# hszhao/semseg

Hardware: NVIDIA B200
Metric: PSPNet50 473x473 training images/sec (higher is better)
Workload: dtype bf16

## Files before the change

include/semseg_b200.h:

```cpp
#ifndef SEMSEG_B200_H
#define SEMSEG_B200_H

#include <stdint.h>

#ifdef __cplusplus
extern "C" {
#endif

#define SEMSEG_OK 0
#define SEMSEG_E_INVALID (-1)
#define SEMSEG_E_CUDA (-2)
#define SEMSEG_E_UNSUPPORTED (-3)

#define SEMSEG_MAX_TAPS 9

const char* semseg_last_error(void);
int semseg_abi_version(void);
long long semseg_launch_count(void);

int semseg_psamask_fwd(int psa_type, const float* in, float* out, int N, int H, int W, int mH, int mW,
                       void* stream);
int semseg_psamask_bwd(int psa_type, const float* dout, float* din, int N, int H, int W, int mH, int mW,
                       void* stream);

int semseg_psa_attend(int mode, int psa_type, const float* attn, int a_pitch, const void* feat, const void* feat_lo,
                      int feat_pitch, float* stats, void* out, void* out_lo, int out_pitch, int N, int H, int W, int mH,
                      int mW, int C, float scale, void* stream);
int semseg_psa_attend_bwd_attn(int psa_type, const float* attn, int a_pitch, const float* stats, const void* feat,
                               const void* feat_lo, int feat_pitch, const void* out, const void* out_lo, int out_pitch,
                               const void* dout, const void* dout_lo, int dout_pitch, float* dattn, int N, int H, int W,
                               int mH, int mW, int C, float scale, void* stream);

enum {
  SEMSEG_EPI_RAW = 0,
  SEMSEG_EPI_AFFINE = 1,
  SEMSEG_EPI_F32 = 2
};

typedef struct semseg_conv_desc {
  int32_t N, H, W;
  int32_t Cin, Cout;
  const void* x;
  int32_t Nin, Hin, Win, x_pitch;
  const void* w;
  int32_t n_wtaps, w_rows, w_cols;
  int32_t taps;
  int32_t dh[SEMSEG_MAX_TAPS], dw[SEMSEG_MAX_TAPS], wtap[SEMSEG_MAX_TAPS];
  int32_t img_mul, img_add[SEMSEG_MAX_TAPS];
  int32_t epi_mode;
  int32_t relu;
  void* y;
  int32_t y_pitch;
  const float* scale;
  const float* shift;
  const void* residual;
  int32_t res_pitch;
  float* out_f32;
  int32_t out_pitch;
  float* stats_partial;
  const void* x_lo;
  void* y_lo;
  const void* residual_lo;
  int32_t w_split;
  int32_t k_slices;
  int64_t slice_stride;
} semseg_conv_desc;

int semseg_conv_k_slices(int Cin, int taps, int max_kblocks);
int semseg_conv_splitk_rows(int M);
int semseg_conv_splitk_finish(const float* partial, int k_slices, long long slice_stride, int part_pitch, int M, int C,
                              int epi_mode, int relu, const float* scale, const float* shift, const void* residual,
                              const void* residual_lo, int res_pitch, void* y, void* y_lo, int y_pitch,
                              float* stats_partial, void* stream);
int semseg_conv_stats_rows(int N, int H, int W, int Cout);
int semseg_conv_fprop(const semseg_conv_desc* d, void* stream);

typedef struct semseg_wgrad_desc {
  int32_t N, H, W;
  int32_t Cin, Cout;
  const void* x;
  int32_t Nin, Hin, Win, x_pitch;
  const void* dy;
  int32_t dy_pitch;
  int32_t taps;
  int32_t dh[SEMSEG_MAX_TAPS], dw[SEMSEG_MAX_TAPS];
  int32_t img_mul, img_add[SEMSEG_MAX_TAPS];
  float* dw_partial;
  int32_t n_splits;
  const void* x_lo;
  const void* dy_lo;
} semseg_wgrad_desc;

int semseg_conv_wgrad_splits(const semseg_wgrad_desc* d);
int semseg_conv_wgrad(const semseg_wgrad_desc* d, void* stream);
int semseg_wgrad_reduce(const float* dw_partial, int n_splits, int taps, int Cout, int Cin, float* dw_oihw,
                        int accumulate, void* stream);

int semseg_pack_weights(const float* w_oihw, int Cout, int Cin, int taps, void* wf, int rows_f, int cols_f,
                        void* wd, int rows_d, int cols_d, int split, void* stream);

typedef struct semseg_pack_item {
  const float* w;
  void* wf;
  void* wd;
  int Cout, Cin, taps;
  int cols_f, cols_d;
  int tile0, tiles_ci;
  int split;
} semseg_pack_item;
int semseg_pack_weights_multi(const semseg_pack_item* items_dev, int n_items, int n_tiles, int max_taps, void* stream);

int semseg_nchw_f32_to_nhwc_bf16(const float* in, void* out, void* out_lo, int N, int C, int H, int W, int out_pitch,
                                 void* stream);
int semseg_nhwc_bf16_to_nchw_f32(const void* in, const void* in_lo, float* out, int N, int C, int H, int W,
                                 int in_pitch, void* stream);
int semseg_nhwc_f32_to_nchw_f32(const float* in, float* out, int N, int C, int H, int W, int in_pitch,
                                void* stream);

int semseg_im2col3x3s2(const void* x, int x_pitch, int N, int H, int W, int Cin, void* out, void* stream);

int semseg_space_to_phases(const void* x, int x_pitch, int N, int H, int W, int C, void* xp, void* stream);
int semseg_phases_to_space(const void* xp, int N, int H, int W, int C, void* x, void* stream);

int semseg_bn_merge_partials(const float* stats_partial, int rows, int C, float* out_stats, void* stream);
int semseg_bn_stats(const void* x, int M, int C, int pitch, float* workspace, long long workspace_floats,
                    float* out_stats, void* stream);
long long semseg_bn_workspace_floats(int M, int C);
int semseg_bn_finalize(const float* rank_stats, int R, int C, const float* gamma, const float* beta, float eps,
                       float momentum, float* running_mean, float* running_var, float* mean_invstd,
                       float* scale_shift, void* stream);
int semseg_bn_finalize_partials(const float* stats_partial, int rows, int C, const float* gamma, const float* beta, float eps, float momentum,
                                float* running_mean, float* running_var, float* mean_invstd, float* scale_shift,
                                void* stream);
int semseg_bn_finalize_p2p(const float* stats_partial, int rows, int C, const float* gamma, const float* beta,
                           float eps, float momentum, float* running_mean, float* running_var, float* mean_invstd,
                           float* scale_shift, void* const* peer_bufs, void* const* peer_flags, void* counter,
                           int world, int rank, int slot, int slot_floats, unsigned seq, const void* seq_ptr,
                           void* stream);
int semseg_bn_bwd_reduce_p2p(const void* dy, const void* dy_lo, int dy_pitch, const void* y, const void* y_lo,
                             int y_pitch, const void* x, const void* x_lo, int x_pitch, const float* mean_invstd,
                             const float* scale_shift, int M, int C, int relu, float* workspace,
                             long long workspace_floats, float* sums_local, float* sums_total,
                             void* const* peer_bufs, void* const* peer_flags, void* counter, int world, int rank,
                             int slot, int slot_floats, unsigned seq, const void* seq_ptr, void* stream);
int semseg_bn_fold_eval(const float* gamma, const float* beta, const float* running_mean,
                        const float* running_var, float eps, int C, float* scale_shift, void* stream);
int semseg_bn_apply(const void* x, const void* x_lo, int x_pitch, const float* scale_shift, const void* residual,
                    const void* residual_lo, int res_pitch, void* y, void* y_lo, int y_pitch, int M, int C, int relu,
                    void* stream);
int semseg_bn_bwd_reduce(const void* dy, const void* dy_lo, int dy_pitch, const void* y, const void* y_lo, int y_pitch,
                         const void* x, const void* x_lo, int x_pitch, const float* mean_invstd,
                         const float* scale_shift, int M, int C, int relu, float* workspace,
                         long long workspace_floats, float* sums, void* stream);
int semseg_bn_bwd_apply(const void* dy, const void* dy_lo, int dy_pitch, const void* y, const void* y_lo, int y_pitch,
                        const void* x, const void* x_lo, int x_pitch, const float* mean_invstd, const float* gamma,
                        const float* scale_shift, const float* sums, float count, int M, int C, int relu, void* dx,
                        void* dx_lo, int dx_pitch, void* dres, void* dres_lo, int dres_pitch, float* dgamma_dbeta,
                        void* stream);
int semseg_add_act(const void* a, const void* a_lo, int a_pitch, const void* b, const void* b_lo, int b_pitch,
                   void* out, void* out_lo, int out_pitch, int M, int C, void* stream);
int semseg_scale_nc(const void* x, const void* x_lo, int x_pitch, const float* scale, void* out, void* out_lo,
                    int out_pitch, int N, int HW, int C, void* stream);
int semseg_f32_to_act(const float* in, int in_pitch, void* out, void* out_lo, int out_pitch, long long M, int C,
                      int Cp, void* stream);
int semseg_act_to_f32(const void* in, const void* in_lo, int in_pitch, float* out, int out_pitch, long long M, int C,
                      void* stream);

int semseg_maxpool3x3s2_fwd(const void* x, const void* x_lo, void* y, void* y_lo, void* argcode, int N, int H, int W,
                            int C, void* stream);
int semseg_maxpool3x3s2_bwd(const void* argcode, const void* dy, const void* dy_lo, void* dx, void* dx_lo, int N,
                            int H, int W, int C, void* stream);

int semseg_ppm_pool(const void* x, const void* x_lo, int x_pitch, int N, int H, int W, int C, const int* bins,
                    void* const* pooled, void* const* pooled_lo, int nb, void* stream);
int semseg_ppm_pool_bwd(void* const* dpooled, void* const* dpooled_lo, const int* bins, int nb, int N, int H, int W,
                        int C, void* dx, void* dx_lo, int dx_pitch, const void* add, const void* add_lo, int add_pitch,
                        void* stream);
int semseg_ppm_upsample_concat(const void* x, const void* x_lo, int x_pitch, void* const* feats, void* const* feats_lo,
                               const int* bins, int nb, int N, int H, int W, int C, int Cr, void* out, void* out_lo,
                               int out_pitch, void* stream);
int semseg_ppm_upsample_bwd(const void* dout, const void* dout_lo, int dout_pitch, int c_off, void* const* dfeats,
                            void* const* dfeats_lo, const int* bins, int nb, int N, int H, int W, int Cr, void* stream);

int semseg_resize_bilinear_fwd(const void* x, const void* x_lo, int x_pitch, int N, int Hi, int Wi, int C, int Ho,
                               int Wo, void* y, void* y_lo, int y_pitch, void* stream);
int semseg_resize_bilinear_bwd(const void* dy, const void* dy_lo, int dy_pitch, int N, int Hi, int Wi, int C, int Ho,
                               int Wo, void* dx, void* dx_lo, int dx_pitch, void* stream);

long long semseg_upsample_ce_workspace_floats(int N, int Ho, int Wo);
int semseg_upsample_ce_fwd(const float* logits, int pitch, int N, int h, int w, int C, const int64_t* target,
                           int Ho, int Wo, int ignore_index, float* workspace, float* loss_out, int64_t* argmax,
                           float* lse, void* stream);
long long semseg_upsample_ce_bwd_workspace_floats(int N, int Ho, int w, int C);
int semseg_upsample_ce_bwd(const float* logits, int pitch, int N, int h, int w, int C, const int64_t* target,
                           int Ho, int Wo, int ignore_index, const float* lse, const float* loss_info,
                           const float* grad_out, float* workspace, float* dlogits, void* stream);

int semseg_iou_hist(void* pred_i64, const void* target_i64, long long n, int K, long long ignore_index, int write_back,
                    int* counts, void* stream);

#define SEMSEG_SGD_MAX_GROUPS 16
typedef struct semseg_sgd_item {
  float* w;
  float* buf;
  long long n;
  int group;
  int chunk0;
  int first;
  int reserved;
} semseg_sgd_item;
typedef struct semseg_sgd_hyper {
  float lr[SEMSEG_SGD_MAX_GROUPS];
  float momentum[SEMSEG_SGD_MAX_GROUPS];
  float weight_decay[SEMSEG_SGD_MAX_GROUPS];
  float dampening[SEMSEG_SGD_MAX_GROUPS];
  int nesterov;
} semseg_sgd_hyper;
int semseg_sgd_chunk_elems(void);
int semseg_sgd_multi(const semseg_sgd_item* items_dev, const void* grad_ptrs_dev, int n_items, int n_chunks,
                     const semseg_sgd_hyper* hyper, void* stream);

#ifdef __cplusplus
}
#endif
#endif
```

semseg_b200/_lib.py:

```python
import ctypes
import os

_HERE = os.path.dirname(os.path.abspath(__file__))
LIB_PATH = os.path.join(_HERE, "lib", "libsemseg_b200.so")

MAX_TAPS = 9
EPI_RAW, EPI_AFFINE, EPI_F32 = 0, 1, 2

c_int = ctypes.c_int
c_i32 = ctypes.c_int32
c_vp = ctypes.c_void_p
c_f = ctypes.c_float
c_ll = ctypes.c_longlong
I9 = c_i32 * MAX_TAPS


class PackItem(ctypes.Structure):
    _fields_ = [
        ("w", c_vp), ("wf", c_vp), ("wd", c_vp),
        ("Cout", c_i32), ("Cin", c_i32), ("taps", c_i32),
        ("cols_f", c_i32), ("cols_d", c_i32),
        ("tile0", c_i32), ("tiles_ci", c_i32),
        ("split", c_i32),
    ]


class SgdItem(ctypes.Structure):
    _fields_ = [("w", c_vp), ("buf", c_vp), ("n", c_ll), ("group", c_i32), ("chunk0", c_i32), ("first", c_i32),
                ("reserved", c_i32)]


class SgdHyper(ctypes.Structure):
    _fields_ = [("lr", c_f * 16), ("momentum", c_f * 16), ("weight_decay", c_f * 16), ("dampening", c_f * 16),
                ("nesterov", c_i32)]


class ConvDesc(ctypes.Structure):
    _fields_ = [
        ("N", c_i32), ("H", c_i32), ("W", c_i32),
        ("Cin", c_i32), ("Cout", c_i32),
        ("x", c_vp),
        ("Nin", c_i32), ("Hin", c_i32), ("Win", c_i32), ("x_pitch", c_i32),
        ("w", c_vp),
        ("n_wtaps", c_i32), ("w_rows", c_i32), ("w_cols", c_i32),
        ("taps", c_i32),
        ("dh", I9), ("dw", I9), ("wtap", I9),
        ("img_mul", c_i32), ("img_add", I9),
        ("epi_mode", c_i32), ("relu", c_i32),
        ("y", c_vp), ("y_pitch", c_i32),
        ("scale", c_vp), ("shift", c_vp),
        ("residual", c_vp), ("res_pitch", c_i32),
        ("out_f32", c_vp), ("out_pitch", c_i32),
        ("stats_partial", c_vp),
        ("x_lo", c_vp), ("y_lo", c_vp), ("residual_lo", c_vp),
        ("w_split", c_i32),
        ("k_slices", c_i32), ("slice_stride", ctypes.c_int64),
    ]


class WgradDesc(ctypes.Structure):
    _fields_ = [
        ("N", c_i32), ("H", c_i32), ("W", c_i32),
        ("Cin", c_i32), ("Cout", c_i32),
        ("x", c_vp),
        ("Nin", c_i32), ("Hin", c_i32), ("Win", c_i32), ("x_pitch", c_i32),
        ("dy", c_vp), ("dy_pitch", c_i32),
        ("taps", c_i32),
        ("dh", I9), ("dw", I9),
        ("img_mul", c_i32), ("img_add", I9),
        ("dw_partial", c_vp),
        ("n_splits", c_i32),
        ("x_lo", c_vp), ("dy_lo", c_vp),
    ]


SIGNATURES = {
    "semseg_last_error": (ctypes.c_char_p, []),
    "semseg_abi_version": (c_int, []),
    "semseg_launch_count": (c_ll, []),
    "semseg_psamask_fwd": (c_int, [c_int, c_vp, c_vp, c_int, c_int, c_int, c_int, c_int, c_vp]),
    "semseg_psamask_bwd": (c_int, [c_int, c_vp, c_vp, c_int, c_int, c_int, c_int, c_int, c_vp]),
    "semseg_psa_attend": (c_int, [c_int, c_int, c_vp, c_int, c_vp, c_vp, c_int, c_vp, c_vp, c_vp, c_int, c_int, c_int,
                                  c_int, c_int, c_int, c_int, c_f, c_vp]),
    "semseg_psa_attend_bwd_attn": (c_int, [c_int, c_vp, c_int, c_vp, c_vp, c_vp, c_int, c_vp, c_vp, c_int, c_vp, c_vp,
                                           c_int, c_vp, c_int, c_int, c_int, c_int, c_int, c_int, c_f, c_vp]),
    "semseg_conv_stats_rows": (c_int, [c_int, c_int, c_int, c_int]),
    "semseg_conv_k_slices": (c_int, [c_int, c_int, c_int]),
    "semseg_conv_splitk_rows": (c_int, [c_int]),
    "semseg_conv_splitk_finish": (c_int, [c_vp, c_int, c_ll, c_int, c_int, c_int, c_int, c_int, c_vp, c_vp, c_vp, c_vp,
                                          c_int, c_vp, c_vp, c_int, c_vp, c_vp]),
    "semseg_conv_fprop": (c_int, [ctypes.POINTER(ConvDesc), c_vp]),
    "semseg_conv_wgrad_splits": (c_int, [ctypes.POINTER(WgradDesc)]),
    "semseg_conv_wgrad": (c_int, [ctypes.POINTER(WgradDesc), c_vp]),
    "semseg_wgrad_reduce": (c_int, [c_vp, c_int, c_int, c_int, c_int, c_vp, c_int, c_vp]),
    "semseg_pack_weights": (c_int, [c_vp, c_int, c_int, c_int, c_vp, c_int, c_int, c_vp, c_int, c_int, c_int, c_vp]),
    "semseg_pack_weights_multi": (c_int, [c_vp, c_int, c_int, c_int, c_vp]),
    "semseg_sgd_chunk_elems": (c_int, []),
    "semseg_sgd_multi": (c_int, [c_vp, c_vp, c_int, c_int, ctypes.POINTER(SgdHyper), c_vp]),
    "semseg_iou_hist": (c_int, [c_vp, c_vp, ctypes.c_longlong, c_int, ctypes.c_longlong, c_int, c_vp, c_vp]),
    "semseg_im2col3x3s2": (c_int, [c_vp, c_int, c_int, c_int, c_int, c_int, c_vp, c_vp]),
    "semseg_nchw_f32_to_nhwc_bf16": (c_int, [c_vp, c_vp, c_vp, c_int, c_int, c_int, c_int, c_int, c_vp]),
    "semseg_nhwc_bf16_to_nchw_f32": (c_int, [c_vp, c_vp, c_vp, c_int, c_int, c_int, c_int, c_int, c_vp]),
    "semseg_nhwc_f32_to_nchw_f32": (c_int, [c_vp, c_vp, c_int, c_int, c_int, c_int, c_int, c_vp]),
    "semseg_space_to_phases": (c_int, [c_vp, c_int, c_int, c_int, c_int, c_int, c_vp, c_vp]),
    "semseg_phases_to_space": (c_int, [c_vp, c_int, c_int, c_int, c_int, c_vp, c_vp]),
    "semseg_bn_merge_partials": (c_int, [c_vp, c_int, c_int, c_vp, c_vp]),
    "semseg_bn_stats": (c_int, [c_vp, c_int, c_int, c_int, c_vp, c_ll, c_vp, c_vp]),
    "semseg_bn_workspace_floats": (c_ll, [c_int, c_int]),
    "semseg_bn_finalize": (c_int, [c_vp, c_int, c_int, c_vp, c_vp, c_f, c_f, c_vp, c_vp, c_vp, c_vp, c_vp]),
    "semseg_bn_finalize_partials": (c_int, [c_vp, c_int, c_int, c_vp, c_vp, c_f, c_f, c_vp, c_vp, c_vp, c_vp, c_vp]),
    "semseg_bn_finalize_p2p": (c_int, [c_vp, c_int, c_int, c_vp, c_vp, c_f, c_f, c_vp, c_vp, c_vp, c_vp, c_vp, c_vp,
                                       c_vp, c_int, c_int, c_int, c_int, ctypes.c_uint, c_vp, c_vp]),
    "semseg_bn_bwd_reduce_p2p": (c_int, [c_vp, c_vp, c_int, c_vp, c_vp, c_int, c_vp, c_vp, c_int, c_vp, c_vp, c_int,
                                         c_int, c_int, c_vp, c_ll, c_vp, c_vp, c_vp, c_vp, c_vp, c_int, c_int, c_int,
                                         c_int, ctypes.c_uint, c_vp, c_vp]),
    "semseg_bn_fold_eval": (c_int, [c_vp, c_vp, c_vp, c_vp, c_f, c_int, c_vp, c_vp]),
    "semseg_bn_apply": (c_int, [c_vp, c_vp, c_int, c_vp, c_vp, c_vp, c_int, c_vp, c_vp, c_int, c_int, c_int, c_int,
                                c_vp]),
    "semseg_bn_bwd_reduce": (c_int, [c_vp, c_vp, c_int, c_vp, c_vp, c_int, c_vp, c_vp, c_int, c_vp, c_vp, c_int, c_int,
                                     c_int, c_vp, c_ll, c_vp, c_vp]),
    "semseg_bn_bwd_apply": (c_int, [c_vp, c_vp, c_int, c_vp, c_vp, c_int, c_vp, c_vp, c_int, c_vp, c_vp, c_vp, c_vp,
                                    c_f, c_int, c_int, c_int, c_vp, c_vp, c_int, c_vp, c_vp, c_int, c_vp, c_vp]),
    "semseg_add_act": (c_int, [c_vp, c_vp, c_int, c_vp, c_vp, c_int, c_vp, c_vp, c_int, c_int, c_int, c_vp]),
    "semseg_scale_nc": (c_int, [c_vp, c_vp, c_int, c_vp, c_vp, c_vp, c_int, c_int, c_int, c_int, c_vp]),
    "semseg_f32_to_act": (c_int, [c_vp, c_int, c_vp, c_vp, c_int, c_ll, c_int, c_int, c_vp]),
    "semseg_act_to_f32": (c_int, [c_vp, c_vp, c_int, c_vp, c_int, c_ll, c_int, c_vp]),
    "semseg_maxpool3x3s2_fwd": (c_int, [c_vp, c_vp, c_vp, c_vp, c_vp, c_int, c_int, c_int, c_int, c_vp]),
    "semseg_maxpool3x3s2_bwd": (c_int, [c_vp, c_vp, c_vp, c_vp, c_vp, c_int, c_int, c_int, c_int, c_vp]),
    "semseg_ppm_pool": (c_int, [c_vp, c_vp, c_int, c_int, c_int, c_int, c_int, c_vp, c_vp, c_vp, c_int, c_vp]),
    "semseg_ppm_pool_bwd": (c_int, [c_vp, c_vp, c_vp, c_int, c_int, c_int, c_int, c_int, c_vp, c_vp, c_int, c_vp, c_vp,
                                    c_int, c_vp]),
    "semseg_ppm_upsample_concat": (c_int, [c_vp, c_vp, c_int, c_vp, c_vp, c_vp, c_int, c_int, c_int, c_int, c_int,
                                           c_int, c_vp, c_vp, c_int, c_vp]),
    "semseg_ppm_upsample_bwd": (c_int, [c_vp, c_vp, c_int, c_int, c_vp, c_vp, c_vp, c_int, c_int, c_int, c_int, c_int,
                                        c_vp]),
    "semseg_resize_bilinear_fwd": (c_int, [c_vp, c_vp, c_int, c_int, c_int, c_int, c_int, c_int, c_int, c_vp, c_vp, c_int,
                                           c_vp]),
    "semseg_resize_bilinear_bwd": (c_int, [c_vp, c_vp, c_int, c_int, c_int, c_int, c_int, c_int, c_int, c_vp, c_vp, c_int,
                                           c_vp]),
    "semseg_upsample_ce_workspace_floats": (c_ll, [c_int, c_int, c_int]),
    "semseg_upsample_ce_fwd": (c_int, [c_vp, c_int, c_int, c_int, c_int, c_int, c_vp, c_int, c_int, c_int, c_vp,
                                       c_vp, c_vp, c_vp, c_vp]),
    "semseg_upsample_ce_bwd_workspace_floats": (c_ll, [c_int, c_int, c_int, c_int]),
    "semseg_upsample_ce_bwd": (c_int, [c_vp, c_int, c_int, c_int, c_int, c_int, c_vp, c_int, c_int, c_int, c_vp,
                                       c_vp, c_vp, c_vp, c_vp, c_vp]),
}

_lib = None


class SemsegError(RuntimeError):
    pass


def load():
    global _lib
    if _lib is not None:
        return _lib
    if not os.path.exists(LIB_PATH):
        raise SemsegError(
            "libsemseg_b200.so is not built (%s). Run `python -m semseg_b200.build` "
            "(or __graft_entry__.build()); there is no CPU/PyTorch fallback for this path." % LIB_PATH)
    lib = ctypes.CDLL(LIB_PATH)
    for name, (res, args) in SIGNATURES.items():
        fn = getattr(lib, name)
        fn.restype = res
        fn.argtypes = args
    _lib = lib
    return lib


def check(status, what):
    if status != 0:
        msg = load().semseg_last_error()
        raise SemsegError("%s failed (%d): %s" % (what, status, msg.decode() if msg else "?"))


def launch_count():
    return int(load().semseg_launch_count())
```

semseg_b200/csrc/act.cuh:

```cuda
#pragma once
#include <cuda_bf16.h>
#include <stdint.h>

#include "ptx.cuh"

namespace sb {

typedef __nv_bfloat16 bf16_t;

__device__ __forceinline__ void act_unpack8(const uint4& v, float (&f)[8]) {
  const __nv_bfloat162* h = reinterpret_cast<const __nv_bfloat162*>(&v);
#pragma unroll
  for (int q = 0; q < 4; ++q) {
    const float2 t = __bfloat1622float2(h[q]);
    f[2 * q] = t.x;
    f[2 * q + 1] = t.y;
  }
}
__device__ __forceinline__ uint4 act_pack8(const float (&f)[8]) {
  uint4 o;
  o.x = pack_bf16x2(f[0], f[1]);
  o.y = pack_bf16x2(f[2], f[3]);
  o.z = pack_bf16x2(f[4], f[5]);
  o.w = pack_bf16x2(f[6], f[7]);
  return o;
}

template <bool S>
struct Raw8 {
  uint4 h;
  uint4 l;
};
template <bool S>
__device__ __forceinline__ Raw8<S> act_ldraw(const bf16_t* hi, const bf16_t* lo, long long off) {
  Raw8<S> r;
  r.h = *reinterpret_cast<const uint4*>(hi + off);
  if constexpr (S) r.l = *reinterpret_cast<const uint4*>(lo + off);
  return r;
}
template <bool S>
__device__ __forceinline__ void act_unpack(const Raw8<S>& r, float (&f)[8]) {
  act_unpack8(r.h, f);
  if constexpr (S) {
    float g[8];
    act_unpack8(r.l, g);
#pragma unroll
    for (int q = 0; q < 8; ++q) f[q] += g[q];
  }
}
template <bool S>
__device__ __forceinline__ void act_ld8(const bf16_t* hi, const bf16_t* lo, long long off, float (&f)[8]) {
  act_unpack<S>(act_ldraw<S>(hi, lo, off), f);
}
template <bool S>
__device__ __forceinline__ void act_st8(bf16_t* hi, bf16_t* lo, long long off, const float (&f)[8]) {
  const uint4 h = act_pack8(f);
  *reinterpret_cast<uint4*>(hi + off) = h;
  if constexpr (S) {
    float hf[8], r[8];
    act_unpack8(h, hf);
#pragma unroll
    for (int q = 0; q < 8; ++q) r[q] = f[q] - hf[q];
    *reinterpret_cast<uint4*>(lo + off) = act_pack8(r);
  }
}
__device__ __forceinline__ void act_split1(float v, bf16_t& hi, bf16_t& lo) {
  hi = __float2bfloat16_rn(v);
  lo = __float2bfloat16_rn(v - __bfloat162float(hi));
}

#define SB_ACT_DISPATCH(split, ...)            \
  do {                                         \
    if (split) {                               \
      constexpr bool kS = true;                \
      __VA_ARGS__;                             \
    } else {                                   \
      constexpr bool kS = false;               \
      __VA_ARGS__;                             \
    }                                          \
  } while (0)

}
```

semseg_b200/csrc/bn.cu:

```cuda
#include "host_common.h"
#include "ptx.cuh"
#include "act.cuh"

namespace sb {

struct Moments {
  float n, mean, m2;
};
__device__ __forceinline__ Moments merge(const Moments& a, const Moments& b) {
  if (b.n == 0.f) return a;
  if (a.n == 0.f) return b;
  Moments r;
  r.n = a.n + b.n;
  const float d = b.mean - a.mean;
  r.mean = a.mean + d * (b.n / r.n);
  r.m2 = a.m2 + b.m2 + d * d * (a.n * b.n / r.n);
  return r;
}

__global__ void __launch_bounds__(1024) bn_merge_partials_kernel(const float* __restrict__ part, const float* __restrict__ cnt, int T, int C,
                                         float* __restrict__ out) {
  __shared__ Moments sm[32][33];
  const int cl = threadIdx.x & 31;
  const int tl = threadIdx.x >> 5;
  const int c = blockIdx.x * 32 + cl;
  Moments acc = {0.f, 0.f, 0.f};
  if (c < C) {
    for (int t = tl; t < T; t += 32) {
      const float n = cnt[t];
      if (n > 0.f) {
        Moments m;
        m.n = n;
        m.mean = part[(static_cast<size_t>(t) * 2) * C + c] / n;
        m.m2 = part[(static_cast<size_t>(t) * 2 + 1) * C + c];
        acc = merge(acc, m);
      }
    }
  }
  sm[tl][cl] = acc;
  __syncthreads();
  if (tl == 0 && c < C) {
    Moments r = sm[0][cl];
    for (int i = 1; i < 32; ++i) r = merge(r, sm[i][cl]);
    out[c] = r.mean;
    out[C + c] = r.m2;
    out[2 * C + c] = r.n;
  }
}


template <int CH>
__device__ __forceinline__ Moments block_conv_moments(const float* __restrict__ part, int T, int C, int c0,
                                                      Moments (*sm)[CH + 1]) {
  constexpr int RL = 1024 / CH;
  constexpr int U = 8;
  const int cl = threadIdx.x % CH;
  const int rl = threadIdx.x / CH;
  const int c = c0 + cl;
  float S = 0.f, Q = 0.f, n = 0.f;
  if (c < C) {
    for (int t0 = rl; t0 < T; t0 += RL * U) {
      float s[U], q[U], m[U];
#pragma unroll
      for (int u = 0; u < U; ++u) {
        const int t = t0 + RL * u;
        const bool ok = t < T;
        const float* row = part + static_cast<size_t>(ok ? t : 0) * 3 * C;
        s[u] = ok ? row[c] : 0.f;
        q[u] = ok ? row[C + c] : 0.f;
        m[u] = ok ? row[2 * C + c] : 0.f;
      }
#pragma unroll
      for (int u = 0; u < U; ++u) {
        S += s[u];
        Q += q[u];
        n += m[u];
      }
    }
  }
#pragma unroll
  for (int o = CH; o < 32; o <<= 1) {
    S += __shfl_xor_sync(0xffffffffu, S, o);
    Q += __shfl_xor_sync(0xffffffffu, Q, o);
    n += __shfl_xor_sync(0xffffffffu, n, o);
  }
  Moments acc = {0.f, 0.f, 0.f};
  if (n > 0.f) {
    acc.n = n;
    acc.mean = S / n;
    acc.m2 = fmaxf(Q - S * acc.mean, 0.f);
  }
  if ((threadIdx.x & 31) < CH) sm[threadIdx.x >> 5][cl] = acc;
  __syncthreads();
  Moments r = {0.f, 0.f, 0.f};
  const int w = threadIdx.x >> 5, lane = threadIdx.x & 31;
  if (w < CH) {
    r = sm[lane][w];
#pragma unroll
    for (int o = 16; o > 0; o >>= 1) {
      Moments other;
      other.mean = __shfl_down_sync(0xffffffffu, r.mean, o);
      other.m2 = __shfl_down_sync(0xffffffffu, r.m2, o);
      other.n = __shfl_down_sync(0xffffffffu, r.n, o);
      r = merge(r, other);
    }
  }
  return r;
}

static int stats_group_channels(int C) { return C <= 1024 ? 8 : (C <= 2048 ? 16 : 32); }

template <int CH>
__global__ void __launch_bounds__(1024) bn_merge_conv_partials_kernel(const float* __restrict__ part, int T, int C,
                                                                      float* __restrict__ out) {
  __shared__ Moments sm[32][CH + 1];
  const Moments r = block_conv_moments<CH>(part, T, C, blockIdx.x * CH, sm);
  const int c = blockIdx.x * CH + (threadIdx.x >> 5);
  if ((threadIdx.x & 31) == 0 && (threadIdx.x >> 5) < CH && c < C) {
    out[c] = r.mean;
    out[C + c] = r.m2;
    out[2 * C + c] = r.n;
  }
}

template <int CH>
__global__ void __launch_bounds__(1024) bn_finalize_partials_kernel(const float* __restrict__ part, int T, int C,
                                            const float* __restrict__ gamma, const float* __restrict__ beta,
                                            float eps, float momentum, float* __restrict__ running_mean,
                                            float* __restrict__ running_var, float* __restrict__ mean_invstd,
                                            float* __restrict__ scale_shift) {
  __shared__ Moments sm[32][CH + 1];
  const Moments r = block_conv_moments<CH>(part, T, C, blockIdx.x * CH, sm);
  const int c = blockIdx.x * CH + (threadIdx.x >> 5);
  if ((threadIdx.x & 31) == 0 && (threadIdx.x >> 5) < CH && c < C) {
    const float var = r.n > 0.f ? r.m2 / r.n : 0.f;
    const float invstd = rsqrtf(var + eps);
    mean_invstd[c] = r.mean;
    mean_invstd[C + c] = invstd;
    mean_invstd[2 * C + c] = r.n;
    const float sc = (gamma ? gamma[c] : 1.f) * invstd;
    scale_shift[c] = sc;
    scale_shift[C + c] = (beta ? beta[c] : 0.f) - r.mean * sc;
    if (running_mean) running_mean[c] = (1.f - momentum) * running_mean[c] + momentum * r.mean;
    if (running_var) {
      const float unb = r.n > 1.f ? r.m2 / (r.n - 1.f) : var;
      running_var[c] = (1.f - momentum) * running_var[c] + momentum * unb;
    }
  }
}

__global__ void bn_chunk_stats_kernel(const __nv_bfloat16* __restrict__ x, int M, int C, int pitch,
                                      int rows_per_chunk, float* __restrict__ part, float* __restrict__ cnt) {
  __shared__ float s_sum[32][65];
  const int gl = threadIdx.x & 7;
  const int pl = threadIdx.x >> 3;
  const int c0 = blockIdx.x * 64 + gl * 8;
  const int chunk = blockIdx.y;
  const int r0 = chunk * rows_per_chunk;
  const int r1 = min(M, r0 + rows_per_chunk);
  const bool active = c0 < C;
  float s[8] = {0, 0, 0, 0, 0, 0, 0, 0};
  if (active) {
    for (int r = r0 + pl; r < r1; r += 32) {
      const uint4 v = *reinterpret_cast<const uint4*>(x + static_cast<size_t>(r) * pitch + c0);
      const __nv_bfloat162* h = reinterpret_cast<const __nv_bfloat162*>(&v);
#pragma unroll
      for (int q = 0; q < 4; ++q) {
        const float2 f = __bfloat1622float2(h[q]);
        s[2 * q] += f.x;
        s[2 * q + 1] += f.y;
      }
    }
  }
#pragma unroll
  for (int q = 0; q < 8; ++q) s_sum[pl][gl * 8 + q] = s[q];
  __syncthreads();
  const float n = static_cast<float>(r1 - r0);
  float mean[8];
#pragma unroll
  for (int q = 0; q < 8; ++q) {
    float t = 0.f;
    for (int i = 0; i < 32; ++i) t += s_sum[i][gl * 8 + q];
    mean[q] = t / n;
    s[q] = t;
  }
  __syncthreads();
  float m2[8] = {0, 0, 0, 0, 0, 0, 0, 0};
  if (active) {
    for (int r = r0 + pl; r < r1; r += 32) {
      const uint4 v = *reinterpret_cast<const uint4*>(x + static_cast<size_t>(r) * pitch + c0);
      const __nv_bfloat162* h = reinterpret_cast<const __nv_bfloat162*>(&v);
#pragma unroll
      for (int q = 0; q < 4; ++q) {
        const float2 f = __bfloat1622float2(h[q]);
        const float d0 = f.x - mean[2 * q], d1 = f.y - mean[2 * q + 1];
        m2[2 * q] = fmaf(d0, d0, m2[2 * q]);
        m2[2 * q + 1] = fmaf(d1, d1, m2[2 * q + 1]);
      }
    }
  }
#pragma unroll
  for (int q = 0; q < 8; ++q) s_sum[pl][gl * 8 + q] = m2[q];
  __syncthreads();
  if (pl == 0 && active) {
#pragma unroll
    for (int q = 0; q < 8; ++q) {
      float t = 0.f;
      for (int i = 0; i < 32; ++i) t += s_sum[i][gl * 8 + q];
      if (c0 + q < C) {
        part[(static_cast<size_t>(chunk) * 2) * C + c0 + q] = s[q];
        part[(static_cast<size_t>(chunk) * 2 + 1) * C + c0 + q] = t;
      }
    }
  }
  if (blockIdx.x == 0 && threadIdx.x == 0) cnt[chunk] = n;
}

__global__ void bn_finalize_kernel(const float* __restrict__ rs, int R, int C, const float* __restrict__ gamma,
                                   const float* __restrict__ beta, float eps, float momentum,
                                   float* __restrict__ running_mean, float* __restrict__ running_var,
                                   float* __restrict__ mean_invstd, float* __restrict__ scale_shift) {
  const int c = blockIdx.x * blockDim.x + threadIdx.x;
  if (c >= C) return;
  Moments acc = {0.f, 0.f, 0.f};
  for (int r = 0; r < R; ++r) {
    const float* b = rs + static_cast<size_t>(r) * 3 * C;
    Moments m;
    m.mean = b[c];
    m.m2 = b[C + c];
    m.n = b[2 * C + c];
    acc = merge(acc, m);
  }
  const float var = acc.n > 0.f ? acc.m2 / acc.n : 0.f;
  const float invstd = rsqrtf(var + eps);
  mean_invstd[c] = acc.mean;
  mean_invstd[C + c] = invstd;
  mean_invstd[2 * C + c] = acc.n;
  const float g = gamma ? gamma[c] : 1.f;
  const float bt = beta ? beta[c] : 0.f;
  const float sc = g * invstd;
  scale_shift[c] = sc;
  scale_shift[C + c] = bt - acc.mean * sc;
  if (running_mean) running_mean[c] = (1.f - momentum) * running_mean[c] + momentum * acc.mean;
  if (running_var) {
    const float unb = acc.n > 1.f ? acc.m2 / (acc.n - 1.f) : var;
    running_var[c] = (1.f - momentum) * running_var[c] + momentum * unb;
  }
}

__global__ void bn_fold_eval_kernel(const float* __restrict__ gamma, const float* __restrict__ beta,
                                    const float* __restrict__ rm, const float* __restrict__ rv, float eps, int C,
                                    float* __restrict__ scale_shift) {
  const int c = blockIdx.x * blockDim.x + threadIdx.x;
  if (c >= C) return;
  const float invstd = rsqrtf(rv[c] + eps);
  const float sc = (gamma ? gamma[c] : 1.f) * invstd;
  scale_shift[c] = sc;
  scale_shift[C + c] = (beta ? beta[c] : 0.f) - rm[c] * sc;
}

__device__ __forceinline__ void unpack8(const uint4& v, float (&f)[8]) {
  const __nv_bfloat162* h = reinterpret_cast<const __nv_bfloat162*>(&v);
#pragma unroll
  for (int q = 0; q < 4; ++q) {
    const float2 t = __bfloat1622float2(h[q]);
    f[2 * q] = t.x;
    f[2 * q + 1] = t.y;
  }
}
__device__ __forceinline__ uint4 pack8(const float (&f)[8]) {
  uint4 o;
  o.x = pack_bf16x2(f[0], f[1]);
  o.y = pack_bf16x2(f[2], f[3]);
  o.z = pack_bf16x2(f[4], f[5]);
  o.w = pack_bf16x2(f[6], f[7]);
  return o;
}

template <bool S>
__global__ void bn_apply_kernel(const __nv_bfloat16* __restrict__ x, const __nv_bfloat16* __restrict__ x_lo, int x_pitch,
                                const float* __restrict__ ss, const __nv_bfloat16* __restrict__ res,
                                const __nv_bfloat16* __restrict__ res_lo, int res_pitch, __nv_bfloat16* __restrict__ y,
                                __nv_bfloat16* __restrict__ y_lo, int y_pitch, long long M, int C, int relu) {
  const int groups = C >> 3;
  long long idx = static_cast<long long>(blockIdx.x) * blockDim.x + threadIdx.x;
  const long long stride = static_cast<long long>(gridDim.x) * blockDim.x;
  const int c0 = static_cast<int>(idx % groups) << 3;
  float sc[8], sh[8];
#pragma unroll
  for (int q = 0; q < 8; ++q) {
    sc[q] = ss[c0 + q];
    sh[q] = ss[C + c0 + q];
  }
  const long long pstride = stride / groups;
  long long p = idx / groups;
  constexpr int U = 4;
  for (; p + (U - 1) * pstride < M; p += U * pstride) {
    Raw8<S> xv[U], rv[U];
#pragma unroll
    for (int u = 0; u < U; ++u) xv[u] = act_ldraw<S>(x, x_lo, (p + u * pstride) * x_pitch + c0);
    if (res) {
#pragma unroll
      for (int u = 0; u < U; ++u) rv[u] = act_ldraw<S>(res, res_lo, (p + u * pstride) * res_pitch + c0);
    }
#pragma unroll
    for (int u = 0; u < U; ++u) {
      float f[8], r[8] = {0, 0, 0, 0, 0, 0, 0, 0};
      act_unpack<S>(xv[u], f);
      if (res) act_unpack<S>(rv[u], r);
#pragma unroll
      for (int q = 0; q < 8; ++q) {
        float v = fmaf(f[q], sc[q], sh[q]) + r[q];
        if (relu) v = fmaxf(v, 0.f);
        f[q] = v;
      }
      act_st8<S>(y, y_lo, (p + u * pstride) * y_pitch + c0, f);
    }
  }
  for (; p < M; p += pstride) {
    float f[8], r[8] = {0, 0, 0, 0, 0, 0, 0, 0};
    act_ld8<S>(x, x_lo, p * x_pitch + c0, f);
    if (res) act_ld8<S>(res, res_lo, p * res_pitch + c0, r);
#pragma unroll
    for (int q = 0; q < 8; ++q) {
      float v = fmaf(f[q], sc[q], sh[q]) + r[q];
      if (relu) v = fmaxf(v, 0.f);
      f[q] = v;
    }
    act_st8<S>(y, y_lo, p * y_pitch + c0, f);
  }
}

template <bool S>
__global__ void bn_bwd_reduce_kernel(const __nv_bfloat16* __restrict__ dy, const __nv_bfloat16* __restrict__ dy_lo,
                                     int dy_pitch, const __nv_bfloat16* __restrict__ y,
                                     const __nv_bfloat16* __restrict__ y_lo, int y_pitch,
                                     const __nv_bfloat16* __restrict__ x, const __nv_bfloat16* __restrict__ x_lo,
                                     int x_pitch, const float* __restrict__ mean_invstd, const float* __restrict__ ss,
                                     int M, int C, int relu, int rows_per_chunk, float* __restrict__ part) {
  __shared__ float s_a[32][65];
  __shared__ float s_b[32][65];
  const int gl = threadIdx.x & 7;
  const int pl = threadIdx.x >> 3;
  const int c0 = blockIdx.x * 64 + gl * 8;
  const int chunk = blockIdx.y;
  const int r0 = chunk * rows_per_chunk;
  const int r1 = min(M, r0 + rows_per_chunk);
  const bool active = c0 < C;
  float a[8] = {0, 0, 0, 0, 0, 0, 0, 0}, b[8] = {0, 0, 0, 0, 0, 0, 0, 0};
  if (active) {
    float mean[8], invstd[8], msc[8], msh[8];
#pragma unroll
    for (int q = 0; q < 8; ++q) {
      mean[q] = mean_invstd[c0 + q];
      invstd[q] = mean_invstd[C + c0 + q];
      msc[q] = ss ? ss[c0 + q] : 0.f;
      msh[q] = ss ? ss[C + c0 + q] : 0.f;
    }
    const bool mask_from_y = relu && y != nullptr;
    const bool mask_from_x = relu && y == nullptr;
    constexpr int U = S ? 2 : 4;
    auto accumulate = [&](float (&d)[8], const float (&xv)[8], const float (&yv)[8]) {
      if (mask_from_y) {
#pragma unroll
        for (int q = 0; q < 8; ++q)
          if (!(yv[q] > 0.f)) d[q] = 0.f;
      } else if (mask_from_x) {
#pragma unroll
        for (int q = 0; q < 8; ++q)
          if (!(fmaf(xv[q], msc[q], msh[q]) > 0.f)) d[q] = 0.f;
      }
#pragma unroll
      for (int q = 0; q < 8; ++q) {
        a[q] += d[q];
        b[q] = fmaf(d[q], (xv[q] - mean[q]) * invstd[q], b[q]);
      }
    };
    int r = r0 + pl;
    for (; r + (U - 1) * 32 < r1; r += U * 32) {
      Raw8<S> dv[U], xr[U], yr[U];
#pragma unroll
      for (int u = 0; u < U; ++u) {
        dv[u] = act_ldraw<S>(dy, dy_lo, static_cast<long long>(r + u * 32) * dy_pitch + c0);
        xr[u] = act_ldraw<S>(x, x_lo, static_cast<long long>(r + u * 32) * x_pitch + c0);
      }
      if (mask_from_y) {
#pragma unroll
        for (int u = 0; u < U; ++u) yr[u] = act_ldraw<S>(y, y_lo, static_cast<long long>(r + u * 32) * y_pitch + c0);
      }
#pragma unroll
      for (int u = 0; u < U; ++u) {
        float d[8], xv[8], yv[8] = {0, 0, 0, 0, 0, 0, 0, 0};
        act_unpack<S>(dv[u], d);
        act_unpack<S>(xr[u], xv);
        if (mask_from_y) act_unpack<S>(yr[u], yv);
        accumulate(d, xv, yv);
      }
    }
    for (; r < r1; r += 32) {
      float d[8], xv[8], yv[8] = {0, 0, 0, 0, 0, 0, 0, 0};
      act_ld8<S>(dy, dy_lo, static_cast<long long>(r) * dy_pitch + c0, d);
      act_ld8<S>(x, x_lo, static_cast<long long>(r) * x_pitch + c0, xv);
      if (mask_from_y) act_ld8<S>(y, y_lo, static_cast<long long>(r) * y_pitch + c0, yv);
      accumulate(d, xv, yv);
    }
  }
#pragma unroll
  for (int q = 0; q < 8; ++q) {
    s_a[pl][gl * 8 + q] = a[q];
    s_b[pl][gl * 8 + q] = b[q];
  }
  __syncthreads();
  if (pl < 2 && active) {
    float(*src)[65] = pl == 0 ? s_a : s_b;
#pragma unroll
    for (int q = 0; q < 8; ++q) {
      float t = 0.f;
      for (int i = 0; i < 32; ++i) t += src[i][gl * 8 + q];
      if (c0 + q < C) part[(static_cast<size_t>(chunk) * 2 + pl) * C + c0 + q] = t;
    }
  }
}

__global__ void __launch_bounds__(1024) bn_bwd_reduce_final_kernel(const float* __restrict__ part, int chunks, int C,
                                           float* __restrict__ sums) {
  __shared__ float sm[32][33];
  const int cl = threadIdx.x & 31;
  const int tl = threadIdx.x >> 5;
  const int idx = blockIdx.x * 32 + cl;
  float acc = 0.f;
  if (idx < 2 * C) {
    const int which = idx / C, c = idx - which * C;
    constexpr int U = 8;
    for (int t0 = tl; t0 < chunks; t0 += 32 * U) {
      float v[U];
#pragma unroll
      for (int u = 0; u < U; ++u) {
        const int t = t0 + 32 * u;
        v[u] = t < chunks ? part[(static_cast<size_t>(t) * 2 + which) * C + c] : 0.f;
      }
#pragma unroll
      for (int u = 0; u < U; ++u) acc += v[u];
    }
  }
  sm[tl][cl] = acc;
  __syncthreads();
  if (tl == 0 && idx < 2 * C) {
    float r = 0.f;
    for (int i = 0; i < 32; ++i) r += sm[i][cl];
    sums[idx] = r;
  }
}

template <bool S>
__global__ void bn_bwd_apply_kernel(const __nv_bfloat16* __restrict__ dy, const __nv_bfloat16* __restrict__ dy_lo,
                                    int dy_pitch, const __nv_bfloat16* __restrict__ y,
                                    const __nv_bfloat16* __restrict__ y_lo, int y_pitch,
                                    const __nv_bfloat16* __restrict__ x, const __nv_bfloat16* __restrict__ x_lo,
                                    int x_pitch, const float* __restrict__ mean_invstd, const float* __restrict__ gamma,
                                    const float* __restrict__ ss, const float* __restrict__ sums, float inv_count,
                                    long long M, int C, int relu, __nv_bfloat16* __restrict__ dx,
                                    __nv_bfloat16* __restrict__ dx_lo, int dx_pitch, __nv_bfloat16* __restrict__ dres,
                                    __nv_bfloat16* __restrict__ dres_lo, int dres_pitch,
                                    float* __restrict__ dgamma_dbeta) {
  const int groups = C >> 3;
  if (dgamma_dbeta && blockIdx.x == 0) {
    for (int c = threadIdx.x; c < C; c += blockDim.x) {
      dgamma_dbeta[c] = sums[C + c];
      dgamma_dbeta[C + c] = sums[c];
    }
  }
  long long idx = static_cast<long long>(blockIdx.x) * blockDim.x + threadIdx.x;
  const long long stride = static_cast<long long>(gridDim.x) * blockDim.x;
  const int c0 = static_cast<int>(idx % groups) << 3;
  float ka[8], kx[8], kb[8], msc[8], msh[8];
  const bool mask_from_y = relu && y != nullptr;
  const bool mask_from_x = relu && y == nullptr;
#pragma unroll
  for (int q = 0; q < 8; ++q) {
    const int c = c0 + q;
    msc[q] = ss ? ss[c] : 0.f;
    msh[q] = ss ? ss[C + c] : 0.f;
    const float mean = mean_invstd[c], invstd = mean_invstd[C + c];
    const float g = gamma ? gamma[c] : 1.f;
    ka[q] = g * invstd;
    const float ic = inv_count > 0.f ? inv_count : 1.f / mean_invstd[2 * C + c];
    kx[q] = -ka[q] * invstd * sums[C + c] * ic;
    kb[q] = -ka[q] * sums[c] * ic - kx[q] * mean;
  }
  auto finish = [&](float (&d)[8], const float (&xv)[8], const float (&yv)[8], long long pp) {
    if (mask_from_y) {
#pragma unroll
      for (int q = 0; q < 8; ++q)
        if (!(yv[q] > 0.f)) d[q] = 0.f;
    } else if (mask_from_x) {
#pragma unroll
      for (int q = 0; q < 8; ++q)
        if (!(fmaf(xv[q], msc[q], msh[q]) > 0.f)) d[q] = 0.f;
    }
    if (dres) act_st8<S>(dres, dres_lo, pp * dres_pitch + c0, d);
    float o[8];
#pragma unroll
    for (int q = 0; q < 8; ++q) o[q] = fmaf(ka[q], d[q], fmaf(kx[q], xv[q], kb[q]));
    act_st8<S>(dx, dx_lo, pp * dx_pitch + c0, o);
  };
  const long long pstride = stride / groups;
  long long p = idx / groups;
  constexpr int U = 2;
  for (; p + (U - 1) * pstride < M; p += U * pstride) {
    Raw8<S> dv[U], xr[U], yr[U];
#pragma unroll
    for (int u = 0; u < U; ++u) {
      dv[u] = act_ldraw<S>(dy, dy_lo, (p + u * pstride) * dy_pitch + c0);
      xr[u] = act_ldraw<S>(x, x_lo, (p + u * pstride) * x_pitch + c0);
    }
    if (mask_from_y) {
#pragma unroll
      for (int u = 0; u < U; ++u) yr[u] = act_ldraw<S>(y, y_lo, (p + u * pstride) * y_pitch + c0);
    }
#pragma unroll
    for (int u = 0; u < U; ++u) {
      float d[8], xv[8], yv[8] = {0, 0, 0, 0, 0, 0, 0, 0};
      act_unpack<S>(dv[u], d);
      act_unpack<S>(xr[u], xv);
      if (mask_from_y) act_unpack<S>(yr[u], yv);
      finish(d, xv, yv, p + u * pstride);
    }
  }
  for (; p < M; p += pstride) {
    float d[8], xv[8], yv[8] = {0, 0, 0, 0, 0, 0, 0, 0};
    act_ld8<S>(dy, dy_lo, p * dy_pitch + c0, d);
    act_ld8<S>(x, x_lo, p * x_pitch + c0, xv);
    if (mask_from_y) act_ld8<S>(y, y_lo, p * y_pitch + c0, yv);
    finish(d, xv, yv, p);
  }
}

template <bool S>
__global__ void add_act_kernel(const __nv_bfloat16* __restrict__ a, const __nv_bfloat16* __restrict__ a_lo, int a_pitch,
                               const __nv_bfloat16* __restrict__ b, const __nv_bfloat16* __restrict__ b_lo, int b_pitch,
                               __nv_bfloat16* __restrict__ out, __nv_bfloat16* __restrict__ out_lo, int out_pitch,
                               long long M, int C) {
  const int groups = C >> 3;
  const long long total = M * groups;
  for (long long idx = static_cast<long long>(blockIdx.x) * blockDim.x + threadIdx.x; idx < total;
       idx += static_cast<long long>(gridDim.x) * blockDim.x) {
    const long long p = idx / groups;
    const int c0 = static_cast<int>(idx - p * groups) << 3;
    float x[8], z[8];
    act_ld8<S>(a, a_lo, p * a_pitch + c0, x);
    act_ld8<S>(b, b_lo, p * b_pitch + c0, z);
#pragma unroll
    for (int q = 0; q < 8; ++q) x[q] += z[q];
    act_st8<S>(out, out_lo, p * out_pitch + c0, x);
  }
}

template <bool S>
__global__ void scale_nc_kernel(const __nv_bfloat16* __restrict__ x, const __nv_bfloat16* __restrict__ x_lo, int x_pitch,
                                const float* __restrict__ s, __nv_bfloat16* __restrict__ out,
                                __nv_bfloat16* __restrict__ out_lo, int out_pitch, int N, long long HW, int C) {
  const int groups = C >> 3;
  const long long total = static_cast<long long>(N) * HW * groups;
  for (long long idx = static_cast<long long>(blockIdx.x) * blockDim.x + threadIdx.x; idx < total;
       idx += static_cast<long long>(gridDim.x) * blockDim.x) {
    const long long p = idx / groups;
    const int c0 = static_cast<int>(idx - p * groups) << 3;
    const int n = static_cast<int>(p / HW);
    float f[8];
    act_ld8<S>(x, x_lo, p * x_pitch + c0, f);
    const float4 s0 = *reinterpret_cast<const float4*>(s + static_cast<size_t>(n) * C + c0);
    const float4 s1 = *reinterpret_cast<const float4*>(s + static_cast<size_t>(n) * C + c0 + 4);
    f[0] *= s0.x; f[1] *= s0.y; f[2] *= s0.z; f[3] *= s0.w;
    f[4] *= s1.x; f[5] *= s1.y; f[6] *= s1.z; f[7] *= s1.w;
    act_st8<S>(out, out_lo, p * out_pitch + c0, f);
  }
}

template <bool S>
__global__ void __launch_bounds__(256)
conv_splitk_finish_kernel(const float* __restrict__ part, int k_slices, long long slice_stride, int part_pitch, int M, int C,
                          int affine, int relu, const float* __restrict__ scale, const float* __restrict__ shift,
                          const __nv_bfloat16* __restrict__ res, const __nv_bfloat16* __restrict__ res_lo, int res_pitch,
                          __nv_bfloat16* __restrict__ y, __nv_bfloat16* __restrict__ y_lo, int y_pitch,
                          int rows_per_chunk, float* __restrict__ stats) {
  __shared__ float s_a[32][65];
  __shared__ float s_b[32][65];
  const int gl = threadIdx.x & 7;
  const int pl = threadIdx.x >> 3;
  const int c0 = blockIdx.x * 64 + gl * 8;
  const int chunk = blockIdx.y;
  const int r0 = chunk * rows_per_chunk;
  const int r1 = min(M, r0 + rows_per_chunk);
  float a[8] = {0, 0, 0, 0, 0, 0, 0, 0}, b[8] = {0, 0, 0, 0, 0, 0, 0, 0};
  float sc[8], sh[8];
#pragma unroll
  for (int q = 0; q < 8; ++q) {
    sc[q] = (affine && scale) ? scale[c0 + q] : 1.f;
    sh[q] = (affine && shift) ? shift[c0 + q] : 0.f;
  }
  for (int r = r0 + pl; r < r1; r += 32) {
    float v[8] = {0, 0, 0, 0, 0, 0, 0, 0};
    const float* src = part + static_cast<long long>(r) * part_pitch + c0;
    for (int s = 0; s < k_slices; ++s) {
      const float4 p0 = *reinterpret_cast<const float4*>(src + s * slice_stride);
      const float4 p1 = *reinterpret_cast<const float4*>(src + s * slice_stride + 4);
      v[0] += p0.x; v[1] += p0.y; v[2] += p0.z; v[3] += p0.w;
      v[4] += p1.x; v[5] += p1.y; v[6] += p1.z; v[7] += p1.w;
    }
    if (affine) {
      float rr[8] = {0, 0, 0, 0, 0, 0, 0, 0};
      if (res) act_ld8<S>(res, res_lo, static_cast<long long>(r) * res_pitch + c0, rr);
#pragma unroll
      for (int q = 0; q < 8; ++q) {
        float t = fmaf(v[q], sc[q], sh[q]) + rr[q];
        v[q] = relu ? fmaxf(t, 0.f) : t;
      }
    }
    act_st8<S>(y, y_lo, static_cast<long long>(r) * y_pitch + c0, v);
    if (stats) {
      float w[8];
      act_ld8<S>(y, y_lo, static_cast<long long>(r) * y_pitch + c0, w);
#pragma unroll
      for (int q = 0; q < 8; ++q) {
        a[q] += w[q];
        b[q] = fmaf(w[q], w[q], b[q]);
      }
    }
  }
  if (!stats) return;
#pragma unroll
  for (int q = 0; q < 8; ++q) {
    s_a[pl][gl * 8 + q] = a[q];
    s_b[pl][gl * 8 + q] = b[q];
  }
  __syncthreads();
  if (pl < 3) {
    float* row = stats + static_cast<size_t>(chunk) * 3 * C;
#pragma unroll
    for (int q = 0; q < 8; ++q) {
      float t = 0.f;
      if (pl < 2) {
        float(*src)[65] = pl == 0 ? s_a : s_b;
        for (int i = 0; i < 32; ++i) t += src[i][gl * 8 + q];
      } else {
        t = static_cast<float>(r1 - r0);
      }
      row[pl * C + c0 + q] = t;
    }
  }
}

template <bool S>
__global__ void f32_to_act_kernel(const float* __restrict__ in, int in_pitch, __nv_bfloat16* __restrict__ out,
                                  __nv_bfloat16* __restrict__ out_lo, int out_pitch, long long M, int C, int Cp) {
  const int groups = Cp >> 3;
  const long long total = M * groups;
  for (long long idx = static_cast<long long>(blockIdx.x) * blockDim.x + threadIdx.x; idx < total;
       idx += static_cast<long long>(gridDim.x) * blockDim.x) {
    const long long p = idx / groups;
    const int c0 = static_cast<int>(idx - p * groups) << 3;
    float f[8];
#pragma unroll
    for (int q = 0; q < 8; ++q) f[q] = (c0 + q < C) ? in[p * in_pitch + c0 + q] : 0.f;
    act_st8<S>(out, out_lo, p * out_pitch + c0, f);
  }
}

template <bool S>
__global__ void act_to_f32_kernel(const __nv_bfloat16* __restrict__ in, const __nv_bfloat16* __restrict__ in_lo,
                                  int in_pitch, float* __restrict__ out, int out_pitch, long long M, int C) {
  const int groups = C >> 3;
  const long long total = M * groups;
  for (long long idx = static_cast<long long>(blockIdx.x) * blockDim.x + threadIdx.x; idx < total;
       idx += static_cast<long long>(gridDim.x) * blockDim.x) {
    const long long p = idx / groups;
    const int c0 = static_cast<int>(idx - p * groups) << 3;
    float f[8];
    act_ld8<S>(in, in_lo, p * in_pitch + c0, f);
#pragma unroll
    for (int q = 0; q < 8; ++q) out[p * out_pitch + c0 + q] = f[q];
  }
}

struct PeerArgs {
  float* buf[8];
  unsigned* flags[8];
  unsigned* counter;
  int world, rank, slot, slot_floats;
  unsigned seq;
  const unsigned* seq_ptr;
  long long timeout_ticks;
};

__device__ __forceinline__ void st_ll(unsigned long long* p, float v, unsigned seq) {
  const unsigned long long w = (static_cast<unsigned long long>(seq) << 32) | __float_as_uint(v);
  asm volatile("st.relaxed.sys.global.u64 [%0], %1;" ::"l"(p), "l"(w) : "memory");
}
__device__ __forceinline__ float ld_ll(const unsigned long long* p, unsigned seq, const PeerArgs& pa, int peer) {
  unsigned long long w;
  const long long t0 = clock64();
  for (;;) {
    asm volatile("ld.relaxed.sys.global.u64 %0, [%1];" : "=l"(w) : "l"(p) : "memory");
    if (static_cast<unsigned>(w >> 32) == seq) break;
    if (clock64() - t0 > pa.timeout_ticks) {
      printf("semseg_b200: SyncBN peer exchange timed out (rank %d waiting for rank %d, slot %d, seq %u)\n", pa.rank, peer,
             pa.slot, seq);
      __trap();
    }
  }
  return __uint_as_float(static_cast<unsigned>(w & 0xffffffffu));
}

template <int CH>
__global__ void __launch_bounds__(1024) bn_finalize_p2p_kernel(const float* __restrict__ part, int T, int C, const float* __restrict__ gamma,
                                       const float* __restrict__ beta, float eps, float momentum,
                                       float* __restrict__ running_mean, float* __restrict__ running_var,
                                       float* __restrict__ mean_invstd, float* __restrict__ scale_shift, PeerArgs pa) {
  __shared__ Moments sm[32][CH + 1];
  const Moments own_m = block_conv_moments<CH>(part, T, C, blockIdx.x * CH, sm);
  const int c = blockIdx.x * CH + (threadIdx.x >> 5);
  if (!((threadIdx.x & 31) == 0 && (threadIdx.x >> 5) < CH && c < C)) return;
  const unsigned seq = pa.seq_ptr ? *pa.seq_ptr : pa.seq;
  const size_t slot0 = static_cast<size_t>(pa.slot) * pa.world * pa.slot_floats;
  {
    const size_t off = slot0 + static_cast<size_t>(pa.rank) * pa.slot_floats;
    for (int p = 0; p < pa.world; ++p) {
      unsigned long long* dst = reinterpret_cast<unsigned long long*>(pa.buf[p]) + off;
      st_ll(dst + c, own_m.mean, seq);
      st_ll(dst + C + c, own_m.m2, seq);
      st_ll(dst + 2 * C + c, own_m.n, seq);
    }
  }
  Moments r = {0.f, 0.f, 0.f};
  for (int p = 0; p < pa.world; ++p) {
    const unsigned long long* b = reinterpret_cast<const unsigned long long*>(pa.buf[pa.rank]) + slot0 +
                                  static_cast<size_t>(p) * pa.slot_floats;
    Moments m;
    m.mean = ld_ll(b + c, seq, pa, p);
    m.m2 = ld_ll(b + C + c, seq, pa, p);
    m.n = ld_ll(b + 2 * C + c, seq, pa, p);
    r = merge(r, m);
  }
  const float var = r.n > 0.f ? r.m2 / r.n : 0.f;
  const float invstd = rsqrtf(var + eps);
  mean_invstd[c] = r.mean;
  mean_invstd[C + c] = invstd;
  mean_invstd[2 * C + c] = r.n;
  const float sc = (gamma ? gamma[c] : 1.f) * invstd;
  scale_shift[c] = sc;
  scale_shift[C + c] = (beta ? beta[c] : 0.f) - r.mean * sc;
  if (running_mean) running_mean[c] = (1.f - momentum) * running_mean[c] + momentum * r.mean;
  if (running_var) {
    const float unb = r.n > 1.f ? r.m2 / (r.n - 1.f) : var;
    running_var[c] = (1.f - momentum) * running_var[c] + momentum * unb;
  }
}

__global__ void __launch_bounds__(1024) bn_bwd_reduce_final_p2p_kernel(const float* __restrict__ part, int chunks, int C,
                                               float* __restrict__ sums_local, float* __restrict__ sums_total,
                                               PeerArgs pa) {
  __shared__ float sm[32][33];
  const int cl = threadIdx.x & 31;
  const int tl = threadIdx.x >> 5;
  const int idx = blockIdx.x * 32 + cl;
  float acc = 0.f;
  if (idx < 2 * C) {
    const int which = idx / C, c = idx - which * C;
    constexpr int U = 8;
    for (int t0 = tl; t0 < chunks; t0 += 32 * U) {
      float v[U];
#pragma unroll
      for (int u = 0; u < U; ++u) {
        const int t = t0 + 32 * u;
        v[u] = t < chunks ? part[(static_cast<size_t>(t) * 2 + which) * C + c] : 0.f;
      }
#pragma unroll
      for (int u = 0; u < U; ++u) acc += v[u];
    }
  }
  sm[tl][cl] = acc;
  __syncthreads();
  if (!(tl == 0 && idx < 2 * C)) return;
  float own = 0.f;
  for (int i = 0; i < 32; ++i) own += sm[i][cl];
  sums_local[idx] = own;
  const unsigned seq = pa.seq_ptr ? *pa.seq_ptr : pa.seq;
  const size_t slot0 = static_cast<size_t>(pa.slot) * pa.world * pa.slot_floats;
  const size_t off = slot0 + static_cast<size_t>(pa.rank) * pa.slot_floats + idx;
  for (int p = 0; p < pa.world; ++p) st_ll(reinterpret_cast<unsigned long long*>(pa.buf[p]) + off, own, seq);
  float r = 0.f;
  for (int p = 0; p < pa.world; ++p)
    r += ld_ll(reinterpret_cast<const unsigned long long*>(pa.buf[pa.rank]) + slot0 + static_cast<size_t>(p) * pa.slot_floats + idx,
               seq, pa, p);
  sums_total[idx] = r;
}

static int ew_grid(long long total, int threads) {
  long long b = (total + threads - 1) / threads;
  const long long cap = static_cast<long long>(num_sms()) * 16;
  if (b > cap) b = cap;
  if (b < 1) b = 1;
  return static_cast<int>(b);
}

static int ew_grid_fixed_channels(long long total, int threads, int groups) {
  long long b = ew_grid(total, threads);
  long long m = 1;
  while ((m * threads) % groups != 0) ++m;
  b = (b + m - 1) / m * m;
  return static_cast<int>(b);
}

static int chunk_rows(int M) {
  int rows = cdiv(M, 1024);
  if (rows < 256) rows = 256;
  return (rows + 31) & ~31;
}

}

using namespace sb;
typedef __nv_bfloat16 bf16;

extern "C" long long semseg_bn_workspace_floats(int M, int C) {
  if (M <= 0 || C <= 0) return 0;
  const int rows = chunk_rows(M);
  const long long chunks = cdiv(M, rows);
  return chunks * 2 * C + chunks + 3LL * C;
}

extern "C" int semseg_bn_merge_partials(const float* stats_partial, int rows, int C, float* out_stats, void* stream_) {
  cudaStream_t stream = static_cast<cudaStream_t>(stream_);
  SB_CHECK_ARG(stats_partial && out_stats && rows > 0 && C > 0, "bn_merge_partials: bad args");
  switch (stats_group_channels(C)) {
    case 8: bn_merge_conv_partials_kernel<8><<<cdiv(C, 8), 1024, 0, stream>>>(stats_partial, rows, C, out_stats); break;
    case 16: bn_merge_conv_partials_kernel<16><<<cdiv(C, 16), 1024, 0, stream>>>(stats_partial, rows, C, out_stats); break;
    default: bn_merge_conv_partials_kernel<32><<<cdiv(C, 32), 1024, 0, stream>>>(stats_partial, rows, C, out_stats); break;
  }
  SB_LAUNCHED();
  return SEMSEG_OK;
}

extern "C" int semseg_bn_finalize_partials(const float* stats_partial, int num_tiles, int C,
                                           const float* gamma, const float* beta, float eps, float momentum,
                                           float* running_mean, float* running_var, float* mean_invstd,
                                           float* scale_shift, void* stream_) {
  cudaStream_t stream = static_cast<cudaStream_t>(stream_);
  SB_CHECK_ARG(stats_partial && mean_invstd && scale_shift && num_tiles > 0 && C > 0,
               "bn_finalize_partials: bad args");
  switch (stats_group_channels(C)) {
    case 8: bn_finalize_partials_kernel<8><<<cdiv(C, 8), 1024, 0, stream>>>(stats_partial, num_tiles, C, gamma, beta, eps, momentum, running_mean, running_var, mean_invstd, scale_shift); break;
    case 16: bn_finalize_partials_kernel<16><<<cdiv(C, 16), 1024, 0, stream>>>(stats_partial, num_tiles, C, gamma, beta, eps, momentum, running_mean, running_var, mean_invstd, scale_shift); break;
    default: bn_finalize_partials_kernel<32><<<cdiv(C, 32), 1024, 0, stream>>>(stats_partial, num_tiles, C, gamma, beta, eps, momentum, running_mean, running_var, mean_invstd, scale_shift); break;
  }
  SB_LAUNCHED();
  return SEMSEG_OK;
}

extern "C" int semseg_bn_stats(const void* x, int M, int C, int pitch, float* workspace, long long workspace_floats,
                               float* out_stats, void* stream_) {
  cudaStream_t stream = static_cast<cudaStream_t>(stream_);
  SB_CHECK_ARG(x && workspace && out_stats && M > 0 && C > 0, "bn_stats: bad args");
  SB_CHECK_ARG(C % 8 == 0 && pitch % 8 == 0 && pitch >= C, "bn_stats: C/pitch must be multiples of 8");
  SB_CHECK_ARG(workspace_floats >= semseg_bn_workspace_floats(M, C), "bn_stats: workspace too small");
  const int rows = chunk_rows(M);
  const int chunks = cdiv(M, rows);
  float* part = workspace;
  float* cnt = workspace + static_cast<size_t>(chunks) * 2 * C;
  dim3 grid(cdiv(C, 64), chunks);
  bn_chunk_stats_kernel<<<grid, 256, 0, stream>>>(static_cast<const bf16*>(x), M, C, pitch, rows, part, cnt);
  SB_LAUNCHED();
  bn_merge_partials_kernel<<<cdiv(C, 32), 1024, 0, stream>>>(part, cnt, chunks, C, out_stats);
  SB_LAUNCHED();
  return SEMSEG_OK;
}

extern "C" int semseg_bn_finalize(const float* rank_stats, int R, int C, const float* gamma, const float* beta,
                                  float eps, float momentum, float* running_mean, float* running_var,
                                  float* mean_invstd, float* scale_shift, void* stream_) {
  cudaStream_t stream = static_cast<cudaStream_t>(stream_);
  SB_CHECK_ARG(rank_stats && mean_invstd && scale_shift && R > 0 && C > 0, "bn_finalize: bad args");
  bn_finalize_kernel<<<cdiv(C, 128), 128, 0, stream>>>(rank_stats, R, C, gamma, beta, eps, momentum, running_mean,
                                                      running_var, mean_invstd, scale_shift);
  SB_LAUNCHED();
  return SEMSEG_OK;
}

extern "C" int semseg_bn_fold_eval(const float* gamma, const float* beta, const float* running_mean,
                                   const float* running_var, float eps, int C, float* scale_shift, void* stream_) {
  cudaStream_t stream = static_cast<cudaStream_t>(stream_);
  SB_CHECK_ARG(running_mean && running_var && scale_shift && C > 0, "bn_fold_eval: bad args");
  bn_fold_eval_kernel<<<cdiv(C, 128), 128, 0, stream>>>(gamma, beta, running_mean, running_var, eps, C, scale_shift);
  SB_LAUNCHED();
  return SEMSEG_OK;
}

extern "C" int semseg_bn_apply(const void* x, const void* x_lo, int x_pitch, const float* scale_shift,
                               const void* residual, const void* residual_lo, int res_pitch, void* y, void* y_lo,
                               int y_pitch, int M, int C, int relu, void* stream_) {
  cudaStream_t stream = static_cast<cudaStream_t>(stream_);
  SB_CHECK_ARG(x && scale_shift && y && M > 0 && C > 0, "bn_apply: bad args");
  SB_CHECK_ARG(C % 8 == 0 && x_pitch % 8 == 0 && y_pitch % 8 == 0 && (!residual || res_pitch % 8 == 0),
               "bn_apply: channels and pitches must be multiples of 8");
  const bool split = x_lo != nullptr;
  SB_CHECK_ARG((y_lo != nullptr) == split && (!residual || (residual_lo != nullptr) == split),
               "bn_apply: all tensors must use the same storage form (plain or split)");
  const long long total = static_cast<long long>(M) * (C / 8);
  const int grid = ew_grid_fixed_channels(total, 256, C / 8);
  SB_ACT_DISPATCH(split, bn_apply_kernel<kS><<<grid, 256, 0, stream>>>(
                             static_cast<const bf16*>(x), static_cast<const bf16*>(x_lo), x_pitch, scale_shift,
                             static_cast<const bf16*>(residual), static_cast<const bf16*>(residual_lo), res_pitch,
                             static_cast<bf16*>(y), static_cast<bf16*>(y_lo), y_pitch, M, C, relu));
  SB_LAUNCHED();
  return SEMSEG_OK;
}

static int launch_bwd_reduce(const void* dy, const void* dy_lo, int dy_pitch, const void* y, const void* y_lo,
                             int y_pitch, const void* x, const void* x_lo, int x_pitch, const float* mean_invstd,
                             const float* scale_shift, int M, int C, int relu, float* workspace, cudaStream_t stream) {
  const bool split = dy_lo != nullptr;
  SB_CHECK_ARG((x_lo != nullptr) == split && (!(relu && y) || (y_lo != nullptr) == split),
               "bn_bwd_reduce: all tensors must use the same storage form (plain or split)");
  const int rows = chunk_rows(M);
  const int chunks = cdiv(M, rows);
  dim3 grid(cdiv(C, 64), chunks);
  SB_ACT_DISPATCH(split, bn_bwd_reduce_kernel<kS><<<grid, 256, 0, stream>>>(
                             static_cast<const bf16*>(dy), static_cast<const bf16*>(dy_lo), dy_pitch,
                             static_cast<const bf16*>(y), static_cast<const bf16*>(y_lo), y_pitch,
                             static_cast<const bf16*>(x), static_cast<const bf16*>(x_lo), x_pitch, mean_invstd,
                             scale_shift, M, C, relu, rows, workspace));
  SB_LAUNCHED();
  return SEMSEG_OK;
}

extern "C" int semseg_bn_bwd_reduce(const void* dy, const void* dy_lo, int dy_pitch, const void* y, const void* y_lo,
                                    int y_pitch, const void* x, const void* x_lo, int x_pitch,
                                    const float* mean_invstd, const float* scale_shift, int M, int C, int relu,
                                    float* workspace, long long workspace_floats, float* sums, void* stream_) {
  cudaStream_t stream = static_cast<cudaStream_t>(stream_);
  SB_CHECK_ARG(dy && x && mean_invstd && workspace && sums && M > 0 && C > 0, "bn_bwd_reduce: bad args");
  SB_CHECK_ARG(!relu || y || scale_shift, "bn_bwd_reduce: relu needs y or scale_shift");
  SB_CHECK_ARG(C % 8 == 0 && dy_pitch % 8 == 0 && x_pitch % 8 == 0 && (!(relu && y) || y_pitch % 8 == 0),
               "bn_bwd_reduce: channels and pitches must be multiples of 8");
  SB_CHECK_ARG(workspace_floats >= semseg_bn_workspace_floats(M, C), "bn_bwd_reduce: workspace too small");
  int r = launch_bwd_reduce(dy, dy_lo, dy_pitch, y, y_lo, y_pitch, x, x_lo, x_pitch, mean_invstd, scale_shift, M, C,
                            relu, workspace, stream);
  if (r) return r;
  bn_bwd_reduce_final_kernel<<<cdiv(2 * C, 32), 1024, 0, stream>>>(workspace, cdiv(M, chunk_rows(M)), C, sums);
  SB_LAUNCHED();
  return SEMSEG_OK;
}

extern "C" int semseg_bn_bwd_apply(const void* dy, const void* dy_lo, int dy_pitch, const void* y, const void* y_lo,
                                   int y_pitch, const void* x, const void* x_lo, int x_pitch,
                                   const float* mean_invstd, const float* gamma, const float* scale_shift,
                                   const float* sums, float count, int M, int C, int relu, void* dx, void* dx_lo,
                                   int dx_pitch, void* dres, void* dres_lo, int dres_pitch, float* dgamma_dbeta,
                                   void* stream_) {
  cudaStream_t stream = static_cast<cudaStream_t>(stream_);
  SB_CHECK_ARG(dy && x && mean_invstd && sums && dx && M > 0 && C > 0, "bn_bwd_apply: bad args");
  SB_CHECK_ARG(!relu || y || scale_shift, "bn_bwd_apply: relu needs y or scale_shift");
  SB_CHECK_ARG(C % 8 == 0 && dy_pitch % 8 == 0 && x_pitch % 8 == 0 && dx_pitch % 8 == 0 &&
                   (!(relu && y) || y_pitch % 8 == 0) && (!dres || dres_pitch % 8 == 0),
               "bn_bwd_apply: channels and pitches must be multiples of 8");
  const bool split = dy_lo != nullptr;
  SB_CHECK_ARG((x_lo != nullptr) == split && (dx_lo != nullptr) == split &&
                   (!(relu && y) || (y_lo != nullptr) == split) && (!dres || (dres_lo != nullptr) == split),
               "bn_bwd_apply: all tensors must use the same storage form (plain or split)");
  const long long total = static_cast<long long>(M) * (C / 8);
  const int grid = ew_grid_fixed_channels(total, 256, C / 8);
  SB_ACT_DISPATCH(split, bn_bwd_apply_kernel<kS><<<grid, 256, 0, stream>>>(
                             static_cast<const bf16*>(dy), static_cast<const bf16*>(dy_lo), dy_pitch,
                             static_cast<const bf16*>(y), static_cast<const bf16*>(y_lo), y_pitch,
                             static_cast<const bf16*>(x), static_cast<const bf16*>(x_lo), x_pitch, mean_invstd, gamma,
                             scale_shift, sums, count > 0.f ? 1.f / count : 0.f, M, C, relu, static_cast<bf16*>(dx),
                             static_cast<bf16*>(dx_lo), dx_pitch, static_cast<bf16*>(dres),
                             static_cast<bf16*>(dres_lo), dres_pitch, dgamma_dbeta));
  SB_LAUNCHED();
  return SEMSEG_OK;
}

extern "C" int semseg_add_act(const void* a, const void* a_lo, int a_pitch, const void* b, const void* b_lo,
                              int b_pitch, void* out, void* out_lo, int out_pitch, int M, int C, void* stream_) {
  cudaStream_t stream = static_cast<cudaStream_t>(stream_);
  SB_CHECK_ARG(a && b && out && M > 0 && C > 0 && C % 8 == 0 && a_pitch % 8 == 0 && b_pitch % 8 == 0 &&
                   out_pitch % 8 == 0,
               "add_act: bad args");
  const bool split = a_lo != nullptr;
  SB_CHECK_ARG((b_lo != nullptr) == split && (out_lo != nullptr) == split,
               "add_act: all tensors must use the same storage form (plain or split)");
  const long long total = static_cast<long long>(M) * (C / 8);
  SB_ACT_DISPATCH(split, add_act_kernel<kS><<<ew_grid(total, 256), 256, 0, stream>>>(
                             static_cast<const bf16*>(a), static_cast<const bf16*>(a_lo), a_pitch,
                             static_cast<const bf16*>(b), static_cast<const bf16*>(b_lo), b_pitch,
                             static_cast<bf16*>(out), static_cast<bf16*>(out_lo), out_pitch, M, C));
  SB_LAUNCHED();
  return SEMSEG_OK;
}

extern "C" int semseg_scale_nc(const void* x, const void* x_lo, int x_pitch, const float* scale, void* out,
                               void* out_lo, int out_pitch, int N, int HW, int C, void* stream_) {
  cudaStream_t stream = static_cast<cudaStream_t>(stream_);
  SB_CHECK_ARG(x && scale && out && N > 0 && HW > 0 && C > 0 && C % 8 == 0 && x_pitch % 8 == 0 && out_pitch % 8 == 0,
               "scale_nc: bad args");
  const bool split = x_lo != nullptr;
  SB_CHECK_ARG((out_lo != nullptr) == split, "scale_nc: input and output must use the same storage form");
  const long long total = static_cast<long long>(N) * HW * (C / 8);
  SB_ACT_DISPATCH(split, scale_nc_kernel<kS><<<ew_grid(total, 256), 256, 0, stream>>>(
                             static_cast<const bf16*>(x), static_cast<const bf16*>(x_lo), x_pitch, scale,
                             static_cast<bf16*>(out), static_cast<bf16*>(out_lo), out_pitch, N, HW, C));
  SB_LAUNCHED();
  return SEMSEG_OK;
}

static int splitk_chunk_rows(int M) {
  int rows = cdiv(M, 2048);
  if (rows < 128) rows = 128;
  return (rows + 31) & ~31;
}

extern "C" int semseg_conv_splitk_rows(int M) { return M > 0 ? cdiv(M, splitk_chunk_rows(M)) : SEMSEG_E_INVALID; }

extern "C" int semseg_conv_splitk_finish(const float* partial, int k_slices, long long slice_stride, int part_pitch,
                                         int M, int C, int epi_mode, int relu, const float* scale, const float* shift,
                                         const void* residual, const void* residual_lo, int res_pitch, void* y,
                                         void* y_lo, int y_pitch, float* stats_partial, void* stream_) {
  cudaStream_t stream = static_cast<cudaStream_t>(stream_);
  SB_CHECK_ARG(partial && y && k_slices >= 1 && M > 0 && C > 0 && C % 64 == 0, "conv_splitk_finish: bad args");
  SB_CHECK_ARG(part_pitch % 4 == 0 && part_pitch >= C && slice_stride % 4 == 0 && y_pitch % 8 == 0 &&
                   (!residual || res_pitch % 8 == 0),
               "conv_splitk_finish: pitches must keep 16-byte alignment");
  SB_CHECK_ARG(epi_mode == SEMSEG_EPI_RAW || epi_mode == SEMSEG_EPI_AFFINE, "conv_splitk_finish: RAW or AFFINE only");
  SB_CHECK_ARG(!stats_partial || epi_mode == SEMSEG_EPI_RAW, "conv_splitk_finish: statistics only in RAW mode");
  const bool split = y_lo != nullptr;
  SB_CHECK_ARG(!residual || (residual_lo != nullptr) == split, "conv_splitk_finish: residual / y storage forms differ");
  const int rows = splitk_chunk_rows(M);
  dim3 grid(C / 64, cdiv(M, rows));
  SB_ACT_DISPATCH(split, conv_splitk_finish_kernel<kS><<<grid, 256, 0, stream>>>(
                             partial, k_slices, slice_stride, part_pitch, M, C, epi_mode == SEMSEG_EPI_AFFINE ? 1 : 0,
                             relu, scale, shift, static_cast<const bf16*>(residual),
                             static_cast<const bf16*>(residual_lo), res_pitch, static_cast<bf16*>(y),
                             static_cast<bf16*>(y_lo), y_pitch, rows, stats_partial));
  SB_LAUNCHED();
  return SEMSEG_OK;
}

extern "C" int semseg_f32_to_act(const float* in, int in_pitch, void* out, void* out_lo, int out_pitch, long long M,
                                 int C, int Cp, void* stream_) {
  cudaStream_t stream = static_cast<cudaStream_t>(stream_);
  SB_CHECK_ARG(in && out && M > 0 && C > 0 && Cp >= C && Cp % 8 == 0 && out_pitch % 8 == 0 && out_pitch >= Cp &&
                   in_pitch >= C,
               "f32_to_act: bad args");
  const long long total = M * (Cp / 8);
  SB_ACT_DISPATCH(out_lo != nullptr, f32_to_act_kernel<kS><<<ew_grid(total, 256), 256, 0, stream>>>(
                                         in, in_pitch, static_cast<bf16*>(out), static_cast<bf16*>(out_lo), out_pitch,
                                         M, C, Cp));
  SB_LAUNCHED();
  return SEMSEG_OK;
}

extern "C" int semseg_act_to_f32(const void* in, const void* in_lo, int in_pitch, float* out, int out_pitch,
                                 long long M, int C, void* stream_) {
  cudaStream_t stream = static_cast<cudaStream_t>(stream_);
  SB_CHECK_ARG(in && out && M > 0 && C > 0 && C % 8 == 0 && in_pitch % 8 == 0 && out_pitch >= C,
               "act_to_f32: bad args");
  const long long total = M * (C / 8);
  SB_ACT_DISPATCH(in_lo != nullptr, act_to_f32_kernel<kS><<<ew_grid(total, 256), 256, 0, stream>>>(
                                        static_cast<const bf16*>(in), static_cast<const bf16*>(in_lo), in_pitch, out,
                                        out_pitch, M, C));
  SB_LAUNCHED();
  return SEMSEG_OK;
}

static int fill_peer_args(sb::PeerArgs* pa, void* const* peer_bufs, void* const* peer_flags, void* counter, int world,
                          int rank, int slot, int slot_floats, unsigned seq, const void* seq_ptr, int need_floats) {
  SB_CHECK_ARG(peer_bufs && peer_flags && counter, "p2p: null peer tables");
  SB_CHECK_ARG(world >= 1 && world <= 8 && rank >= 0 && rank < world, "p2p: world %d rank %d unsupported", world, rank);
  SB_CHECK_ARG(slot >= 0 && need_floats <= slot_floats, "p2p: slot too small (%d > %d floats)", need_floats,
               slot_floats);
  for (int i = 0; i < world; ++i) {
    SB_CHECK_ARG(peer_bufs[i] && peer_flags[i], "p2p: null peer pointer %d", i);
    pa->buf[i] = static_cast<float*>(peer_bufs[i]);
    pa->flags[i] = static_cast<unsigned*>(peer_flags[i]);
  }
  pa->counter = static_cast<unsigned*>(counter);
  pa->world = world;
  pa->rank = rank;
  pa->slot = slot;
  pa->slot_floats = slot_floats;
  pa->seq = seq;
  pa->seq_ptr = static_cast<const unsigned*>(seq_ptr);
  static long long ticks = 0;
  if (ticks == 0) {
    const char* e = getenv("SEMSEG_B200_P2P_TIMEOUT_S");
    double sec = e ? atof(e) : 600.0;
    if (!(sec > 0.0)) sec = 600.0;
    ticks = static_cast<long long>(sec * 2.0e9);
  }
  pa->timeout_ticks = ticks;
  return SEMSEG_OK;
}

extern "C" int semseg_bn_finalize_p2p(const float* stats_partial, int rows, int C, const float* gamma,
                                      const float* beta, float eps, float momentum, float* running_mean,
                                      float* running_var, float* mean_invstd, float* scale_shift,
                                      void* const* peer_bufs, void* const* peer_flags, void* counter, int world,
                                      int rank, int slot, int slot_floats, unsigned seq, const void* seq_ptr,
                                      void* stream_) {
  cudaStream_t stream = static_cast<cudaStream_t>(stream_);
  SB_CHECK_ARG(stats_partial && mean_invstd && scale_shift && rows > 0 && C > 0, "bn_finalize_p2p: bad args");
  sb::PeerArgs pa;
  int r = fill_peer_args(&pa, peer_bufs, peer_flags, counter, world, rank, slot, slot_floats, seq, seq_ptr, 3 * C);
  if (r) return r;
  switch (stats_group_channels(C)) {
    case 8: bn_finalize_p2p_kernel<8><<<cdiv(C, 8), 1024, 0, stream>>>(stats_partial, rows, C, gamma, beta, eps, momentum, running_mean, running_var, mean_invstd, scale_shift, pa); break;
    case 16: bn_finalize_p2p_kernel<16><<<cdiv(C, 16), 1024, 0, stream>>>(stats_partial, rows, C, gamma, beta, eps, momentum, running_mean, running_var, mean_invstd, scale_shift, pa); break;
    default: bn_finalize_p2p_kernel<32><<<cdiv(C, 32), 1024, 0, stream>>>(stats_partial, rows, C, gamma, beta, eps, momentum, running_mean, running_var, mean_invstd, scale_shift, pa); break;
  }
  SB_LAUNCHED();
  return SEMSEG_OK;
}

extern "C" int semseg_bn_bwd_reduce_p2p(const void* dy, const void* dy_lo, int dy_pitch, const void* y,
                                        const void* y_lo, int y_pitch, const void* x, const void* x_lo, int x_pitch,
                                        const float* mean_invstd, const float* scale_shift, int M, int C, int relu,
                                        float* workspace, long long workspace_floats, float* sums_local,
                                        float* sums_total, void* const* peer_bufs, void* const* peer_flags,
                                        void* counter, int world, int rank, int slot, int slot_floats, unsigned seq,
                                        const void* seq_ptr, void* stream_) {
  cudaStream_t stream = static_cast<cudaStream_t>(stream_);
  SB_CHECK_ARG(dy && x && mean_invstd && workspace && sums_local && sums_total && M > 0 && C > 0,
               "bn_bwd_reduce_p2p: bad args");
  SB_CHECK_ARG(!relu || y || scale_shift, "bn_bwd_reduce_p2p: relu needs y or scale_shift");
  SB_CHECK_ARG(C % 8 == 0 && dy_pitch % 8 == 0 && x_pitch % 8 == 0 && (!(relu && y) || y_pitch % 8 == 0),
               "bn_bwd_reduce_p2p: channels and pitches must be multiples of 8");
  SB_CHECK_ARG(workspace_floats >= semseg_bn_workspace_floats(M, C), "bn_bwd_reduce_p2p: workspace too small");
  sb::PeerArgs pa;
  int r = fill_peer_args(&pa, peer_bufs, peer_flags, counter, world, rank, slot, slot_floats, seq, seq_ptr, 2 * C);
  if (r) return r;
  r = launch_bwd_reduce(dy, dy_lo, dy_pitch, y, y_lo, y_pitch, x, x_lo, x_pitch, mean_invstd, scale_shift, M, C, relu,
                        workspace, stream);
  if (r) return r;
  bn_bwd_reduce_final_p2p_kernel<<<cdiv(2 * C, 32), 1024, 0, stream>>>(workspace, cdiv(M, chunk_rows(M)), C,
                                                                      sums_local, sums_total, pa);
  SB_LAUNCHED();
  return SEMSEG_OK;
}
```

semseg_b200/functional.py:

```python
import torch
import torch.distributed as dist
import torch.nn as nn
import torch.nn.functional as F

from . import ops
from . import p2p
from . import precision
from .dist_utils import gather_rank_stats
from .ops import EPI_RAW, EPI_AFFINE, EPI_F32


def packed(conv, need_dgrad=True, split=False):
    w = conv.weight
    key = (w._version, w.data_ptr(), need_dgrad, split)
    cache = conv.__dict__.get("_sb_pack")
    if cache is not None and cache[0] == key:
        return cache[1]
    if cache is not None and cache[0][:2] == key[:2] and cache[0][3] == split and cache[0][2]:
        return cache[1]
    pw = ops.pack_weights(w, need_dgrad=need_dgrad, split=split)
    conv.__dict__["_sb_pack"] = (key, pw)
    return pw


def invalidate_packs(model):
    for m in model.modules():
        m.__dict__.pop("_sb_pack", None)
        m.__dict__.pop("_sb_pack_patches", None)
    model.__dict__.pop("_sb_pack_plan", None)


def packed_patches(conv, split=False):
    w = conv.weight
    key = (w._version, w.data_ptr(), "patches", split)
    cache = conv.__dict__.get("_sb_pack_patches")
    if cache is not None and cache[0] == key:
        return cache[1]
    cout, cin = w.shape[0], w.shape[1]
    flat = torch.zeros((1, cout, 32), dtype=torch.float32, device=w.device)
    flat[0, :, :9 * cin] = w.detach().permute(0, 2, 3, 1).reshape(cout, 9 * cin)
    hi = flat.to(torch.bfloat16)
    wf = torch.stack([hi, (flat - hi.float()).to(torch.bfloat16)], 0) if split else hi
    conv.__dict__["_sb_pack_patches"] = (key, wf)
    return wf


def _is_patch_conv(conv, x):
    return (conv.kernel_size == (3, 3) and conv.stride == (2, 2) and conv.dilation == (1, 1) and conv.padding == (1, 1)
            and conv.in_channels <= 3 and conv.groups == 1 and x.shape[-1] >= 4)


def prepack(model, force=False):
    convs = [m for m in model.modules() if isinstance(m, nn.Conv2d) and m.weight.is_cuda and
             m.weight.dtype == torch.float32 and m.weight.is_contiguous() and m.kernel_size[0] == m.kernel_size[1] and
             m.kernel_size[0] * m.kernel_size[1] <= ops.MAX_TAPS]
    if not convs:
        return
    split = precision.split_enabled()
    keys = [(c.weight._version, c.weight.data_ptr(), True, split) for c in convs]
    if not force and all(c.__dict__.get("_sb_pack", (None,))[0] == k for c, k in zip(convs, keys)):
        return
    plan = model.__dict__.get("_sb_pack_plan")
    weights = [c.weight.detach() for c in convs]
    if plan is None or not plan.valid_for(weights, split):
        plan = ops.WeightPackPlan(weights, split)
        model.__dict__["_sb_pack_plan"] = plan
    plan.refresh()
    for c, k, pw in zip(convs, keys, plan.packs):
        c.__dict__["_sb_pack"] = (k, pw)


def _sync_group(bn):
    if isinstance(bn, nn.SyncBatchNorm) and dist.is_available() and dist.is_initialized():
        pg = bn.process_group if bn.process_group is not None else dist.group.WORLD
        if dist.get_world_size(pg) > 1:
            return pg
    return None


def _bn_momentum(bn):
    if bn.momentum is None:
        return 1.0 / float(bn.num_batches_tracked.item() + 1)
    return bn.momentum


def _finalize_stats(stats, bn, pg, count_batches=True):
    world = 1
    if pg is not None:
        world = dist.get_world_size(pg)
        stats = gather_rank_stats(stats, pg)
    track = bn.track_running_stats and bn.running_mean is not None
    mom = _bn_momentum(bn) if track else 0.0
    mi, ss = ops.bn_finalize(stats, bn.weight, bn.bias, bn.eps, mom, bn.running_mean if track else None,
                             bn.running_var if track else None)
    if count_batches and track and bn.num_batches_tracked is not None:
        bn.num_batches_tracked.add_(1)
    return mi, ss, world


def _bn_backward(ctx_pg, world, dy, y, raw, mi, gamma, relu, want_dres, ss=None):
    n, h, w, c = raw.shape[-4:]
    if not dy.is_contiguous():
        dy = dy.contiguous()
    px = p2p.get_exchange(ctx_pg) if ctx_pg is not None else None
    if px is not None and 2 * c <= p2p.SLOT_FLOATS:
        local, sums = ops.bn_bwd_reduce_p2p(dy, y if relu else None, raw, mi, relu, ss if y is None else None, px)
        dbeta, dgamma = local[0], local[1]
    else:
        sums = ops.bn_bwd_reduce(dy, y if relu else None, raw, mi, relu, scale_shift=ss if y is None else None)
        dbeta, dgamma = sums[0], sums[1]
        if ctx_pg is not None:
            dbeta, dgamma = dbeta.clone(), dgamma.clone()
            dist.all_reduce(sums, group=ctx_pg)
    count = float(n * h * w) if world == 1 else 0.0
    d_raw, dres, _ = ops.bn_bwd_apply(dy, y if relu else None, raw, mi, gamma, sums, count, relu, want_dres=want_dres,
                                      scale_shift=ss if y is None else None)
    return d_raw, dres, dgamma, dbeta


class _CbaState:
    __slots__ = ("xin", "raw", "y", "mi", "gamma", "ss", "pw", "k", "dil", "stride", "relu", "pg", "world",
                 "in_shape", "has_res")


def cba_forward(x, conv, bn, relu, residual, out=None, input_needs_grad=True):
    split = ops.is_split(x)
    pw = packed(conv, split=split)
    k, dil, stride = conv.kernel_size[0], conv.dilation[0], conv.stride[0]
    n, h, w, cx = x.shape[-4:]
    wf = pw.wf
    if stride == 1:
        xin, img_add, out_nhw = x, None, None
        taps = ops.conv_taps(k, dil)
    elif not input_needs_grad and _is_patch_conv(conv, x):
        xin, img_add, out_nhw = ops.im2col3x3s2(x, conv.in_channels), None, None
        taps, wf, stride = ops.conv_taps(1, 1), packed_patches(conv, split), 0
    else:
        xin = ops.space_to_phases(x)
        t2 = ops.conv_taps_s2(k, n)
        taps, img_add = [t[:3] for t in t2], [t[3] for t in t2]
        out_nhw = (n, (h - 1) // 2 + 1, (w - 1) // 2 + 1)
    raw, sp = ops.conv_fprop(xin, wf, pw.cout, taps, stats=True, img_add=img_add, out_nhw=out_nhw)
    pg = _sync_group(bn)
    track = bn.track_running_stats and bn.running_mean is not None
    mom = _bn_momentum(bn) if track else 0.0
    rm, rv = (bn.running_mean, bn.running_var) if track else (None, None)
    px = p2p.get_exchange(pg) if pg is not None else None
    if pg is None:
        mi, ss = ops.bn_finalize_partials(sp, bn.weight, bn.bias, bn.eps, mom, rm, rv)
        world = 1
    elif px is not None and 3 * pw.cout <= p2p.SLOT_FLOATS:
        mi, ss = ops.bn_finalize_p2p(sp, bn.weight, bn.bias, bn.eps, mom, rm, rv, px)
        world = px.world
    else:
        mi, ss, world = _finalize_stats(ops.bn_merge_partials(sp), bn, pg, count_batches=False)
    if track and bn.num_batches_tracked is not None:
        bn.num_batches_tracked.add_(1)
    y = ops.bn_apply(raw, ss, residual=residual, relu=relu, out=out)
    st = _CbaState()
    need_y = relu and residual is not None
    st.xin, st.raw, st.y, st.mi, st.gamma = xin, raw, (y if need_y else None), mi, bn.weight
    st.ss = ss if (relu and not need_y) else None
    st.pw, st.k, st.dil, st.stride, st.relu, st.pg, st.world = pw, k, dil, stride, relu, pg, world
    st.in_shape, st.has_res = (n, h, w, cx), residual is not None
    return y, st


def cba_backward(st, dy, need_dx=True, need_dw=True, need_dres=False, dx_add=None):
    pw = st.pw
    n, h, w, cx = st.in_shape
    d_raw, dres, dgamma, dbeta = _bn_backward(st.pg, st.world, dy, st.y, st.raw, st.mi, st.gamma, st.relu,
                                              st.has_res and need_dres, st.ss)
    dx = dw = None
    if st.stride == 0:
        if need_dx:
            raise RuntimeError("semseg_b200: the patch form of the stem conv was chosen but dx is requested")
        if need_dw:
            cin = pw.cin
            dwp = ops.conv_wgrad(st.xin, d_raw, 32, pw.cout, ops.conv_taps(1, 1))
            dw = dwp[:, :9 * cin, 0, 0].reshape(pw.cout, 3, 3, cin).permute(0, 3, 1, 2).contiguous()
        return dx, dw, dgamma, dbeta, dres
    if st.stride == 1:
        if need_dx:
            if dx_add is not None:
                dx, _ = ops.conv_fprop(d_raw, pw.wd, pw.cin, ops.conv_taps(st.k, st.dil, transpose=True),
                                       epi=EPI_AFFINE, residual=dx_add)
            else:
                dx, _ = ops.conv_fprop(d_raw, pw.wd, pw.cin, ops.conv_taps(st.k, st.dil, transpose=True))
        if need_dw:
            dw = ops.conv_wgrad(st.xin, d_raw, cx, pw.cout, ops.conv_taps(st.k, st.dil))
    else:
        t2 = ops.conv_taps_s2(st.k, n)
        if need_dx:
            if pw.cin % 64 != 0:
                raise NotImplementedError("semseg_b200: input gradient of a stride-2 conv needs Cin % 64 == 0")
            hh, wh = st.xin.shape[-3], st.xin.shape[-2]
            dxp = ops.empty_act((4 * n, hh, wh, pw.cin), ops.is_split(d_raw), dy.device)
            for q in range(4):
                sub = [(-t[0], -t[1], t[2]) for t in t2 if t[4] == (q >> 1, q & 1)]
                part = ops.act_batch_slice(dxp, q * n, (q + 1) * n)
                if sub:
                    ops.conv_fprop(d_raw, pw.wd, pw.cin, sub, out=part, out_nhw=(n, hh, wh))
                else:
                    part.zero_()
            dx = ops.phases_to_space(dxp, n, h, w)
            if dx_add is not None:
                dx = ops.add_act(dx, dx_add)
        if need_dw:
            dw = ops.conv_wgrad(st.xin, d_raw, cx, pw.cout, [t[:2] for t in t2], img_add=[t[3] for t in t2])
    if dw is not None and cx != pw.cin and st.stride != 0:
        dw = dw[:, :pw.cin].contiguous()
    return dx, dw, dgamma, dbeta, dres


class _ConvBnAct(torch.autograd.Function):

    @staticmethod
    def forward(ctx, x, weight, gamma, beta, residual, conv, bn, relu, out):
        y, st = cba_forward(x, conv, bn, relu, residual, out, input_needs_grad=ctx.needs_input_grad[0])
        ctx.st = st
        if out is not None:
            ctx.mark_dirty(out)
        return y

    @staticmethod
    def backward(ctx, dy):
        ni = ctx.needs_input_grad
        dx, dw, dgamma, dbeta, dres = cba_backward(ctx.st, dy, need_dx=ni[0], need_dw=ni[1], need_dres=ni[4])
        ctx.st = None
        return dx, dw, dgamma, dbeta, dres, None, None, None, None


class _BottleneckFn(torch.autograd.Function):

    @staticmethod
    def forward(ctx, x, blk, *params):
        y1, s1 = cba_forward(x, blk.conv1, blk.bn1, True, None)
        y2, s2 = cba_forward(y1, blk.conv2, blk.bn2, True, None)
        if blk.downsample is not None:
            res, sd = cba_forward(x, blk.downsample[0], blk.downsample[1], False, None)
        else:
            res, sd = x, None
        y3, s3 = cba_forward(y2, blk.conv3, blk.bn3, True, res)
        ctx.states = (s1, s2, s3, sd)
        return y3

    @staticmethod
    def backward(ctx, dy):
        s1, s2, s3, sd = ctx.states
        ctx.states = None
        need_dx = ctx.needs_input_grad[0]
        d2, dw3, dg3, db3, dres = cba_backward(s3, dy, need_dres=True)
        d1, dw2, dg2, db2, _ = cba_backward(s2, d2)
        grads_ds = ()
        if sd is not None:
            dxd, dwd, dgd, dbd, _ = cba_backward(sd, dres, need_dx=need_dx)
            dres_to_x = dxd
            grads_ds = (dwd, dgd, dbd)
        else:
            dres_to_x = dres
        dx, dw1, dg1, db1, _ = cba_backward(s1, d1, need_dx=need_dx, dx_add=dres_to_x if need_dx else None)
        return (dx, None, dw1, dg1, db1, dw2, dg2, db2, dw3, dg3, db3) + grads_ds


def bottleneck(x, blk):
    convs = [blk.conv1, blk.conv2, blk.conv3] + ([blk.downsample[0]] if blk.downsample is not None else [])
    bns = [blk.bn1, blk.bn2, blk.bn3] + ([blk.downsample[1]] if blk.downsample is not None else [])
    cins = [x.shape[-1], blk.conv1.out_channels, blk.conv2.out_channels, x.shape[-1]]
    fused = (torch.is_grad_enabled() and all(b.training or b.running_mean is None for b in bns) and
             all(_is_native_conv(c, ci) for c, ci in zip(convs, cins)) and
             (blk.downsample is None or len(blk.downsample) == 2))
    if fused:
        params = [blk.conv1.weight, blk.bn1.weight, blk.bn1.bias, blk.conv2.weight, blk.bn2.weight, blk.bn2.bias,
                  blk.conv3.weight, blk.bn3.weight, blk.bn3.bias]
        if blk.downsample is not None:
            params += [blk.downsample[0].weight, blk.downsample[1].weight, blk.downsample[1].bias]
        return _BottleneckFn.apply(x, blk, *params)
    y = conv_bn_act(x, blk.conv1, blk.bn1, relu=True)
    y = conv_bn_act(y, blk.conv2, blk.bn2, relu=True)
    residual = conv_bn_act(x, blk.downsample[0], blk.downsample[1], relu=False) if blk.downsample is not None else x
    return conv_bn_act(y, blk.conv3, blk.bn3, relu=True, residual=residual)


def _is_native_conv(conv, cin):
    ok = (conv.kernel_size in ((1, 1), (3, 3)) and conv.groups == 1 and conv.bias is None and
          conv.padding == (conv.dilation[0] * (conv.kernel_size[0] // 2),) * 2 and
          conv.dilation[0] == conv.dilation[1] and cin % 8 == 0 and conv.out_channels % 64 == 0)
    if conv.stride == (1, 1):
        return ok
    return ok and conv.stride == (2, 2) and conv.dilation == (1, 1)


def _require_native(conv, cin):
    if not _is_native_conv(conv, cin):
        raise NotImplementedError(
            "semseg_b200: convolution %r on %d input channels is outside the tensor-core kernel's coverage (1x1 / 3x3 "
            "'same' convs without bias, stride 1 with any dilation or stride 2 undilated, Cin %% 8 == 0, Cout %% 64 == 0); "
            "there is no library fallback" % (conv, cin))


def conv_bn_act(x, conv, bn, relu=True, residual=None, out=None):
    use_batch_stats = bn.training or (bn.running_mean is None)
    _require_native(conv, x.shape[-1])
    if use_batch_stats:
        return _ConvBnAct.apply(x, conv.weight, bn.weight, bn.bias, residual, conv, bn, relu, out)
    ss = ops.bn_fold_eval(bn.weight, bn.bias, bn.running_mean, bn.running_var, bn.eps)
    split = ops.is_split(x)
    with torch.no_grad():
        pw = packed(conv, need_dgrad=False, split=split)
        if conv.stride == (1, 1):
            y, _ = ops.conv_fprop(x, pw.wf, pw.cout, ops.conv_taps(conv.kernel_size[0], conv.dilation[0]),
                                  epi=EPI_AFFINE, relu=relu, scale=ss[0], shift=ss[1], residual=residual, out=out)
        else:
            n, h, w, _ = x.shape[-4:]
            t2 = ops.conv_taps_s2(conv.kernel_size[0], n)
            y, _ = ops.conv_fprop(ops.space_to_phases(x), pw.wf, pw.cout, [t[:3] for t in t2], epi=EPI_AFFINE,
                                  relu=relu, scale=ss[0], shift=ss[1], residual=residual, out=out,
                                  img_add=[t[3] for t in t2], out_nhw=(n, (h - 1) // 2 + 1, (w - 1) // 2 + 1))
    return y


class _ConvBiasF32(torch.autograd.Function):

    @staticmethod
    def forward(ctx, x, weight, bias, conv):
        pw = packed(conv, split=ops.is_split(x))
        y, _ = ops.conv_fprop(x, pw.wf, pw.cout, ops.conv_taps(1, 1), epi=EPI_F32, shift=bias)
        ctx.save_for_backward(x)
        ctx.pw = pw
        return y

    @staticmethod
    def backward(ctx, dy):
        (x,) = ctx.saved_tensors
        pw = ctx.pw
        n, h, w, c = dy.shape
        cp = pw.wd.shape[-1]
        dyb = ops.f32_to_act(dy.contiguous(), ops.is_split(x))
        dx = dw = db = None
        if ctx.needs_input_grad[0]:
            dx, _ = ops.conv_fprop(dyb, pw.wd, pw.cin, ops.conv_taps(1, 1))
        if ctx.needs_input_grad[1]:
            dwp = ops.conv_wgrad(x, dyb, pw.cin, cp, ops.conv_taps(1, 1))
            dw = dwp[:c].contiguous()
        if ctx.needs_input_grad[2]:
            db = dy.sum(dim=(0, 1, 2))
        return dx, dw, db, None


def conv_bias_f32(x, conv):
    assert conv.kernel_size == (1, 1) and conv.stride == (1, 1) and x.shape[-1] % 8 == 0
    if torch.is_grad_enabled() and (x.requires_grad or conv.weight.requires_grad):
        return _ConvBiasF32.apply(x, conv.weight, conv.bias, conv)
    pw = packed(conv, need_dgrad=False, split=ops.is_split(x))
    y, _ = ops.conv_fprop(x, pw.wf, pw.cout, ops.conv_taps(1, 1), epi=EPI_F32, shift=conv.bias)
    return y


class _UpsampleCE(torch.autograd.Function):

    @staticmethod
    def forward(ctx, logits, target, ignore_index):
        info, amax, lse = ops.upsample_ce_fwd(logits, target, ignore_index)
        ctx.save_for_backward(logits, target, lse, info)
        ctx.ignore_index = ignore_index
        ctx.mark_non_differentiable(amax)
        return info[0], amax

    @staticmethod
    def backward(ctx, grad_loss, _grad_amax):
        logits, target, lse, info = ctx.saved_tensors
        return ops.upsample_ce_bwd(logits, target, ctx.ignore_index, lse, info, grad_loss), None, None


def fused_tail_supported(criterion, logits, target, zoom_factor, x_size=None):
    if not (type(criterion) is nn.CrossEntropyLoss and criterion.weight is None and criterion.reduction == 'mean'
            and getattr(criterion, 'label_smoothing', 0.0) == 0.0 and zoom_factor == 8 and target is not None
            and target.dtype == torch.int64 and target.dim() == 3):
        return False
    if logits is None:
        return target.shape[1] == x_size[2] and target.shape[2] == x_size[3]
    return (logits.shape[-1] <= 256 and target.shape[1] == 8 * (logits.shape[1] - 1) + 1
            and target.shape[2] == 8 * (logits.shape[2] - 1) + 1)


def upsample_ce(logits, target, ignore_index):
    return _UpsampleCE.apply(logits, target.contiguous(), ignore_index)


class _PPMLink:
    __slots__ = ("dx_identity",)

    def __init__(self):
        self.dx_identity = None


class _PPMPool(torch.autograd.Function):

    @staticmethod
    def forward(ctx, x, bins, link):
        ctx.bins, ctx.shape, ctx.link = bins, tuple(x.shape[-4:]), link
        return tuple(ops.ppm_pool(x, bins))

    @staticmethod
    def backward(ctx, *dpooled):
        n, h, w, c = ctx.shape
        add = None
        if ctx.link is not None:
            add, ctx.link.dx_identity = ctx.link.dx_identity, None
        return ops.ppm_pool_bwd(list(dpooled), ctx.bins, n, h, w, c, add=add), None, None


class _PPMUpsampleConcat(torch.autograd.Function):

    @staticmethod
    def forward(ctx, x, bins, link, *feats):
        ctx.bins, ctx.c, ctx.cr, ctx.link = bins, x.shape[-1], feats[0].shape[-1], link
        return ops.ppm_upsample_concat(x, list(feats), bins)

    @staticmethod
    def backward(ctx, dout):
        if not dout.is_contiguous():
            dout = dout.contiguous()
        dfeats = ops.ppm_upsample_bwd(dout, ctx.c, ctx.bins, ctx.cr)
        dx = dout[..., :ctx.c]
        if ctx.link is not None and ctx.needs_input_grad[0] and all(ctx.needs_input_grad[3:]):
            ctx.link.dx_identity = dx
            dx = None
        return (dx, None, None) + tuple(dfeats)


def ppm_pool(x, bins, link=None):
    return _PPMPool.apply(x, tuple(bins), link)


def ppm_upsample_concat(x, feats, bins, link=None):
    return _PPMUpsampleConcat.apply(x, tuple(bins), link, *feats)


def ppm_link():
    return _PPMLink()


class _PSAAttend(torch.autograd.Function):

    @staticmethod
    def forward(ctx, attn, feat, psa_type, mask_h, mask_w, scale):
        out, stats = ops.psa_attend(attn, feat, psa_type, mask_h, mask_w, scale)
        ctx.save_for_backward(attn, feat, out, stats)
        ctx.cfg = (psa_type, mask_h, mask_w, scale)
        return out

    @staticmethod
    def backward(ctx, dout):
        attn, feat, out, stats = ctx.saved_tensors
        psa_type, mask_h, mask_w, scale = ctx.cfg
        if not dout.is_contiguous():
            dout = dout.contiguous()
        dattn = dfeat = None
        if ctx.needs_input_grad[1]:
            dfeat, _ = ops.psa_attend(attn, dout, psa_type, mask_h, mask_w, scale, stats=stats, mode=1)
        if ctx.needs_input_grad[0]:
            dattn = ops.psa_attend_bwd_attn(attn, stats, feat, out, dout, psa_type, mask_h, mask_w, scale)
        return dattn, dfeat, None, None, None, None


def psa_attend(attn, feat, psa_type, mask_h, mask_w, scale):
    return _PSAAttend.apply(attn.contiguous(), feat, psa_type, mask_h, mask_w, scale)


def psa_attend_supported(feat, mask_h, mask_w):
    return feat.shape[-1] == 512 and feat.shape[-2] <= 128 and mask_h % 2 == 1 and mask_w % 2 == 1


class _ResizeBilinear(torch.autograd.Function):

    @staticmethod
    def forward(ctx, x, size):
        ctx.in_size = tuple(x.shape[-3:-1])
        return ops.resize_bilinear(x, size)

    @staticmethod
    def backward(ctx, dy):
        return ops.resize_bilinear_bwd(dy if dy.is_contiguous() else dy.contiguous(), ctx.in_size), None


def resize_bilinear(x, size):
    return _ResizeBilinear.apply(x, tuple(size))


def to_nhwc_bf16(x_nchw):
    return ops.nchw_to_nhwc_bf16(x_nchw.contiguous().float(), split=precision.split_enabled())


class _ActToF32(torch.autograd.Function):

    @staticmethod
    def forward(ctx, x):
        ctx.split = ops.is_split(x)
        return ops.act_to_f32(x)

    @staticmethod
    def backward(ctx, dy):
        return ops.f32_to_act(dy.contiguous(), ctx.split)


class _F32ToAct(torch.autograd.Function):

    @staticmethod
    def forward(ctx, x, split):
        return ops.f32_to_act(x.contiguous(), split)

    @staticmethod
    def backward(ctx, dy):
        return ops.act_to_f32(dy.contiguous()), None


def act_to_f32(x):
    return _ActToF32.apply(x)


def f32_to_act(x, split):
    return _F32ToAct.apply(x, split)


def to_nchw_f32(y):
    if not (torch.is_grad_enabled() and y.requires_grad):
        return ops.nhwc_bf16_to_nchw(y)
    return act_to_f32(y).permute(0, 3, 1, 2)


class _Fork(torch.autograd.Function):

    @staticmethod
    def forward(ctx, x, k):
        return tuple(x.view_as(x) for _ in range(k))

    @staticmethod
    def backward(ctx, *grads):
        acc = None
        for g in grads:
            if g is None:
                continue
            g = g if g.is_contiguous() else g.contiguous()
            acc = g if acc is None else ops.add_act(acc, g)
        return acc, None


def fork(x, k=2):
    if not (torch.is_grad_enabled() and x.requires_grad):
        return (x,) * k
    return _Fork.apply(x, k)


class _ScaleNC(torch.autograd.Function):
    @staticmethod
    def forward(ctx, x, scale):
        ctx.save_for_backward(scale)
        return ops.scale_nc(x, scale)

    @staticmethod
    def backward(ctx, dy):
        (scale,) = ctx.saved_tensors
        return ops.scale_nc(dy if dy.is_contiguous() else dy.contiguous(), scale), None


def dropout2d_nhwc(x, p, training):
    if not training or p == 0.0:
        return x
    n, c = x.shape[-4], x.shape[-1]
    scale = torch.empty((n, c), device=x.device, dtype=torch.float32).bernoulli_(1.0 - p).mul_(1.0 / (1.0 - p))
    return _ScaleNC.apply(x, scale)


class _MaxPool3x3s2(torch.autograd.Function):
    @staticmethod
    def forward(ctx, x):
        y, code = ops.maxpool3x3s2_fwd(x, want_argcode=True)
        ctx.save_for_backward(code)
        ctx.in_shape = tuple(x.shape[-4:])
        return y

    @staticmethod
    def backward(ctx, dy):
        (code,) = ctx.saved_tensors
        return ops.maxpool3x3s2_bwd(code, dy, ctx.in_shape)


def _pair(v):
    return tuple(v) if isinstance(v, (tuple, list)) else (v, v)


def maxpool_nhwc(x, pool):
    if (_pair(pool.kernel_size) == (3, 3) and _pair(pool.stride) == (2, 2) and _pair(pool.padding) == (1, 1)
            and _pair(pool.dilation) == (1, 1) and not pool.ceil_mode and x.shape[-1] % 8 == 0):
        return _MaxPool3x3s2.apply(x)
    raise NotImplementedError("semseg_b200: only MaxPool2d(kernel_size=3, stride=2, padding=1) (model/resnet.py:115) is "
                              "implemented; there is no library fallback (got %r)" % (pool,))
```

semseg_b200/ops.py:

```python
import ctypes

import torch

from . import _lib
from ._lib import ConvDesc, WgradDesc, EPI_RAW, EPI_AFFINE, EPI_F32, MAX_TAPS


X3_MAX_KBLOCKS = 8

_raw_stream = getattr(torch._C, "_cuda_getCurrentRawStream", None)
_cur_device = getattr(torch._C, "_cuda_getDevice", None)


def _stream():
    if _raw_stream is not None and _cur_device is not None:
        return ctypes.c_void_p(_raw_stream(_cur_device()))
    return ctypes.c_void_p(torch.cuda.current_stream().cuda_stream)


def _ptr(t):
    return ctypes.c_void_p(t.data_ptr()) if t is not None else ctypes.c_void_p(0)


def _require_cuda(*ts):
    for t in ts:
        if t is not None and not t.is_cuda:
            raise _lib.SemsegError("semseg_b200 ops require CUDA tensors (no CPU fallback); got device %s" % t.device)


def is_split(t):
    return t is not None and t.dim() == 5


def _nhwc_meta(t):
    assert t.dtype == torch.bfloat16 and t.dim() in (4, 5), (t.shape, t.dtype)
    if t.dim() == 5:
        assert t.shape[0] == 2, "split activation must be [2,N,H,W,C] (hi, lo planes)"
    n, h, w, c = t.shape[-4:]
    sn, sh, sw, sc = t.stride()[-4:]
    assert sc == 1 and sh == sw * w and sn == sh * h, "NHWC tensor must be pixel-contiguous (stride %s)" % (t.stride(),)
    return n, h, w, c, sw


def _lo(t):
    if t is not None and t.dim() == 5:
        return ctypes.c_void_p(t.data_ptr() + 2 * t.stride(0))
    return ctypes.c_void_p(0)


def _lo_int(t):
    return t.data_ptr() + 2 * t.stride(0) if (t is not None and t.dim() == 5) else 0


def empty_act(shape, split, device):
    return torch.empty(((2,) + tuple(shape)) if split else tuple(shape), dtype=torch.bfloat16, device=device)


def _same_form(*ts):
    forms = {t.dim() == 5 for t in ts if t is not None}
    assert len(forms) <= 1, "activations of one call must all be plain or all be split"


def act_batch_slice(t, a, b):
    return t[:, a:b] if t.dim() == 5 else t[a:b]


def round_up(a, b):
    return (a + b - 1) // b * b


def psamask_fwd(x, psa_type, mask_h, mask_w):
    _require_cuda(x)
    lib = _lib.load()
    assert x.dtype == torch.float32 and x.is_contiguous()
    n, c, h, w = x.shape
    out = torch.empty((n, h * w, h, w), dtype=torch.float32, device=x.device)
    _lib.check(lib.semseg_psamask_fwd(psa_type, _ptr(x), _ptr(out), n, h, w, mask_h, mask_w, _stream()),
               "semseg_psamask_fwd")
    return out


def psamask_bwd(grad_out, psa_type, mask_h, mask_w):
    _require_cuda(grad_out)
    lib = _lib.load()
    assert grad_out.dtype == torch.float32 and grad_out.is_contiguous()
    n, hw, h, w = grad_out.shape
    din = torch.empty((n, mask_h * mask_w, h, w), dtype=torch.float32, device=grad_out.device)
    _lib.check(lib.semseg_psamask_bwd(psa_type, _ptr(grad_out), _ptr(din), n, h, w, mask_h, mask_w, _stream()),
               "semseg_psamask_bwd")
    return din


def psa_attend(attn, feat, psa_type, mask_h, mask_w, scale, stats=None, mode=0):
    _require_cuda(attn, feat)
    lib = _lib.load()
    assert attn.dtype == torch.float32 and attn.dim() == 4 and attn.is_contiguous()
    n, h, w, c, fp = _nhwc_meta(feat)
    assert tuple(attn.shape[:3]) == (n, h, w) and attn.shape[3] >= mask_h * mask_w
    out = empty_act((n, h, w, c), is_split(feat), feat.device)
    if stats is None:
        assert mode == 0
        stats = torch.empty((n, h * w, 2), dtype=torch.float32, device=feat.device)
    _lib.check(lib.semseg_psa_attend(mode, psa_type, _ptr(attn), attn.shape[3], _ptr(feat), _lo(feat), fp, _ptr(stats),
                                     _ptr(out), _lo(out), c, n, h, w, mask_h, mask_w, c, float(scale), _stream()),
               "semseg_psa_attend")
    return out, stats


def psa_attend_bwd_attn(attn, stats, feat, out, dout, psa_type, mask_h, mask_w, scale):
    lib = _lib.load()
    n, h, w, c, fp = _nhwc_meta(feat)
    op, dp = _nhwc_meta(out)[4], _nhwc_meta(dout)[4]
    _same_form(feat, out, dout)
    dattn = torch.empty_like(attn)
    _lib.check(lib.semseg_psa_attend_bwd_attn(psa_type, _ptr(attn), attn.shape[3], _ptr(stats), _ptr(feat), _lo(feat), fp,
                                              _ptr(out), _lo(out), op, _ptr(dout), _lo(dout), dp, _ptr(dattn), n, h, w,
                                              mask_h, mask_w, c, float(scale), _stream()),
               "semseg_psa_attend_bwd_attn")
    return dattn


class PackedWeight:
    __slots__ = ("wf", "wd", "cout", "cin", "taps", "ksize", "split")

    def __init__(self, wf, wd, cout, cin, taps, ksize, split=False):
        self.wf, self.wd, self.cout, self.cin, self.taps, self.ksize, self.split = wf, wd, cout, cin, taps, ksize, split


def _slab(taps, rows, cols, split, device):
    return torch.empty(((2,) if split else ()) + (taps, rows, cols), dtype=torch.bfloat16, device=device)


def pack_weights(w, need_dgrad=True, split=False):
    _require_cuda(w)
    lib = _lib.load()
    w = w.detach()
    assert w.dtype == torch.float32 and w.dim() == 4
    if not w.is_contiguous():
        w = w.contiguous()
    cout, cin, kh, kw = w.shape
    assert kh == kw
    taps = kh * kw
    cin_p, cout_p = round_up(cin, 8), round_up(cout, 8)
    wf = _slab(taps, cout, cin_p, split, w.device)
    wd = _slab(taps, cin, cout_p, split, w.device) if need_dgrad else None
    _lib.check(lib.semseg_pack_weights(_ptr(w), cout, cin, taps, _ptr(wf), cout, cin_p, _ptr(wd),
                                       cin if need_dgrad else 0, cout_p if need_dgrad else 0, int(bool(split)),
                                       _stream()),
               "semseg_pack_weights")
    return PackedWeight(wf, wd, cout, cin, taps, kh, bool(split))


class WeightPackPlan:

    def __init__(self, weights, split=False):
        import ctypes
        _require_cuda(*weights)
        self.split = bool(split)
        self.weights = [w for w in weights]
        self.ptrs = [w.data_ptr() for w in weights]
        self.packs = []
        items = (_lib.PackItem * len(weights))()
        tile0, max_taps = 0, 1
        for k, w in enumerate(weights):
            assert w.dtype == torch.float32 and w.dim() == 4 and w.is_contiguous() and w.shape[2] == w.shape[3]
            cout, cin, kh, _ = w.shape
            taps = kh * kh
            assert taps <= MAX_TAPS
            cin_p, cout_p = round_up(cin, 8), round_up(cout, 8)
            wf = _slab(taps, cout, cin_p, self.split, w.device)
            wd = _slab(taps, cin, cout_p, self.split, w.device)
            self.packs.append(PackedWeight(wf, wd, cout, cin, taps, kh, self.split))
            it = items[k]
            it.w, it.wf, it.wd = w.data_ptr(), wf.data_ptr(), wd.data_ptr()
            it.Cout, it.Cin, it.taps, it.cols_f, it.cols_d = cout, cin, taps, cin_p, cout_p
            it.tile0, it.tiles_ci, it.split = tile0, (cin_p + 31) // 32, int(self.split)
            tile0 += it.tiles_ci * ((cout_p + 31) // 32)
            max_taps = max(max_taps, taps)
        self.n_items, self.n_tiles, self.max_taps = len(weights), tile0, max_taps
        raw = torch.frombuffer(bytearray(bytes(items)), dtype=torch.uint8)
        self.items_dev = raw.to(weights[0].device)

    def valid_for(self, weights, split=False):
        return (bool(split) == self.split and len(weights) == len(self.ptrs) and
                all(w.data_ptr() == p for w, p in zip(weights, self.ptrs)))

    def refresh(self):
        lib = _lib.load()
        _lib.check(lib.semseg_pack_weights_multi(_ptr(self.items_dev), self.n_items, self.n_tiles, self.max_taps,
                                                 _stream()), "semseg_pack_weights_multi")


def conv_taps(ksize, dilation, transpose=False):
    taps = []
    half = ksize // 2
    for r in range(ksize):
        for s in range(ksize):
            dh, dw = (r - half) * dilation, (s - half) * dilation
            if transpose:
                dh, dw = -dh, -dw
            taps.append((dh, dw, r * ksize + s))
    return taps


def _fill_taps(desc, taps, with_wtap=True, img_add=None):
    assert 1 <= len(taps) <= MAX_TAPS
    desc.taps = len(taps)
    for i, t in enumerate(taps):
        desc.dh[i], desc.dw[i] = t[0], t[1]
        if with_wtap:
            desc.wtap[i] = t[2]
        desc.img_add[i] = img_add[i] if img_add is not None else 0
    desc.img_mul = 1


def conv_taps_s2(ksize, n):
    taps = []
    for r in range(ksize):
        for s in range(ksize):
            if ksize == 3:
                ph, dh = (0, 0) if r == 1 else (1, -1 if r == 0 else 0)
                pw, dw = (0, 0) if s == 1 else (1, -1 if s == 0 else 0)
            else:
                ph = pw = dh = dw = 0
            taps.append((dh, dw, r * ksize + s, (ph * 2 + pw) * n, (ph, pw)))
    return taps


def _planes(*ts):
    _same_form(*ts)
    if ts[0].dim() == 5:
        return [tuple(t[0] for t in ts), tuple(t[1] for t in ts)]
    return [tuple(ts)]


def im2col3x3s2(x, cin):
    lib = _lib.load()
    n, h, w, _, p = _nhwc_meta(x)
    out = empty_act((n, (h - 1) // 2 + 1, (w - 1) // 2 + 1, 32), is_split(x), x.device)
    for xi, oi in _planes(x, out):
        _lib.check(lib.semseg_im2col3x3s2(_ptr(xi), p, n, h, w, int(cin), _ptr(oi), _stream()), "semseg_im2col3x3s2")
    return out


def space_to_phases(x):
    _require_cuda(x)
    lib = _lib.load()
    n, h, w, c, p = _nhwc_meta(x)
    xp = empty_act((4 * n, (h + 1) // 2, (w + 1) // 2, c), is_split(x), x.device)
    for xi, oi in _planes(x, xp):
        _lib.check(lib.semseg_space_to_phases(_ptr(xi), p, n, h, w, c, _ptr(oi), _stream()), "semseg_space_to_phases")
    return xp


def phases_to_space(xp, n, h, w):
    lib = _lib.load()
    c = xp.shape[-1]
    assert xp.is_contiguous() and xp.shape[-4] == 4 * n
    x = empty_act((n, h, w, c), is_split(xp), xp.device)
    for xi, oi in _planes(xp, x):
        _lib.check(lib.semseg_phases_to_space(_ptr(xi), n, h, w, c, _ptr(oi), _stream()), "semseg_phases_to_space")
    return x


def conv_stats_rows(n, h, w, cout):
    return int(_lib.load().semseg_conv_stats_rows(n, h, w, cout))


def conv_fprop(x, w3d, cout, taps, *, out=None, epi=EPI_RAW, relu=False, scale=None, shift=None, residual=None,
               stats=False, out_f32=None, img_add=None, out_nhw=None):
    _require_cuda(x, w3d)
    lib = _lib.load()
    nin, hin, win, cin, xp = _nhwc_meta(x)
    split = is_split(x)
    n, h, w = out_nhw if out_nhw is not None else (nin, hin, win)
    d = ConvDesc()
    d.N, d.H, d.W, d.Cin, d.Cout = n, h, w, cin, cout
    d.x, d.Nin, d.Hin, d.Win, d.x_pitch = x.data_ptr(), nin, hin, win, xp
    d.x_lo = _lo_int(x)
    assert w3d.dtype == torch.bfloat16 and w3d.is_contiguous() and w3d.dim() == (4 if split else 3), \
        "packed weights must be [taps][rows][cols] (plain) or [2][taps][rows][cols] (split, hi then lo slab)"
    d.w, d.n_wtaps, d.w_rows, d.w_cols = w3d.data_ptr(), w3d.shape[-3], w3d.shape[-2], w3d.shape[-1]
    d.w_split = int(split)
    _fill_taps(d, taps, img_add=img_add)
    d.epi_mode, d.relu = epi, int(bool(relu))
    sp = None
    if epi == EPI_F32:
        if out_f32 is None:
            out_f32 = torch.empty((n, h, w, cout), dtype=torch.float32, device=x.device)
        assert out_f32.dtype == torch.float32 and out_f32.stride(-1) == 1
        d.out_f32, d.out_pitch = out_f32.data_ptr(), out_f32.stride(2)
        y = out_f32
    else:
        if out is None:
            out = empty_act((n, h, w, cout), split, x.device)
        on, oh, ow, oc, op = _nhwc_meta(out)
        assert (on, oh, ow, oc) == (n, h, w, cout) and is_split(out) == split
        d.y, d.y_pitch, d.y_lo = out.data_ptr(), op, _lo_int(out)
        y = out
    if scale is not None:
        assert scale.dtype == torch.float32 and scale.numel() >= cout
        d.scale = scale.data_ptr()
    if shift is not None:
        assert shift.dtype == torch.float32 and shift.numel() >= cout
        d.shift = shift.data_ptr()
    if residual is not None:
        rn, rh, rw, rc, rp = _nhwc_meta(residual)
        assert (rn, rh, rw, rc) == (n, h, w, cout) and is_split(residual) == split
        d.residual, d.res_pitch, d.residual_lo = residual.data_ptr(), rp, _lo_int(residual)
    k_slices = int(lib.semseg_conv_k_slices(cin, len(taps), X3_MAX_KBLOCKS)) if (split and epi != EPI_F32) else 1
    if k_slices > 1:
        part = torch.empty((k_slices, n, h, w, cout), dtype=torch.float32, device=x.device)
        d.epi_mode, d.relu = EPI_F32, 0
        d.out_f32, d.out_pitch = part.data_ptr(), cout
        d.k_slices, d.slice_stride = k_slices, part.stride(0)
        sc, sh, rs, rsl, rpitch, ylo = d.scale, d.shift, d.residual, d.residual_lo, d.res_pitch, d.y_lo
        d.scale = d.shift = d.residual = d.residual_lo = d.y_lo = None
        _lib.check(lib.semseg_conv_fprop(ctypes.byref(d), _stream()), "semseg_conv_fprop (K-sliced)")
        m = n * h * w
        if stats:
            assert epi == EPI_RAW
            sp = torch.empty((int(lib.semseg_conv_splitk_rows(m)), 3, cout), dtype=torch.float32, device=x.device)
        _lib.check(lib.semseg_conv_splitk_finish(_ptr(part), k_slices, part.stride(0), cout, m, cout, epi,
                                                 int(bool(relu)), sc, sh, rs, rsl, rpitch, d.y, ylo, d.y_pitch,
                                                 _ptr(sp), _stream()), "semseg_conv_splitk_finish")
        return y, sp
    if stats:
        assert epi == EPI_RAW
        sp = torch.empty((conv_stats_rows(n, h, w, cout), 3, cout), dtype=torch.float32, device=x.device)
        d.stats_partial = sp.data_ptr()
    _lib.check(lib.semseg_conv_fprop(ctypes.byref(d), _stream()), "semseg_conv_fprop")
    return y, sp


def conv_wgrad(x, dy, cin, cout, taps, grad_out=None, accumulate=False, img_add=None):
    _require_cuda(x, dy)
    lib = _lib.load()
    nin, hin, win, xc, xp = _nhwc_meta(x)
    n, h, w, dc, dp = _nhwc_meta(dy)
    assert xc >= cin and dc >= cout
    assert img_add is not None or (nin, hin, win) == (n, h, w)
    _same_form(x, dy)
    d = WgradDesc()
    d.N, d.H, d.W, d.Cin, d.Cout = n, h, w, cin, cout
    d.x, d.Nin, d.Hin, d.Win, d.x_pitch = x.data_ptr(), nin, hin, win, xp
    d.dy, d.dy_pitch = dy.data_ptr(), dp
    d.x_lo, d.dy_lo = _lo_int(x), _lo_int(dy)
    _fill_taps(d, taps, with_wtap=False, img_add=img_add)
    d.n_splits = 0
    splits = lib.semseg_conv_wgrad_splits(ctypes.byref(d))
    if splits <= 0:
        raise _lib.SemsegError("semseg_conv_wgrad_splits failed (%d)" % splits)
    ntaps = len(taps)
    part = torch.empty((splits, ntaps, cout, cin), dtype=torch.float32, device=x.device)
    d.dw_partial = part.data_ptr()
    d.n_splits = splits
    _lib.check(lib.semseg_conv_wgrad(ctypes.byref(d), _stream()), "semseg_conv_wgrad")
    k = int(round(ntaps ** 0.5))
    if grad_out is None:
        grad_out = torch.empty((cout, cin, k, k), dtype=torch.float32, device=x.device)
        accumulate = False
    assert grad_out.is_contiguous() and grad_out.dtype == torch.float32
    _lib.check(lib.semseg_wgrad_reduce(_ptr(part), splits, ntaps, cout, cin, _ptr(grad_out), int(accumulate),
                                       _stream()), "semseg_wgrad_reduce")
    return grad_out


def nchw_to_nhwc_bf16(x, pad_to=8, split=False):
    _require_cuda(x)
    lib = _lib.load()
    assert x.dtype == torch.float32 and x.is_contiguous()
    n, c, h, w = x.shape
    cp = round_up(c, pad_to)
    shape = ((2,) if split else ()) + (n, h, w, cp)
    out = (torch.zeros if cp != c else torch.empty)(shape, dtype=torch.bfloat16, device=x.device)
    _lib.check(lib.semseg_nchw_f32_to_nhwc_bf16(_ptr(x), _ptr(out), _lo(out), n, c, h, w, cp, _stream()),
               "semseg_nchw_f32_to_nhwc_bf16")
    return out


def nhwc_bf16_to_nchw(x):
    _require_cuda(x)
    lib = _lib.load()
    n, h, w, c, p = _nhwc_meta(x)
    out = torch.empty((n, c, h, w), dtype=torch.float32, device=x.device)
    _lib.check(lib.semseg_nhwc_bf16_to_nchw_f32(_ptr(x), _lo(x), _ptr(out), n, c, h, w, p, _stream()),
               "semseg_nhwc_bf16_to_nchw_f32")
    return out


def nhwc_f32_to_nchw(x):
    _require_cuda(x)
    lib = _lib.load()
    assert x.dtype == torch.float32 and x.dim() == 4 and x.stride(-1) == 1
    n, h, w, c = x.shape
    out = torch.empty((n, c, h, w), dtype=torch.float32, device=x.device)
    _lib.check(lib.semseg_nhwc_f32_to_nchw_f32(_ptr(x), _ptr(out), n, c, h, w, x.stride(2), _stream()),
               "semseg_nhwc_f32_to_nchw_f32")
    return out


def bn_workspace(m, c, device):
    nf = int(_lib.load().semseg_bn_workspace_floats(m, c))
    return torch.empty((nf,), dtype=torch.float32, device=device), nf


def bn_merge_partials(stats_partial):
    lib = _lib.load()
    t, _, c = stats_partial.shape
    out = torch.empty((3, c), dtype=torch.float32, device=stats_partial.device)
    _lib.check(lib.semseg_bn_merge_partials(_ptr(stats_partial), t, c, _ptr(out), _stream()),
               "semseg_bn_merge_partials")
    return out


def bn_stats(x):
    _require_cuda(x)
    lib = _lib.load()
    n, h, w, c, p = _nhwc_meta(x)
    m = n * h * w
    ws, nf = bn_workspace(m, c, x.device)
    out = torch.empty((3, c), dtype=torch.float32, device=x.device)
    _lib.check(lib.semseg_bn_stats(_ptr(x), m, c, p, _ptr(ws), nf, _ptr(out), _stream()), "semseg_bn_stats")
    return out


def bn_finalize(rank_stats, gamma, beta, eps, momentum, running_mean, running_var):
    lib = _lib.load()
    if rank_stats.dim() == 2:
        rank_stats = rank_stats.unsqueeze(0)
    r, _, c = rank_stats.shape
    assert rank_stats.is_contiguous()
    mi = torch.empty((3, c), dtype=torch.float32, device=rank_stats.device)
    ss = torch.empty((2, c), dtype=torch.float32, device=rank_stats.device)
    _lib.check(lib.semseg_bn_finalize(_ptr(rank_stats), r, c, _ptr(gamma), _ptr(beta), float(eps), float(momentum),
                                      _ptr(running_mean), _ptr(running_var), _ptr(mi), _ptr(ss), _stream()),
               "semseg_bn_finalize")
    return mi, ss


def bn_finalize_partials(stats_partial, gamma, beta, eps, momentum, running_mean, running_var):
    lib = _lib.load()
    t, _, c = stats_partial.shape
    buf = torch.empty((5, c), dtype=torch.float32, device=stats_partial.device)
    mi, ss = buf[:3], buf[3:]
    _lib.check(lib.semseg_bn_finalize_partials(_ptr(stats_partial), t, c, _ptr(gamma), _ptr(beta),
                                               float(eps), float(momentum), _ptr(running_mean), _ptr(running_var),
                                               _ptr(mi), _ptr(ss), _stream()), "semseg_bn_finalize_partials")
    return mi, ss


def bn_fold_eval(gamma, beta, running_mean, running_var, eps):
    lib = _lib.load()
    c = running_mean.numel()
    ss = torch.empty((2, c), dtype=torch.float32, device=running_mean.device)
    _lib.check(lib.semseg_bn_fold_eval(_ptr(gamma), _ptr(beta), _ptr(running_mean), _ptr(running_var), float(eps), c,
                                       _ptr(ss), _stream()), "semseg_bn_fold_eval")
    return ss


def bn_apply(x, scale_shift, residual=None, relu=True, out=None):
    _require_cuda(x)
    lib = _lib.load()
    n, h, w, c, xp = _nhwc_meta(x)
    if out is None:
        out = empty_act((n, h, w, c), is_split(x), x.device)
    _, _, _, oc, op = _nhwc_meta(out)
    assert oc == c
    rp = 0
    if residual is not None:
        _, _, _, rc, rp = _nhwc_meta(residual)
        assert rc == c
    _same_form(x, out, residual)
    _lib.check(lib.semseg_bn_apply(_ptr(x), _lo(x), xp, _ptr(scale_shift), _ptr(residual), _lo(residual), rp,
                                   _ptr(out), _lo(out), op, n * h * w, c, int(bool(relu)), _stream()),
               "semseg_bn_apply")
    return out


def bn_bwd_reduce(dy, y, x, mean_invstd, relu, scale_shift=None):
    lib = _lib.load()
    n, h, w, c, dp = _nhwc_meta(dy)
    _, _, _, _, xp = _nhwc_meta(x)
    yp = _nhwc_meta(y)[4] if y is not None else 0
    m = n * h * w
    ws, nf = bn_workspace(m, c, dy.device)
    sums = torch.empty((2, c), dtype=torch.float32, device=dy.device)
    _same_form(dy, y, x)
    _lib.check(lib.semseg_bn_bwd_reduce(_ptr(dy), _lo(dy), dp, _ptr(y), _lo(y), yp, _ptr(x), _lo(x), xp,
                                        _ptr(mean_invstd), _ptr(scale_shift), m, c, int(bool(relu)), _ptr(ws), nf,
                                        _ptr(sums), _stream()),
               "semseg_bn_bwd_reduce")
    return sums


def bn_bwd_apply(dy, y, x, mean_invstd, gamma, sums, count, relu, want_dres=False, scale_shift=None):
    lib = _lib.load()
    n, h, w, c, dp = _nhwc_meta(dy)
    _, _, _, _, xp = _nhwc_meta(x)
    yp = _nhwc_meta(y)[4] if y is not None else 0
    _same_form(dy, y, x)
    split = is_split(dy)
    dx = empty_act((n, h, w, c), split, dy.device)
    dres = empty_act((n, h, w, c), split, dy.device) if want_dres else None
    dgb = torch.empty((2, c), dtype=torch.float32, device=dy.device)
    _lib.check(lib.semseg_bn_bwd_apply(_ptr(dy), _lo(dy), dp, _ptr(y), _lo(y), yp, _ptr(x), _lo(x), xp,
                                       _ptr(mean_invstd), _ptr(gamma), _ptr(scale_shift), _ptr(sums), float(count),
                                       n * h * w, c, int(bool(relu)), _ptr(dx), _lo(dx), c, _ptr(dres), _lo(dres), c,
                                       _ptr(dgb), _stream()), "semseg_bn_bwd_apply")
    return dx, dres, dgb


def add_act(a, b, out=None):
    lib = _lib.load()
    n, h, w, c, ap = _nhwc_meta(a)
    bp = _nhwc_meta(b)[4]
    if out is None:
        out = empty_act((n, h, w, c), is_split(a), a.device)
    op = _nhwc_meta(out)[4]
    _same_form(a, b, out)
    _lib.check(lib.semseg_add_act(_ptr(a), _lo(a), ap, _ptr(b), _lo(b), bp, _ptr(out), _lo(out), op, n * h * w, c,
                                  _stream()), "semseg_add_act")
    return out


def scale_nc(x, scale):
    lib = _lib.load()
    n, h, w, c, xp = _nhwc_meta(x)
    assert scale.dtype == torch.float32 and scale.is_contiguous() and scale.numel() == n * c
    out = empty_act((n, h, w, c), is_split(x), x.device)
    _lib.check(lib.semseg_scale_nc(_ptr(x), _lo(x), xp, _ptr(scale), _ptr(out), _lo(out), c, n, h * w, c, _stream()),
               "semseg_scale_nc")
    return out


def f32_to_act(x, split, pad_to=8):
    _require_cuda(x)
    lib = _lib.load()
    assert x.dtype == torch.float32 and x.dim() == 4 and x.stride(-1) == 1
    n, h, w, c = x.shape
    sn, sh, sw, _ = x.stride()
    assert sh == sw * w and sn == sh * h
    cp = round_up(c, pad_to)
    out = empty_act((n, h, w, cp), split, x.device)
    _lib.check(lib.semseg_f32_to_act(_ptr(x), sw, _ptr(out), _lo(out), cp, n * h * w, c, cp, _stream()),
               "semseg_f32_to_act")
    return out


def act_to_f32(x):
    lib = _lib.load()
    n, h, w, c, p = _nhwc_meta(x)
    out = torch.empty((n, h, w, c), dtype=torch.float32, device=x.device)
    _lib.check(lib.semseg_act_to_f32(_ptr(x), _lo(x), p, _ptr(out), c, n * h * w, c, _stream()), "semseg_act_to_f32")
    return out


def upsample_ce_fwd(logits, target, ignore_index, want_argmax=True):
    _require_cuda(logits, target)
    lib = _lib.load()
    assert logits.dtype == torch.float32 and logits.dim() == 4 and logits.stride(-1) == 1
    assert target.dtype == torch.int64 and target.is_contiguous()
    n, h, w, c = logits.shape
    _, ho, wo = target.shape
    nws = int(lib.semseg_upsample_ce_workspace_floats(n, ho, wo))
    ws = torch.empty((nws,), dtype=torch.float32, device=logits.device)
    info = torch.empty((2,), dtype=torch.float32, device=logits.device)
    amax = torch.empty((n, ho, wo), dtype=torch.int64, device=logits.device) if want_argmax else None
    lse = torch.empty((n, ho, wo), dtype=torch.float32, device=logits.device)
    _lib.check(lib.semseg_upsample_ce_fwd(_ptr(logits), logits.stride(2), n, h, w, c, _ptr(target), ho, wo,
                                          int(ignore_index), _ptr(ws), _ptr(info), _ptr(amax), _ptr(lse), _stream()),
               "semseg_upsample_ce_fwd")
    return info, amax, lse


def upsample_ce_bwd(logits, target, ignore_index, lse, info, grad_out):
    lib = _lib.load()
    n, h, w, c = logits.shape
    _, ho, wo = target.shape
    dl = torch.empty((n, h, w, c), dtype=torch.float32, device=logits.device)
    ws = torch.empty((int(lib.semseg_upsample_ce_bwd_workspace_floats(n, ho, w, c)),), dtype=torch.float32,
                     device=logits.device)
    g = grad_out.reshape(1).float().contiguous()
    _lib.check(lib.semseg_upsample_ce_bwd(_ptr(logits), logits.stride(2), n, h, w, c, _ptr(target), ho, wo,
                                          int(ignore_index), _ptr(lse), _ptr(info), _ptr(g), _ptr(ws), _ptr(dl),
                                          _stream()),
               "semseg_upsample_ce_bwd")
    return dl


def _bin_args(bins, tensors):
    nb = len(bins)
    barr = (ctypes.c_int * nb)(*bins)
    parr = (ctypes.c_void_p * nb)(*[t.data_ptr() for t in tensors])
    larr = (ctypes.c_void_p * nb)(*[_lo_int(t) for t in tensors]) if is_split(tensors[0]) else None
    return barr, parr, larr, nb


def ppm_pool(x, bins):
    _require_cuda(x)
    lib = _lib.load()
    n, h, w, c, p = _nhwc_meta(x)
    outs = [empty_act((n, b, b, c), is_split(x), x.device) for b in bins]
    barr, parr, larr, nb = _bin_args(bins, outs)
    _lib.check(lib.semseg_ppm_pool(_ptr(x), _lo(x), p, n, h, w, c, barr, parr, larr, nb, _stream()), "semseg_ppm_pool")
    return outs


def ppm_pool_bwd(dpooled, bins, n, h, w, c, add=None):
    lib = _lib.load()
    dpooled = [d.contiguous() for d in dpooled]
    dx = empty_act((n, h, w, c), is_split(dpooled[0]), dpooled[0].device)
    barr, parr, larr, nb = _bin_args(bins, dpooled)
    ap = _nhwc_meta(add)[4] if add is not None else 0
    _same_form(dx, add)
    _lib.check(lib.semseg_ppm_pool_bwd(parr, larr, barr, nb, n, h, w, c, _ptr(dx), _lo(dx), c, _ptr(add), _lo(add), ap,
                                       _stream()), "semseg_ppm_pool_bwd")
    return dx


def ppm_upsample_concat(x, feats, bins):
    lib = _lib.load()
    n, h, w, c, p = _nhwc_meta(x)
    feats = [f.contiguous() for f in feats]
    cr = feats[0].shape[-1]
    out = empty_act((n, h, w, c + len(bins) * cr), is_split(x), x.device)
    barr, parr, larr, nb = _bin_args(bins, feats)
    _same_form(x, feats[0])
    _lib.check(lib.semseg_ppm_upsample_concat(_ptr(x), _lo(x), p, parr, larr, barr, nb, n, h, w, c, cr, _ptr(out),
                                              _lo(out), out.shape[-1], _stream()), "semseg_ppm_upsample_concat")
    return out


def ppm_upsample_bwd(dout, c_off, bins, cr):
    lib = _lib.load()
    n, h, w, ct, p = _nhwc_meta(dout)
    dfeats = [empty_act((n, b, b, cr), is_split(dout), dout.device) for b in bins]
    barr, parr, larr, nb = _bin_args(bins, dfeats)
    _lib.check(lib.semseg_ppm_upsample_bwd(_ptr(dout), _lo(dout), p, c_off, parr, larr, barr, nb, n, h, w, cr,
                                           _stream()), "semseg_ppm_upsample_bwd")
    return dfeats


def resize_bilinear(x, size):
    _require_cuda(x)
    lib = _lib.load()
    n, hi, wi, c, p = _nhwc_meta(x)
    ho, wo = int(size[0]), int(size[1])
    y = empty_act((n, ho, wo, c), is_split(x), x.device)
    _lib.check(lib.semseg_resize_bilinear_fwd(_ptr(x), _lo(x), p, n, hi, wi, c, ho, wo, _ptr(y), _lo(y), c, _stream()),
               "semseg_resize_bilinear_fwd")
    return y


def resize_bilinear_bwd(dy, in_size):
    lib = _lib.load()
    n, ho, wo, c, p = _nhwc_meta(dy)
    hi, wi = int(in_size[0]), int(in_size[1])
    dx = empty_act((n, hi, wi, c), is_split(dy), dy.device)
    _lib.check(lib.semseg_resize_bilinear_bwd(_ptr(dy), _lo(dy), p, n, hi, wi, c, ho, wo, _ptr(dx), _lo(dx), c, _stream()),
               "semseg_resize_bilinear_bwd")
    return dx


def maxpool3x3s2_fwd(x, want_argcode=True):
    _require_cuda(x)
    lib = _lib.load()
    n, h, w, c, p = _nhwc_meta(x)
    assert p == c, "maxpool expects a dense NHWC tensor"
    shape = (n, (h - 1) // 2 + 1, (w - 1) // 2 + 1, c)
    y = empty_act(shape, is_split(x), x.device)
    code = torch.empty(shape, dtype=torch.uint8, device=x.device) if want_argcode else None
    _lib.check(lib.semseg_maxpool3x3s2_fwd(_ptr(x), _lo(x), _ptr(y), _lo(y), _ptr(code), n, h, w, c, _stream()),
               "semseg_maxpool3x3s2_fwd")
    return y, code


def maxpool3x3s2_bwd(argcode, dy, in_shape):
    lib = _lib.load()
    n, h, w, c = in_shape
    dy = dy.contiguous()
    dx = empty_act((n, h, w, c), is_split(dy), dy.device)
    _lib.check(lib.semseg_maxpool3x3s2_bwd(_ptr(argcode), _ptr(dy), _lo(dy), _ptr(dx), _lo(dx), n, h, w, c,
                                           _stream()), "semseg_maxpool3x3s2_bwd")
    return dx


def bn_finalize_p2p(stats_partial, gamma, beta, eps, momentum, running_mean, running_var, px):
    lib = _lib.load()
    t, _, c = stats_partial.shape
    buf = torch.empty((5, c), dtype=torch.float32, device=stats_partial.device)
    mi, ss = buf[:3], buf[3:]
    slot, seq = px.next()
    _lib.check(lib.semseg_bn_finalize_p2p(_ptr(stats_partial), t, c, _ptr(gamma), _ptr(beta), float(eps),
                                          float(momentum), _ptr(running_mean), _ptr(running_var), _ptr(mi), _ptr(ss),
                                          px.data_ptrs, px.flag_ptrs, _ptr(px.counter), px.world, px.rank, slot,
                                          int(__import__("semseg_b200.p2p", fromlist=["x"]).SLOT_FLOATS), seq,
                                          _ptr(px.step), _stream()), "semseg_bn_finalize_p2p")
    return mi, ss


def bn_bwd_reduce_p2p(dy, y, x, mean_invstd, relu, scale_shift, px):
    lib = _lib.load()
    n, h, w, c, dp = _nhwc_meta(dy)
    _, _, _, _, xp = _nhwc_meta(x)
    yp = _nhwc_meta(y)[4] if y is not None else 0
    m = n * h * w
    ws, nf = bn_workspace(m, c, dy.device)
    out = torch.empty((2, 2, c), dtype=torch.float32, device=dy.device)
    slot, seq = px.next()
    _same_form(dy, y, x)
    _lib.check(lib.semseg_bn_bwd_reduce_p2p(_ptr(dy), _lo(dy), dp, _ptr(y), _lo(y), yp, _ptr(x), _lo(x), xp,
                                            _ptr(mean_invstd),
                                            _ptr(scale_shift), m, c, int(bool(relu)), _ptr(ws), nf, _ptr(out[0]),
                                            _ptr(out[1]), px.data_ptrs, px.flag_ptrs, _ptr(px.counter), px.world,
                                            px.rank, slot,
                                            int(__import__("semseg_b200.p2p", fromlist=["x"]).SLOT_FLOATS), seq,
                                            _ptr(px.step), _stream()), "semseg_bn_bwd_reduce_p2p")
    return out[0], out[1]
```

Before: 520.4.

## Store ReLU sign bitmask in BN apply and use it in backward instead of y

BN apply now optionally writes a 1-bit-per-channel ReLU mask for conv+BN+residual+ReLU blocks. The backward reduce and apply kernels read this mask instead of reloading the full bf16 output y, and the output no longer has to be kept alive for backward. The reduce kernel is also templated on the mask source, loops over multiple chunks per block with double-buffered shared memory, and gains launch bounds. The cost is an extra mask allocation and write in the forward pass, plus more kernel variants to compile.

```diff
diff --git a/include/semseg_b200.h b/include/semseg_b200.h
--- a/include/semseg_b200.h
+++ b/include/semseg_b200.h
@@ -138,7 +138,8 @@
                            int world, int rank, int slot, int slot_floats, unsigned seq, const void* seq_ptr,
                            void* stream);
 int semseg_bn_bwd_reduce_p2p(const void* dy, const void* dy_lo, int dy_pitch, const void* y, const void* y_lo,
-                             int y_pitch, const void* x, const void* x_lo, int x_pitch, const float* mean_invstd,
+                             int y_pitch, const unsigned char* relu_mask, const void* x, const void* x_lo, int x_pitch,
+                             const float* mean_invstd,
                              const float* scale_shift, int M, int C, int relu, float* workspace,
                              long long workspace_floats, float* sums_local, float* sums_total,
                              void* const* peer_bufs, void* const* peer_flags, void* counter, int world, int rank,
@@ -146,14 +147,16 @@
 int semseg_bn_fold_eval(const float* gamma, const float* beta, const float* running_mean,
                         const float* running_var, float eps, int C, float* scale_shift, void* stream);
 int semseg_bn_apply(const void* x, const void* x_lo, int x_pitch, const float* scale_shift, const void* residual,
-                    const void* residual_lo, int res_pitch, void* y, void* y_lo, int y_pitch, int M, int C, int relu,
-                    void* stream);
+                    const void* residual_lo, int res_pitch, void* y, void* y_lo, int y_pitch, unsigned char* relu_mask,
+                    int M, int C, int relu, void* stream);
 int semseg_bn_bwd_reduce(const void* dy, const void* dy_lo, int dy_pitch, const void* y, const void* y_lo, int y_pitch,
-                         const void* x, const void* x_lo, int x_pitch, const float* mean_invstd,
+                         const unsigned char* relu_mask, const void* x, const void* x_lo, int x_pitch,
+                         const float* mean_invstd,
                          const float* scale_shift, int M, int C, int relu, float* workspace,
                          long long workspace_floats, float* sums, void* stream);
 int semseg_bn_bwd_apply(const void* dy, const void* dy_lo, int dy_pitch, const void* y, const void* y_lo, int y_pitch,
-                        const void* x, const void* x_lo, int x_pitch, const float* mean_invstd, const float* gamma,
+                        const unsigned char* relu_mask, const void* x, const void* x_lo, int x_pitch,
+                        const float* mean_invstd, const float* gamma,
                         const float* scale_shift, const float* sums, float count, int M, int C, int relu, void* dx,
                         void* dx_lo, int dx_pitch, void* dres, void* dres_lo, int dres_pitch, float* dgamma_dbeta,
                         void* stream);
diff --git a/semseg_b200/_lib.py b/semseg_b200/_lib.py
--- a/semseg_b200/_lib.py
+++ b/semseg_b200/_lib.py
@@ -111,16 +111,16 @@
     "semseg_bn_finalize_partials": (c_int, [c_vp, c_int, c_int, c_vp, c_vp, c_f, c_f, c_vp, c_vp, c_vp, c_vp, c_vp]),
     "semseg_bn_finalize_p2p": (c_int, [c_vp, c_int, c_int, c_vp, c_vp, c_f, c_f, c_vp, c_vp, c_vp, c_vp, c_vp, c_vp,
                                        c_vp, c_int, c_int, c_int, c_int, ctypes.c_uint, c_vp, c_vp]),
-    "semseg_bn_bwd_reduce_p2p": (c_int, [c_vp, c_vp, c_int, c_vp, c_vp, c_int, c_vp, c_vp, c_int, c_vp, c_vp, c_int,
+    "semseg_bn_bwd_reduce_p2p": (c_int, [c_vp, c_vp, c_int, c_vp, c_vp, c_int, c_vp, c_vp, c_vp, c_int, c_vp, c_vp, c_int,
                                          c_int, c_int, c_vp, c_ll, c_vp, c_vp, c_vp, c_vp, c_vp, c_int, c_int, c_int,
                                          c_int, ctypes.c_uint, c_vp, c_vp]),
     "semseg_bn_fold_eval": (c_int, [c_vp, c_vp, c_vp, c_vp, c_f, c_int, c_vp, c_vp]),
-    "semseg_bn_apply": (c_int, [c_vp, c_vp, c_int, c_vp, c_vp, c_vp, c_int, c_vp, c_vp, c_int, c_int, c_int, c_int,
-                                c_vp]),
-    "semseg_bn_bwd_reduce": (c_int, [c_vp, c_vp, c_int, c_vp, c_vp, c_int, c_vp, c_vp, c_int, c_vp, c_vp, c_int, c_int,
-                                     c_int, c_vp, c_ll, c_vp, c_vp]),
-    "semseg_bn_bwd_apply": (c_int, [c_vp, c_vp, c_int, c_vp, c_vp, c_int, c_vp, c_vp, c_int, c_vp, c_vp, c_vp, c_vp,
-                                    c_f, c_int, c_int, c_int, c_vp, c_vp, c_int, c_vp, c_vp, c_int, c_vp, c_vp]),
+    "semseg_bn_apply": (c_int, [c_vp, c_vp, c_int, c_vp, c_vp, c_vp, c_int, c_vp, c_vp, c_int, c_vp, c_int, c_int,
+                                c_int, c_vp]),
+    "semseg_bn_bwd_reduce": (c_int, [c_vp, c_vp, c_int, c_vp, c_vp, c_int, c_vp, c_vp, c_vp, c_int, c_vp, c_vp, c_int,
+                                     c_int, c_int, c_vp, c_ll, c_vp, c_vp]),
+    "semseg_bn_bwd_apply": (c_int, [c_vp, c_vp, c_int, c_vp, c_vp, c_int, c_vp, c_vp, c_vp, c_int, c_vp, c_vp, c_vp,
+                                    c_vp, c_f, c_int, c_int, c_int, c_vp, c_vp, c_int, c_vp, c_vp, c_int, c_vp, c_vp]),
     "semseg_add_act": (c_int, [c_vp, c_vp, c_int, c_vp, c_vp, c_int, c_vp, c_vp, c_int, c_int, c_int, c_vp]),
     "semseg_scale_nc": (c_int, [c_vp, c_vp, c_int, c_vp, c_vp, c_vp, c_int, c_int, c_int, c_int, c_vp]),
     "semseg_f32_to_act": (c_int, [c_vp, c_int, c_vp, c_vp, c_int, c_ll, c_int, c_int, c_vp]),
diff --git a/semseg_b200/csrc/act.cuh b/semseg_b200/csrc/act.cuh
--- a/semseg_b200/csrc/act.cuh
+++ b/semseg_b200/csrc/act.cuh
@@ -64,6 +64,28 @@
     *reinterpret_cast<uint4*>(lo + off) = act_pack8(r);
   }
 }
+template <bool S>
+__device__ __forceinline__ unsigned act_st8_pos(bf16_t* hi, bf16_t* lo, long long off, const float (&f)[8]) {
+  const uint4 h = act_pack8(f);
+  *reinterpret_cast<uint4*>(hi + off) = h;
+  float v[8];
+  act_unpack8(h, v);
+  if constexpr (S) {
+    float r[8], g[8];
+#pragma unroll
+    for (int q = 0; q < 8; ++q) r[q] = f[q] - v[q];
+    const uint4 l = act_pack8(r);
+    *reinterpret_cast<uint4*>(lo + off) = l;
+    act_unpack8(l, g);
+#pragma unroll
+    for (int q = 0; q < 8; ++q) v[q] += g[q];
+  }
+  unsigned m = 0;
+#pragma unroll
+  for (int q = 0; q < 8; ++q) m |= (v[q] > 0.f ? 1u : 0u) << q;
+  return m;
+}
+
 __device__ __forceinline__ void act_split1(float v, bf16_t& hi, bf16_t& lo) {
   hi = __float2bfloat16_rn(v);
   lo = __float2bfloat16_rn(v - __bfloat162float(hi));
diff --git a/semseg_b200/csrc/bn.cu b/semseg_b200/csrc/bn.cu
--- a/semseg_b200/csrc/bn.cu
+++ b/semseg_b200/csrc/bn.cu
@@ -281,7 +281,8 @@
 __global__ void bn_apply_kernel(const __nv_bfloat16* __restrict__ x, const __nv_bfloat16* __restrict__ x_lo, int x_pitch,
                                 const float* __restrict__ ss, const __nv_bfloat16* __restrict__ res,
                                 const __nv_bfloat16* __restrict__ res_lo, int res_pitch, __nv_bfloat16* __restrict__ y,
-                                __nv_bfloat16* __restrict__ y_lo, int y_pitch, long long M, int C, int relu) {
+                                __nv_bfloat16* __restrict__ y_lo, int y_pitch, uint8_t* __restrict__ mask, long long M,
+                                int C, int relu) {
   const int groups = C >> 3;
   long long idx = static_cast<long long>(blockIdx.x) * blockDim.x + threadIdx.x;
   const long long stride = static_cast<long long>(gridDim.x) * blockDim.x;
@@ -314,7 +315,11 @@
         if (relu) v = fmaxf(v, 0.f);
         f[q] = v;
       }
-      act_st8<S>(y, y_lo, (p + u * pstride) * y_pitch + c0, f);
+      const long long pp = p + u * pstride;
+      if (mask)
+        mask[pp * groups + (c0 >> 3)] = static_cast<uint8_t>(act_st8_pos<S>(y, y_lo, pp * y_pitch + c0, f));
+      else
+        act_st8<S>(y, y_lo, pp * y_pitch + c0, f);
     }
   }
   for (; p < M; p += pstride) {
@@ -327,97 +332,112 @@
       if (relu) v = fmaxf(v, 0.f);
       f[q] = v;
     }
-    act_st8<S>(y, y_lo, p * y_pitch + c0, f);
-  }
-}
-
-template <bool S>
-__global__ void bn_bwd_reduce_kernel(const __nv_bfloat16* __restrict__ dy, const __nv_bfloat16* __restrict__ dy_lo,
-                                     int dy_pitch, const __nv_bfloat16* __restrict__ y,
-                                     const __nv_bfloat16* __restrict__ y_lo, int y_pitch,
-                                     const __nv_bfloat16* __restrict__ x, const __nv_bfloat16* __restrict__ x_lo,
-                                     int x_pitch, const float* __restrict__ mean_invstd, const float* __restrict__ ss,
-                                     int M, int C, int relu, int rows_per_chunk, float* __restrict__ part) {
-  __shared__ float s_a[32][65];
-  __shared__ float s_b[32][65];
+    if (mask)
+      mask[p * groups + (c0 >> 3)] = static_cast<uint8_t>(act_st8_pos<S>(y, y_lo, p * y_pitch + c0, f));
+    else
+      act_st8<S>(y, y_lo, p * y_pitch + c0, f);
+  }
+}
+
+enum MaskSrc {
+  kMaskNone = 0,
+  kMaskBits = 1,
+  kMaskY = 2,
+  kMaskRaw = 3,
+};
+
+template <int MS>
+__device__ __forceinline__ void apply_relu_mask(float (&d)[8], const float (&xv)[8], const float (&yv)[8], unsigned bits,
+                                                const float (&msc)[8], const float (&msh)[8]) {
+#pragma unroll
+  for (int q = 0; q < 8; ++q) {
+    bool keep = true;
+    if constexpr (MS == kMaskBits) keep = (bits >> q) & 1u;
+    if constexpr (MS == kMaskY) keep = yv[q] > 0.f;
+    if constexpr (MS == kMaskRaw) keep = fmaf(xv[q], msc[q], msh[q]) > 0.f;
+    if (!keep) d[q] = 0.f;
+  }
+}
+
+template <bool S, int MS>
+__global__ void __launch_bounds__(256, S ? 2 : 3) bn_bwd_reduce_kernel(
+    const __nv_bfloat16* __restrict__ dy, const __nv_bfloat16* __restrict__ dy_lo, int dy_pitch,
+    const __nv_bfloat16* __restrict__ y, const __nv_bfloat16* __restrict__ y_lo, int y_pitch,
+    const uint8_t* __restrict__ mask, const __nv_bfloat16* __restrict__ x, const __nv_bfloat16* __restrict__ x_lo,
+    int x_pitch, const float* __restrict__ mean_invstd, const float* __restrict__ ss, int M, int C, int rows_per_chunk,
+    int chunks, float* __restrict__ part) {
+  __shared__ float s_ab[2][2][32][65];
   const int gl = threadIdx.x & 7;
   const int pl = threadIdx.x >> 3;
   const int c0 = blockIdx.x * 64 + gl * 8;
-  const int chunk = blockIdx.y;
-  const int r0 = chunk * rows_per_chunk;
-  const int r1 = min(M, r0 + rows_per_chunk);
+  const int groups = C >> 3;
   const bool active = c0 < C;
-  float a[8] = {0, 0, 0, 0, 0, 0, 0, 0}, b[8] = {0, 0, 0, 0, 0, 0, 0, 0};
-  if (active) {
-    float mean[8], invstd[8], msc[8], msh[8];
+  float mean[8], invstd[8], msc[8], msh[8];
+#pragma unroll
+  for (int q = 0; q < 8; ++q) {
+    mean[q] = active ? mean_invstd[c0 + q] : 0.f;
+    invstd[q] = active ? mean_invstd[C + c0 + q] : 0.f;
+    msc[q] = (MS == kMaskRaw && active) ? ss[c0 + q] : 0.f;
+    msh[q] = (MS == kMaskRaw && active) ? ss[C + c0 + q] : 0.f;
+  }
+  int buf = 0;
+  for (int chunk = blockIdx.y; chunk < chunks; chunk += gridDim.y, buf ^= 1) {
+    const int r0 = chunk * rows_per_chunk;
+    const int r1 = min(M, r0 + rows_per_chunk);
+    float a[8] = {0, 0, 0, 0, 0, 0, 0, 0}, b[8] = {0, 0, 0, 0, 0, 0, 0, 0};
+    if (active) {
+      auto accumulate = [&](float (&d)[8], const float (&xv)[8], const float (&yv)[8], unsigned bits) {
+        apply_relu_mask<MS>(d, xv, yv, bits, msc, msh);
+#pragma unroll
+        for (int q = 0; q < 8; ++q) {
+          a[q] += d[q];
+          b[q] = fmaf(d[q], (xv[q] - mean[q]) * invstd[q], b[q]);
+        }
+      };
+      constexpr int U = S ? 2 : 4;
+      int r = r0 + pl;
+      for (; r + (U - 1) * 32 < r1; r += U * 32) {
+        Raw8<S> dv[U], xr[U], yr[U];
+        unsigned mb[U];
+#pragma unroll
+        for (int u = 0; u < U; ++u) {
+          dv[u] = act_ldraw<S>(dy, dy_lo, static_cast<long long>(r + u * 32) * dy_pitch + c0);
+          xr[u] = act_ldraw<S>(x, x_lo, static_cast<long long>(r + u * 32) * x_pitch + c0);
+          if constexpr (MS == kMaskY) yr[u] = act_ldraw<S>(y, y_lo, static_cast<long long>(r + u * 32) * y_pitch + c0);
+          mb[u] = MS == kMaskBits ? mask[static_cast<long long>(r + u * 32) * groups + (c0 >> 3)] : 0u;
+        }
+#pragma unroll
+        for (int u = 0; u < U; ++u) {
+          float d[8], xv[8], yv[8] = {0, 0, 0, 0, 0, 0, 0, 0};
+          act_unpack<S>(dv[u], d);
+          act_unpack<S>(xr[u], xv);
+          if constexpr (MS == kMaskY) act_unpack<S>(yr[u], yv);
+          accumulate(d, xv, yv, mb[u]);
+        }
+      }
+      for (; r < r1; r += 32) {
+        float d[8], xv[8], yv[8] = {0, 0, 0, 0, 0, 0, 0, 0};
+        act_ld8<S>(dy, dy_lo, static_cast<long long>(r) * dy_pitch + c0, d);
+        act_ld8<S>(x, x_lo, static_cast<long long>(r) * x_pitch + c0, xv);
+        if constexpr (MS == kMaskY) act_ld8<S>(y, y_lo, static_cast<long long>(r) * y_pitch + c0, yv);
+        const unsigned bits = MS == kMaskBits ? mask[static_cast<long long>(r) * groups + (c0 >> 3)] : 0u;
+        accumulate(d, xv, yv, bits);
+      }
+    }
 #pragma unroll
     for (int q = 0; q < 8; ++q) {
-      mean[q] = mean_invstd[c0 + q];
-      invstd[q] = mean_invstd[C + c0 + q];
-      msc[q] = ss ? ss[c0 + q] : 0.f;
-      msh[q] = ss ? ss[C + c0 + q] : 0.f;
-    }
-    const bool mask_from_y = relu && y != nullptr;
-    const bool mask_from_x = relu && y == nullptr;
-    constexpr int U = S ? 2 : 4;
-    auto accumulate = [&](float (&d)[8], const float (&xv)[8], const float (&yv)[8]) {
-      if (mask_from_y) {
-#pragma unroll
-        for (int q = 0; q < 8; ++q)
-          if (!(yv[q] > 0.f)) d[q] = 0.f;
-      } else if (mask_from_x) {
-#pragma unroll
-        for (int q = 0; q < 8; ++q)
-          if (!(fmaf(xv[q], msc[q], msh[q]) > 0.f)) d[q] = 0.f;
-      }
-#pragma unroll
-      for (int q = 0; q < 8; ++q) {
-        a[q] += d[q];
-        b[q] = fmaf(d[q], (xv[q] - mean[q]) * invstd[q], b[q]);
-      }
-    };
-    int r = r0 + pl;
-    for (; r + (U - 1) * 32 < r1; r += U * 32) {
-      Raw8<S> dv[U], xr[U], yr[U];
-#pragma unroll
-      for (int u = 0; u < U; ++u) {
-        dv[u] = act_ldraw<S>(dy, dy_lo, static_cast<long long>(r + u * 32) * dy_pitch + c0);
-        xr[u] = act_ldraw<S>(x, x_lo, static_cast<long long>(r + u * 32) * x_pitch + c0);
-      }
-      if (mask_from_y) {
-#pragma unroll
-        for (int u = 0; u < U; ++u) yr[u] = act_ldraw<S>(y, y_lo, static_cast<long long>(r + u * 32) * y_pitch + c0);
-      }
-#pragma unroll
-      for (int u = 0; u < U; ++u) {
-        float d[8], xv[8], yv[8] = {0, 0, 0, 0, 0, 0, 0, 0};
-        act_unpack<S>(dv[u], d);
-        act_unpack<S>(xr[u], xv);
-        if (mask_from_y) act_unpack<S>(yr[u], yv);
-        accumulate(d, xv, yv);
-      }
-    }
-    for (; r < r1; r += 32) {
-      float d[8], xv[8], yv[8] = {0, 0, 0, 0, 0, 0, 0, 0};
-      act_ld8<S>(dy, dy_lo, static_cast<long long>(r) * dy_pitch + c0, d);
-      act_ld8<S>(x, x_lo, static_cast<long long>(r) * x_pitch + c0, xv);
-      if (mask_from_y) act_ld8<S>(y, y_lo, static_cast<long long>(r) * y_pitch + c0, yv);
-      accumulate(d, xv, yv);
-    }
-  }
-#pragma unroll
-  for (int q = 0; q < 8; ++q) {
-    s_a[pl][gl * 8 + q] = a[q];
-    s_b[pl][gl * 8 + q] = b[q];
-  }
-  __syncthreads();
-  if (pl < 2 && active) {
-    float(*src)[65] = pl == 0 ? s_a : s_b;
-#pragma unroll
-    for (int q = 0; q < 8; ++q) {
-      float t = 0.f;
-      for (int i = 0; i < 32; ++i) t += src[i][gl * 8 + q];
-      if (c0 + q < C) part[(static_cast<size_t>(chunk) * 2 + pl) * C + c0 + q] = t;
+      s_ab[buf][0][pl][gl * 8 + q] = a[q];
+      s_ab[buf][1][pl][gl * 8 + q] = b[q];
+    }
+    __syncthreads();
+    if (threadIdx.x < 128) {
+      const int which = threadIdx.x >> 6, cl = threadIdx.x & 63;
+      const int c = blockIdx.x * 64 + cl;
+      if (c < C) {
+        float t = 0.f;
+        for (int i = 0; i < 32; ++i) t += s_ab[buf][which][i][cl];
+        part[(static_cast<size_t>(chunk) * 2 + which) * C + c] = t;
+      }
     }
   }
 }
@@ -452,17 +472,15 @@
   }
 }
 
-template <bool S>
-__global__ void bn_bwd_apply_kernel(const __nv_bfloat16* __restrict__ dy, const __nv_bfloat16* __restrict__ dy_lo,
-                                    int dy_pitch, const __nv_bfloat16* __restrict__ y,
-                                    const __nv_bfloat16* __restrict__ y_lo, int y_pitch,
-                                    const __nv_bfloat16* __restrict__ x, const __nv_bfloat16* __restrict__ x_lo,
-                                    int x_pitch, const float* __restrict__ mean_invstd, const float* __restrict__ gamma,
-                                    const float* __restrict__ ss, const float* __restrict__ sums, float inv_count,
-                                    long long M, int C, int relu, __nv_bfloat16* __restrict__ dx,
-                                    __nv_bfloat16* __restrict__ dx_lo, int dx_pitch, __nv_bfloat16* __restrict__ dres,
-                                    __nv_bfloat16* __restrict__ dres_lo, int dres_pitch,
-                                    float* __restrict__ dgamma_dbeta) {
+template <bool S, int MS>
+__global__ void __launch_bounds__(256, 2) bn_bwd_apply_kernel(
+    const __nv_bfloat16* __restrict__ dy, const __nv_bfloat16* __restrict__ dy_lo, int dy_pitch,
+    const __nv_bfloat16* __restrict__ y, const __nv_bfloat16* __restrict__ y_lo, int y_pitch,
+    const uint8_t* __restrict__ mask, const __nv_bfloat16* __restrict__ x, const __nv_bfloat16* __restrict__ x_lo,
+    int x_pitch, const float* __restrict__ mean_invstd, const float* __restrict__ gamma, const float* __restrict__ ss,
+    const float* __restrict__ sums, float inv_count, long long M, int C, __nv_bfloat16* __restrict__ dx,
+    __nv_bfloat16* __restrict__ dx_lo, int dx_pitch, __nv_bfloat16* __restrict__ dres,
+    __nv_bfloat16* __restrict__ dres_lo, int dres_pitch, float* __restrict__ dgamma_dbeta) {
   const int groups = C >> 3;
   if (dgamma_dbeta && blockIdx.x == 0) {
     for (int c = threadIdx.x; c < C; c += blockDim.x) {
@@ -474,13 +492,11 @@
   const long long stride = static_cast<long long>(gridDim.x) * blockDim.x;
   const int c0 = static_cast<int>(idx % groups) << 3;
   float ka[8], kx[8], kb[8], msc[8], msh[8];
-  const bool mask_from_y = relu && y != nullptr;
-  const bool mask_from_x = relu && y == nullptr;
 #pragma unroll
   for (int q = 0; q < 8; ++q) {
     const int c = c0 + q;
-    msc[q] = ss ? ss[c] : 0.f;
-    msh[q] = ss ? ss[C + c] : 0.f;
+    msc[q] = MS == kMaskRaw ? ss[c] : 0.f;
+    msh[q] = MS == kMaskRaw ? ss[C + c] : 0.f;
     const float mean = mean_invstd[c], invstd = mean_invstd[C + c];
     const float g = gamma ? gamma[c] : 1.f;
     ka[q] = g * invstd;
@@ -488,16 +504,8 @@
     kx[q] = -ka[q] * invstd * sums[C + c] * ic;
     kb[q] = -ka[q] * sums[c] * ic - kx[q] * mean;
   }
-  auto finish = [&](float (&d)[8], const float (&xv)[8], const float (&yv)[8], long long pp) {
-    if (mask_from_y) {
-#pragma unroll
-      for (int q = 0; q < 8; ++q)
-        if (!(yv[q] > 0.f)) d[q] = 0.f;
-    } else if (mask_from_x) {
-#pragma unroll
-      for (int q = 0; q < 8; ++q)
-        if (!(fmaf(xv[q], msc[q], msh[q]) > 0.f)) d[q] = 0.f;
-    }
+  auto finish = [&](float (&d)[8], const float (&xv)[8], const float (&yv)[8], unsigned bits, long long pp) {
+    apply_relu_mask<MS>(d, xv, yv, bits, msc, msh);
     if (dres) act_st8<S>(dres, dres_lo, pp * dres_pitch + c0, d);
     float o[8];
 #pragma unroll
@@ -506,33 +514,33 @@
   };
   const long long pstride = stride / groups;
   long long p = idx / groups;
-  constexpr int U = 2;
+  constexpr int U = S ? 2 : 4;
   for (; p + (U - 1) * pstride < M; p += U * pstride) {
     Raw8<S> dv[U], xr[U], yr[U];
+    unsigned mb[U];
 #pragma unroll
     for (int u = 0; u < U; ++u) {
       dv[u] = act_ldraw<S>(dy, dy_lo, (p + u * pstride) * dy_pitch + c0);
       xr[u] = act_ldraw<S>(x, x_lo, (p + u * pstride) * x_pitch + c0);
-    }
-    if (mask_from_y) {
-#pragma unroll
-      for (int u = 0; u < U; ++u) yr[u] = act_ldraw<S>(y, y_lo, (p + u * pstride) * y_pitch + c0);
+      if constexpr (MS == kMaskY) yr[u] = act_ldraw<S>(y, y_lo, (p + u * pstride) * y_pitch + c0);
+      mb[u] = MS == kMaskBits ? mask[(p + u * pstride) * groups + (c0 >> 3)] : 0u;
     }
 #pragma unroll
     for (int u = 0; u < U; ++u) {
       float d[8], xv[8], yv[8] = {0, 0, 0, 0, 0, 0, 0, 0};
       act_unpack<S>(dv[u], d);
       act_unpack<S>(xr[u], xv);
-      if (mask_from_y) act_unpack<S>(yr[u], yv);
-      finish(d, xv, yv, p + u * pstride);
+      if constexpr (MS == kMaskY) act_unpack<S>(yr[u], yv);
+      finish(d, xv, yv, mb[u], p + u * pstride);
     }
   }
   for (; p < M; p += pstride) {
     float d[8], xv[8], yv[8] = {0, 0, 0, 0, 0, 0, 0, 0};
     act_ld8<S>(dy, dy_lo, p * dy_pitch + c0, d);
     act_ld8<S>(x, x_lo, p * x_pitch + c0, xv);
-    if (mask_from_y) act_ld8<S>(y, y_lo, p * y_pitch + c0, yv);
-    finish(d, xv, yv, p);
+    if constexpr (MS == kMaskY) act_ld8<S>(y, y_lo, p * y_pitch + c0, yv);
+    const unsigned bits = MS == kMaskBits ? mask[p * groups + (c0 >> 3)] : 0u;
+    finish(d, xv, yv, bits, p);
   }
 }
 
@@ -898,7 +906,7 @@
 
 extern "C" int semseg_bn_apply(const void* x, const void* x_lo, int x_pitch, const float* scale_shift,
                                const void* residual, const void* residual_lo, int res_pitch, void* y, void* y_lo,
-                               int y_pitch, int M, int C, int relu, void* stream_) {
+                               int y_pitch, unsigned char* relu_mask, int M, int C, int relu, void* stream_) {
   cudaStream_t stream = static_cast<cudaStream_t>(stream_);
   SB_CHECK_ARG(x && scale_shift && y && M > 0 && C > 0, "bn_apply: bad args");
   SB_CHECK_ARG(C % 8 == 0 && x_pitch % 8 == 0 && y_pitch % 8 == 0 && (!residual || res_pitch % 8 == 0),
@@ -911,41 +919,61 @@
   SB_ACT_DISPATCH(split, bn_apply_kernel<kS><<<grid, 256, 0, stream>>>(
                              static_cast<const bf16*>(x), static_cast<const bf16*>(x_lo), x_pitch, scale_shift,
                              static_cast<const bf16*>(residual), static_cast<const bf16*>(residual_lo), res_pitch,
-                             static_cast<bf16*>(y), static_cast<bf16*>(y_lo), y_pitch, M, C, relu));
-  SB_LAUNCHED();
-  return SEMSEG_OK;
-}
+                             static_cast<bf16*>(y), static_cast<bf16*>(y_lo), y_pitch, relu_mask, M, C, relu));
+  SB_LAUNCHED();
+  return SEMSEG_OK;
+}
+
+static int mask_source(int relu, const void* relu_mask, const void* y) {
+  return !relu ? kMaskNone : relu_mask ? kMaskBits : y ? kMaskY : kMaskRaw;
+}
+
+#define SB_MASK_DISPATCH(ms, ...)                                   \
+  do {                                                              \
+    switch (ms) {                                                   \
+      case kMaskNone: { constexpr int kM = kMaskNone; __VA_ARGS__; } break; \
+      case kMaskBits: { constexpr int kM = kMaskBits; __VA_ARGS__; } break; \
+      case kMaskY: { constexpr int kM = kMaskY; __VA_ARGS__; } break;       \
+      default: { constexpr int kM = kMaskRaw; __VA_ARGS__; } break;         \
+    }                                                               \
+  } while (0)
 
 static int launch_bwd_reduce(const void* dy, const void* dy_lo, int dy_pitch, const void* y, const void* y_lo,
-                             int y_pitch, const void* x, const void* x_lo, int x_pitch, const float* mean_invstd,
-                             const float* scale_shift, int M, int C, int relu, float* workspace, cudaStream_t stream) {
+                             int y_pitch, const unsigned char* relu_mask, const void* x, const void* x_lo, int x_pitch,
+                             const float* mean_invstd, const float* scale_shift, int M, int C, int relu,
+                             float* workspace, cudaStream_t stream) {
   const bool split = dy_lo != nullptr;
-  SB_CHECK_ARG((x_lo != nullptr) == split && (!(relu && y) || (y_lo != nullptr) == split),
+  const int ms = mask_source(relu, relu_mask, y);
+  SB_CHECK_ARG((x_lo != nullptr) == split && (ms != kMaskY || (y_lo != nullptr) == split),
                "bn_bwd_reduce: all tensors must use the same storage form (plain or split)");
   const int rows = chunk_rows(M);
   const int chunks = cdiv(M, rows);
-  dim3 grid(cdiv(C, 64), chunks);
-  SB_ACT_DISPATCH(split, bn_bwd_reduce_kernel<kS><<<grid, 256, 0, stream>>>(
+  const int gx = cdiv(C, 64);
+  const int per_col = num_sms() * (split ? 2 : 3) / gx;
+  const int per_block = cdiv(chunks, per_col > 0 ? per_col : 1);
+  dim3 grid(gx, cdiv(chunks, per_block));
+  SB_ACT_DISPATCH(split, SB_MASK_DISPATCH(ms, bn_bwd_reduce_kernel<kS, kM><<<grid, 256, 0, stream>>>(
                              static_cast<const bf16*>(dy), static_cast<const bf16*>(dy_lo), dy_pitch,
-                             static_cast<const bf16*>(y), static_cast<const bf16*>(y_lo), y_pitch,
+                             static_cast<const bf16*>(y), static_cast<const bf16*>(y_lo), y_pitch, relu_mask,
                              static_cast<const bf16*>(x), static_cast<const bf16*>(x_lo), x_pitch, mean_invstd,
-                             scale_shift, M, C, relu, rows, workspace));
+                             scale_shift, M, C, rows, chunks, workspace)));
   SB_LAUNCHED();
   return SEMSEG_OK;
 }
 
 extern "C" int semseg_bn_bwd_reduce(const void* dy, const void* dy_lo, int dy_pitch, const void* y, const void* y_lo,
-                                    int y_pitch, const void* x, const void* x_lo, int x_pitch,
+                                    int y_pitch, const unsigned char* relu_mask, const void* x, const void* x_lo,
+                                    int x_pitch,
                                     const float* mean_invstd, const float* scale_shift, int M, int C, int relu,
                                     float* workspace, long long workspace_floats, float* sums, void* stream_) {
   cudaStream_t stream = static_cast<cudaStream_t>(stream_);
   SB_CHECK_ARG(dy && x && mean_invstd && workspace && sums && M > 0 && C > 0, "bn_bwd_reduce: bad args");
-  SB_CHECK_ARG(!relu || y || scale_shift, "bn_bwd_reduce: relu needs y or scale_shift");
+  SB_CHECK_ARG(!relu || relu_mask || y || scale_shift, "bn_bwd_reduce: relu needs relu_mask, y or scale_shift");
   SB_CHECK_ARG(C % 8 == 0 && dy_pitch % 8 == 0 && x_pitch % 8 == 0 && (!(relu && y) || y_pitch % 8 == 0),
                "bn_bwd_reduce: channels and pitches must be multiples of 8");
   SB_CHECK_ARG(workspace_floats >= semseg_bn_workspace_floats(M, C), "bn_bwd_reduce: workspace too small");
-  int r = launch_bwd_reduce(dy, dy_lo, dy_pitch, y, y_lo, y_pitch, x, x_lo, x_pitch, mean_invstd, scale_shift, M, C,
-                            relu, workspace, stream);
+  int r = launch_bwd_reduce(dy, dy_lo, dy_pitch, y, y_lo, y_pitch, relu_mask, x, x_lo, x_pitch, mean_invstd,
+                            scale_shift, M, C, relu, workspace, stream);
   if (r) return r;
   bn_bwd_reduce_final_kernel<<<cdiv(2 * C, 32), 1024, 0, stream>>>(workspace, cdiv(M, chunk_rows(M)), C, sums);
   SB_LAUNCHED();
@@ -953,30 +981,32 @@
 }
 
 extern "C" int semseg_bn_bwd_apply(const void* dy, const void* dy_lo, int dy_pitch, const void* y, const void* y_lo,
-                                   int y_pitch, const void* x, const void* x_lo, int x_pitch,
+                                   int y_pitch, const unsigned char* relu_mask, const void* x, const void* x_lo,
+                                   int x_pitch,
                                    const float* mean_invstd, const float* gamma, const float* scale_shift,
                                    const float* sums, float count, int M, int C, int relu, void* dx, void* dx_lo,
                                    int dx_pitch, void* dres, void* dres_lo, int dres_pitch, float* dgamma_dbeta,
                                    void* stream_) {
   cudaStream_t stream = static_cast<cudaStream_t>(stream_);
   SB_CHECK_ARG(dy && x && mean_invstd && sums && dx && M > 0 && C > 0, "bn_bwd_apply: bad args");
-  SB_CHECK_ARG(!relu || y || scale_shift, "bn_bwd_apply: relu needs y or scale_shift");
+  SB_CHECK_ARG(!relu || relu_mask || y || scale_shift, "bn_bwd_apply: relu needs relu_mask, y or scale_shift");
   SB_CHECK_ARG(C % 8 == 0 && dy_pitch % 8 == 0 && x_pitch % 8 == 0 && dx_pitch % 8 == 0 &&
                    (!(relu && y) || y_pitch % 8 == 0) && (!dres || dres_pitch % 8 == 0),
                "bn_bwd_apply: channels and pitches must be multiples of 8");
   const bool split = dy_lo != nullptr;
+  const int ms = mask_source(relu, relu_mask, y);
   SB_CHECK_ARG((x_lo != nullptr) == split && (dx_lo != nullptr) == split &&
-                   (!(relu && y) || (y_lo != nullptr) == split) && (!dres || (dres_lo != nullptr) == split),
+                   (ms != kMaskY || (y_lo != nullptr) == split) && (!dres || (dres_lo != nullptr) == split),
                "bn_bwd_apply: all tensors must use the same storage form (plain or split)");
   const long long total = static_cast<long long>(M) * (C / 8);
   const int grid = ew_grid_fixed_channels(total, 256, C / 8);
-  SB_ACT_DISPATCH(split, bn_bwd_apply_kernel<kS><<<grid, 256, 0, stream>>>(
+  SB_ACT_DISPATCH(split, SB_MASK_DISPATCH(ms, bn_bwd_apply_kernel<kS, kM><<<grid, 256, 0, stream>>>(
                              static_cast<const bf16*>(dy), static_cast<const bf16*>(dy_lo), dy_pitch,
-                             static_cast<const bf16*>(y), static_cast<const bf16*>(y_lo), y_pitch,
+                             static_cast<const bf16*>(y), static_cast<const bf16*>(y_lo), y_pitch, relu_mask,
                              static_cast<const bf16*>(x), static_cast<const bf16*>(x_lo), x_pitch, mean_invstd, gamma,
-                             scale_shift, sums, count > 0.f ? 1.f / count : 0.f, M, C, relu, static_cast<bf16*>(dx),
+                             scale_shift, sums, count > 0.f ? 1.f / count : 0.f, M, C, static_cast<bf16*>(dx),
                              static_cast<bf16*>(dx_lo), dx_pitch, static_cast<bf16*>(dres),
-                             static_cast<bf16*>(dres_lo), dres_pitch, dgamma_dbeta));
+                             static_cast<bf16*>(dres_lo), dres_pitch, dgamma_dbeta)));
   SB_LAUNCHED();
   return SEMSEG_OK;
 }
@@ -1123,7 +1153,8 @@
 }
 
 extern "C" int semseg_bn_bwd_reduce_p2p(const void* dy, const void* dy_lo, int dy_pitch, const void* y,
-                                        const void* y_lo, int y_pitch, const void* x, const void* x_lo, int x_pitch,
+                                        const void* y_lo, int y_pitch, const unsigned char* relu_mask, const void* x,
+                                        const void* x_lo, int x_pitch,
                                         const float* mean_invstd, const float* scale_shift, int M, int C, int relu,
                                         float* workspace, long long workspace_floats, float* sums_local,
                                         float* sums_total, void* const* peer_bufs, void* const* peer_flags,
@@ -1132,15 +1163,15 @@
   cudaStream_t stream = static_cast<cudaStream_t>(stream_);
   SB_CHECK_ARG(dy && x && mean_invstd && workspace && sums_local && sums_total && M > 0 && C > 0,
                "bn_bwd_reduce_p2p: bad args");
-  SB_CHECK_ARG(!relu || y || scale_shift, "bn_bwd_reduce_p2p: relu needs y or scale_shift");
+  SB_CHECK_ARG(!relu || relu_mask || y || scale_shift, "bn_bwd_reduce_p2p: relu needs relu_mask, y or scale_shift");
   SB_CHECK_ARG(C % 8 == 0 && dy_pitch % 8 == 0 && x_pitch % 8 == 0 && (!(relu && y) || y_pitch % 8 == 0),
                "bn_bwd_reduce_p2p: channels and pitches must be multiples of 8");
   SB_CHECK_ARG(workspace_floats >= semseg_bn_workspace_floats(M, C), "bn_bwd_reduce_p2p: workspace too small");
   sb::PeerArgs pa;
   int r = fill_peer_args(&pa, peer_bufs, peer_flags, counter, world, rank, slot, slot_floats, seq, seq_ptr, 2 * C);
   if (r) return r;
-  r = launch_bwd_reduce(dy, dy_lo, dy_pitch, y, y_lo, y_pitch, x, x_lo, x_pitch, mean_invstd, scale_shift, M, C, relu,
-                        workspace, stream);
+  r = launch_bwd_reduce(dy, dy_lo, dy_pitch, y, y_lo, y_pitch, relu_mask, x, x_lo, x_pitch, mean_invstd, scale_shift,
+                        M, C, relu, workspace, stream);
   if (r) return r;
   bn_bwd_reduce_final_p2p_kernel<<<cdiv(2 * C, 32), 1024, 0, stream>>>(workspace, cdiv(M, chunk_rows(M)), C,
                                                                       sums_local, sums_total, pa);
diff --git a/semseg_b200/functional.py b/semseg_b200/functional.py
--- a/semseg_b200/functional.py
+++ b/semseg_b200/functional.py
@@ -98,28 +98,28 @@
     return mi, ss, world
 
 
-def _bn_backward(ctx_pg, world, dy, y, raw, mi, gamma, relu, want_dres, ss=None):
+def _bn_backward(ctx_pg, world, dy, mask, raw, mi, gamma, relu, want_dres, ss=None):
     n, h, w, c = raw.shape[-4:]
     if not dy.is_contiguous():
         dy = dy.contiguous()
     px = p2p.get_exchange(ctx_pg) if ctx_pg is not None else None
     if px is not None and 2 * c <= p2p.SLOT_FLOATS:
-        local, sums = ops.bn_bwd_reduce_p2p(dy, y if relu else None, raw, mi, relu, ss if y is None else None, px)
+        local, sums = ops.bn_bwd_reduce_p2p(dy, None, raw, mi, relu, ss if mask is None else None, px, mask=mask)
         dbeta, dgamma = local[0], local[1]
     else:
-        sums = ops.bn_bwd_reduce(dy, y if relu else None, raw, mi, relu, scale_shift=ss if y is None else None)
+        sums = ops.bn_bwd_reduce(dy, None, raw, mi, relu, scale_shift=ss if mask is None else None, mask=mask)
         dbeta, dgamma = sums[0], sums[1]
         if ctx_pg is not None:
             dbeta, dgamma = dbeta.clone(), dgamma.clone()
             dist.all_reduce(sums, group=ctx_pg)
     count = float(n * h * w) if world == 1 else 0.0
-    d_raw, dres, _ = ops.bn_bwd_apply(dy, y if relu else None, raw, mi, gamma, sums, count, relu, want_dres=want_dres,
-                                      scale_shift=ss if y is None else None)
+    d_raw, dres, _ = ops.bn_bwd_apply(dy, None, raw, mi, gamma, sums, count, relu, want_dres=want_dres,
+                                      scale_shift=ss if mask is None else None, mask=mask)
     return d_raw, dres, dgamma, dbeta
 
 
 class _CbaState:
-    __slots__ = ("xin", "raw", "y", "mi", "gamma", "ss", "pw", "k", "dil", "stride", "relu", "pg", "world",
+    __slots__ = ("xin", "raw", "mask", "mi", "gamma", "ss", "pw", "k", "dil", "stride", "relu", "pg", "world",
                  "in_shape", "has_res")
 
 
@@ -156,11 +156,12 @@
         mi, ss, world = _finalize_stats(ops.bn_merge_partials(sp), bn, pg, count_batches=False)
     if track and bn.num_batches_tracked is not None:
         bn.num_batches_tracked.add_(1)
-    y = ops.bn_apply(raw, ss, residual=residual, relu=relu, out=out)
+    n_out, h_out, w_out = raw.shape[-4:-1]
+    mask = ops.empty_relu_mask((n_out, h_out, w_out, pw.cout), raw.device) if (relu and residual is not None) else None
+    y = ops.bn_apply(raw, ss, residual=residual, relu=relu, out=out, mask=mask)
     st = _CbaState()
-    need_y = relu and residual is not None
-    st.xin, st.raw, st.y, st.mi, st.gamma = xin, raw, (y if need_y else None), mi, bn.weight
-    st.ss = ss if (relu and not need_y) else None
+    st.xin, st.raw, st.mask, st.mi, st.gamma = xin, raw, mask, mi, bn.weight
+    st.ss = ss if (relu and mask is None) else None
     st.pw, st.k, st.dil, st.stride, st.relu, st.pg, st.world = pw, k, dil, stride, relu, pg, world
     st.in_shape, st.has_res = (n, h, w, cx), residual is not None
     return y, st
@@ -169,7 +170,7 @@
 def cba_backward(st, dy, need_dx=True, need_dw=True, need_dres=False, dx_add=None):
     pw = st.pw
     n, h, w, cx = st.in_shape
-    d_raw, dres, dgamma, dbeta = _bn_backward(st.pg, st.world, dy, st.y, st.raw, st.mi, st.gamma, st.relu,
+    d_raw, dres, dgamma, dbeta = _bn_backward(st.pg, st.world, dy, st.mask, st.raw, st.mi, st.gamma, st.relu,
                                               st.has_res and need_dres, st.ss)
     dx = dw = None
     if st.stride == 0:
diff --git a/semseg_b200/ops.py b/semseg_b200/ops.py
--- a/semseg_b200/ops.py
+++ b/semseg_b200/ops.py
@@ -459,7 +459,20 @@
     return ss
 
 
-def bn_apply(x, scale_shift, residual=None, relu=True, out=None):
+def empty_relu_mask(shape, device):
+    n, h, w, c = shape
+    assert c % 8 == 0
+    return torch.empty((n * h * w, c // 8), dtype=torch.uint8, device=device)
+
+
+def _mask_ptr(mask, m, c):
+    if mask is None:
+        return ctypes.c_void_p(0)
+    assert mask.dtype == torch.uint8 and mask.is_contiguous() and mask.shape == (m, c // 8), (mask.shape, mask.dtype)
+    return _ptr(mask)
+
+
+def bn_apply(x, scale_shift, residual=None, relu=True, out=None, mask=None):
     _require_cuda(x)
     lib = _lib.load()
     n, h, w, c, xp = _nhwc_meta(x)
@@ -473,12 +486,13 @@
         assert rc == c
     _same_form(x, out, residual)
     _lib.check(lib.semseg_bn_apply(_ptr(x), _lo(x), xp, _ptr(scale_shift), _ptr(residual), _lo(residual), rp,
-                                   _ptr(out), _lo(out), op, n * h * w, c, int(bool(relu)), _stream()),
+                                   _ptr(out), _lo(out), op, _mask_ptr(mask, n * h * w, c), n * h * w, c,
+                                   int(bool(relu)), _stream()),
                "semseg_bn_apply")
     return out
 
 
-def bn_bwd_reduce(dy, y, x, mean_invstd, relu, scale_shift=None):
+def bn_bwd_reduce(dy, y, x, mean_invstd, relu, scale_shift=None, mask=None):
     lib = _lib.load()
     n, h, w, c, dp = _nhwc_meta(dy)
     _, _, _, _, xp = _nhwc_meta(x)
@@ -487,14 +501,15 @@
     ws, nf = bn_workspace(m, c, dy.device)
     sums = torch.empty((2, c), dtype=torch.float32, device=dy.device)
     _same_form(dy, y, x)
-    _lib.check(lib.semseg_bn_bwd_reduce(_ptr(dy), _lo(dy), dp, _ptr(y), _lo(y), yp, _ptr(x), _lo(x), xp,
+    _lib.check(lib.semseg_bn_bwd_reduce(_ptr(dy), _lo(dy), dp, _ptr(y), _lo(y), yp, _mask_ptr(mask, m, c), _ptr(x),
+                                        _lo(x), xp,
                                         _ptr(mean_invstd), _ptr(scale_shift), m, c, int(bool(relu)), _ptr(ws), nf,
                                         _ptr(sums), _stream()),
                "semseg_bn_bwd_reduce")
     return sums
 
 
-def bn_bwd_apply(dy, y, x, mean_invstd, gamma, sums, count, relu, want_dres=False, scale_shift=None):
+def bn_bwd_apply(dy, y, x, mean_invstd, gamma, sums, count, relu, want_dres=False, scale_shift=None, mask=None):
     lib = _lib.load()
     n, h, w, c, dp = _nhwc_meta(dy)
     _, _, _, _, xp = _nhwc_meta(x)
@@ -504,7 +519,8 @@
     dx = empty_act((n, h, w, c), split, dy.device)
     dres = empty_act((n, h, w, c), split, dy.device) if want_dres else None
     dgb = torch.empty((2, c), dtype=torch.float32, device=dy.device)
-    _lib.check(lib.semseg_bn_bwd_apply(_ptr(dy), _lo(dy), dp, _ptr(y), _lo(y), yp, _ptr(x), _lo(x), xp,
+    _lib.check(lib.semseg_bn_bwd_apply(_ptr(dy), _lo(dy), dp, _ptr(y), _lo(y), yp, _mask_ptr(mask, n * h * w, c),
+                                       _ptr(x), _lo(x), xp,
                                        _ptr(mean_invstd), _ptr(gamma), _ptr(scale_shift), _ptr(sums), float(count),
                                        n * h * w, c, int(bool(relu)), _ptr(dx), _lo(dx), c, _ptr(dres), _lo(dres), c,
                                        _ptr(dgb), _stream()), "semseg_bn_bwd_apply")
@@ -700,7 +716,7 @@
     return mi, ss
 
 
-def bn_bwd_reduce_p2p(dy, y, x, mean_invstd, relu, scale_shift, px):
+def bn_bwd_reduce_p2p(dy, y, x, mean_invstd, relu, scale_shift, px, mask=None):
     lib = _lib.load()
     n, h, w, c, dp = _nhwc_meta(dy)
     _, _, _, _, xp = _nhwc_meta(x)
@@ -710,7 +726,8 @@
     out = torch.empty((2, 2, c), dtype=torch.float32, device=dy.device)
     slot, seq = px.next()
     _same_form(dy, y, x)
-    _lib.check(lib.semseg_bn_bwd_reduce_p2p(_ptr(dy), _lo(dy), dp, _ptr(y), _lo(y), yp, _ptr(x), _lo(x), xp,
+    _lib.check(lib.semseg_bn_bwd_reduce_p2p(_ptr(dy), _lo(dy), dp, _ptr(y), _lo(y), yp, _mask_ptr(mask, m, c), _ptr(x),
+                                            _lo(x), xp,
                                             _ptr(mean_invstd),
                                             _ptr(scale_shift), m, c, int(bool(relu)), _ptr(ws), nf, _ptr(out[0]),
                                             _ptr(out[1]), px.data_ptrs, px.flag_ptrs, _ptr(px.counter), px.world,
```

Result: faster. 542.3 (median of 6 runs) (+4.2%).
